# apelykh/deep-audio-mixer

Hardware: AMD Instinct MI355X
Metric: stem-spectrogram-frames/sec (train) (higher is better)
Workload: dtype f32; 1 GPU; C3: model_resnet (ResNet18, 8 stems) train step incl. STFT front-end, 8-stem 3 s @ 44.1 kHz stereo clips, n_fft 2048 hop 1024 -> 8x1025x130 per clip; batch_per_gpu=8, global_batch=8, parallelism=dp1, hip_graph=True, world_size=1, device_index=0, grad_buckets=1, allreduce_overlap=False

## Files before the change

deep-audio-mixer_amd/_lib.py:

```python
import ctypes
import os

import torch
import torch.utils.data

_HERE = os.path.dirname(os.path.abspath(__file__))
LIB_PATH = os.environ.get('DAM_LIB_PATH') or os.path.join(_HERE, 'libdam_hip.so')

EXPECTED_ABI = 27

_STATUS = {0: 'DAM_OK', -1: 'DAM_ERR_BAD_ARG', -2: 'DAM_ERR_UNSUPPORTED', -3: 'DAM_ERR_LAUNCH',
           -4: 'DAM_ERR_WORKSPACE'}

c_i, c_i64, c_f, c_p = ctypes.c_int, ctypes.c_int64, ctypes.c_float, ctypes.c_void_p
c_d = ctypes.c_double

SIGNATURES = {
    'dam_arch': (ctypes.c_char_p, []),
    'dam_abi_version': (c_i, []),
    'dam_host_dontfork_pinned': (c_i, [c_p, c_p]),
    'dam_step_mark_create': (c_i, [c_p]),
    'dam_step_mark_record': (c_i, [c_p, c_p]),
    'dam_step_mark_wait': (c_i, [c_p, c_p]),
    'dam_step_mark_synchronize': (c_i, [c_p]),
    'dam_step_mark_destroy': (c_i, [c_p]),
    'dam_stft_twiddle_count': (c_i64, [c_i]),
    'dam_stft_fill_twiddles_host': (c_i, [c_i, c_p]),
    'dam_stft_logmag_f32': (c_i, [c_p, c_i, c_i64, c_i64, c_i, c_i64, c_p, c_p, c_p, c_i, c_i, c_f, c_i, c_p, c_p]),
    'dam_stft_logmag_strided_f32': (c_i, [c_p, c_i, c_i64, c_i64, c_i64, c_i64, c_i64, c_i, c_i64, c_i64, c_p, c_p, c_p,
                                          c_i, c_i, c_f, c_i, c_p, c_p, c_i, c_p]),
    'dam_stft_complex_f32': (c_i, [c_p, c_i, c_i64, c_i64, c_i, c_i64, c_i64, c_i64, c_p, c_p, c_p, c_i, c_i, c_p, c_p]),
    'dam_stft_complex_strided_f32': (c_i, [c_p, c_i, c_i64, c_i64, c_i64, c_i64, c_i64, c_i64, c_i64, c_i, c_i64, c_i64,
                                           c_p, c_p, c_p, c_i, c_i, c_p, c_p]),
    'dam_istft_workspace_bytes': (c_i64, [c_i64, c_i64, c_i, c_i, c_i64]),
    'dam_istft_f32': (c_i, [c_p, c_p, c_i64, c_i64, c_i, c_i, c_i64, c_p, c_p, c_p, c_p, c_i64, c_p]),
    'dam_augment_gains_f32': (c_i, [ctypes.c_uint64, c_p, c_i64, c_i, c_i, c_f, c_f, c_p, c_p]),
    'dam_conv_packed_weight_count': (c_i64, [c_i, c_i, c_i, c_i]),
    'dam_conv_pack_weights_f32': (c_i, [c_p, c_i, c_i, c_i, c_i, c_i, c_p, c_p]),
    'dam_conv_pack_weights_multi_f32': (c_i, [c_p, c_i, c_i64, c_p]),
    'dam_conv2d_tapgrid_f32': (c_i, [c_p, c_i, c_i, c_i, c_i, c_i, c_p, c_i, c_i, c_p, c_p, c_p, c_i, c_i, c_p] +
                               [c_i] * 17 + [c_p, c_p, c_p, c_p, c_p, c_p, c_i64, c_p, c_p]),
    'dam_conv_batch_bytes': (c_i64, []),
    'dam_conv_batch_init': (c_i, [c_p]),
    'dam_conv_batch_flush': (c_i, [c_p, c_p]),
    'dam_conv_last_launch': (c_i, [c_p]),
    'dam_conv2d_wgrad_workspace_floats': (c_i64, [c_i, c_i, c_i, c_i]),
    'dam_conv2d_wgrad_f32': (c_i, [c_p, c_i, c_i, c_i, c_i, c_i, c_p, c_p, c_i, c_p] + [c_i] * 9 +
                             [c_p, c_i, c_p, c_i64, c_p, c_p]),
    'dam_wgrad_queue_bytes': (c_i64, []),
    'dam_wgrad_queue_init': (c_i, [c_p]),
    'dam_wgrad_queue_pending': (c_i, [c_p]),
    'dam_wgrad_queue_flush': (c_i, [c_p, c_p]),
    'dam_wgrad_queue_set_batching': (c_i, [c_p, c_i]),
    'dam_wgrad_last_launch': (c_i, [c_p]),
    'dam_bn_workspace_floats': (c_i64, [c_i]),
    'dam_bn_stats_f32': (c_i, [c_p, c_i64, c_i, c_p, c_p, c_p, c_p, c_p, c_f, c_f, c_p, c_p, c_p, c_p, c_p, c_p]),
    'dam_bn_finalize_f32': (c_i, [c_p, c_i, c_i, c_p, c_p, c_p, c_p, c_p, c_f, c_f, c_p, c_p, c_p, c_p, c_p]),
    'dam_conv1x1_pair_f32': (c_i, [c_p, c_p, c_i, c_p, c_p, c_i, c_i, c_i, c_i, c_i, c_i, c_p, c_i, c_i, c_i, c_i, c_i, c_p]),
    'dam_dgrad_s2_3x3_f32': (c_i, [c_p, c_p, c_p, c_p, c_i, c_i, c_i, c_i, c_i, c_p, c_i, c_i, c_p, c_p, c_p, c_p]),
    'dam_conv_s2_pair_fwd_f32': (c_i, [c_p, c_p, c_p, c_i, c_i, c_i, c_i, c_i, c_p, c_p, c_p, c_p, c_p, c_p]),
    'dam_bn_finalize_pair_f32': (c_i, [c_p, c_p, c_i, c_i, c_p, c_p, c_p]),
    'dam_strip_diag_counters': (c_i, [c_p, c_i]),
    'dam_bn_stats_partial_f32': (c_i, [c_p, c_i64, c_i, c_p, c_p, c_p]),
    'dam_bn_finalize_apply_f32': (c_i, [c_p, c_i, c_i, c_p, c_p, c_i64, c_p, c_p, c_p, c_i, c_p, c_p, c_p]),
    'dam_bn_eval_affine_f32': (c_i, [c_i, c_p, c_p, c_p, c_p, c_f, c_p, c_p, c_p, c_p, c_p]),
    'dam_bn_apply_f32': (c_i, [c_p, c_i64, c_i, c_p, c_p, c_p, c_p, c_p, c_i, c_p, c_p, c_p]),
    'dam_bn_stats_pair_f32': (c_i, [c_p, c_p, c_i64, c_i, c_p, c_p, c_p, c_p]),
    'dam_bn_pair_workspace_floats': (c_i64, [c_i]),
    'dam_bn_backward_pair_f32': (c_i, [c_p, c_p, c_p, c_i64, c_i, c_i] + [c_p] * 16),
    'dam_bn_backward_f32': (c_i, [c_p, c_p, c_p, c_i64, c_i, c_p, c_p, c_p, c_i, c_p, c_p, c_p, c_p, c_p, c_p, c_p, c_i, c_p]),
    'dam_channel_sum_f32': (c_i, [c_p, c_i64, c_i, c_i, c_p, c_p, c_p]),
    'dam_dropout_tick': (c_i, [c_p, c_i64, c_p, c_p]),
    'dam_dropout_apply_f32': (c_i, [c_p, c_i64, c_f, ctypes.c_uint64, c_p, c_p, c_p]),
    'dam_heads_fwd_f32': (c_i, [c_p, c_i, c_i, c_i, c_i, c_p, c_p, c_p, c_p, c_p, c_p, c_p]),
    'dam_heads_bwd_workspace_floats': (c_i64, [c_i, c_i, c_i, c_i]),
    'dam_heads_bwd_f32': (c_i, [c_p, c_p, c_p, c_i, c_i, c_i, c_i, c_p, c_p, c_p, c_p, c_p, c_p, c_p, c_p, c_p]),
    'dam_masksum_fwd_f32': (c_i, [c_p, c_p, c_i, c_i, c_i64, c_p, c_p]),
    'dam_masksum_workspace_floats': (c_i64, [c_i, c_i]),
    'dam_masksum_bwd_f32': (c_i, [c_p, c_p, c_i, c_i, c_i64, c_p, c_p, c_p]),
    'dam_masksum_mse_f32': (c_i, [c_p, c_p, c_p, c_i, c_i, c_i64, c_p, c_p, c_p, c_p, c_p]),
    'dam_adam_l2_step_f32': (c_i, [c_p, c_p, c_p, c_p, c_i64, c_p, c_p, c_f, c_f, c_f, c_f, c_f, c_f, c_p, c_p]),
    'dam_digest64_u32': (c_i, [c_p, c_i64, c_i64, c_i, c_i, c_p, c_p]),
    'dam_gains_smooth': (c_i, [c_p, c_i, c_i, c_i, c_i, c_p, c_p, c_p, c_p]),
    'dam_gain_ramp_apply': (c_i, [c_p, c_i, c_p, c_i64, c_i64, c_i64, c_i, c_p, c_i, c_p]),
    'dam_mixdown_workspace_elems': (c_i64, [c_i64]),
    'dam_mixdown_peak_normalize': (c_i, [c_p, c_i, c_p, c_i, c_i64, c_i64, c_i, c_i, c_p, c_i, c_p, c_p]),
    'dam_nchw_to_nhwc16_f32': (c_i, [c_p, c_i, c_i, c_i64, c_p, c_p]),
    'dam_loudness_kweight_coeffs': (c_i, [c_d, c_p]),
    'dam_loudness_workspace_bytes': (c_i64, [c_i64, c_i]),
    'dam_loudness_block_energy': (c_i, [c_p, c_i, c_i64, c_i, c_i64, c_i64, c_p, c_p, c_p, c_i, c_d, c_p, c_p, c_p]),
    'dam_loudness_batch_workspace_bytes': (c_i64, [c_i, c_i64, c_i, c_i]),
    'dam_loudness_block_energy_batch': (c_i, [c_p, c_i, c_i, c_i64, c_i, c_i64, c_i64, c_i64, c_p, c_i, c_p, c_p, c_p, c_i,
                                              c_d, c_p, c_p, c_p]),
    'dam_loudness_gate': (c_i, [c_p, c_i, c_i, c_i, c_p, c_p]),
    'dam_loudness_target_gains': (c_i, [c_p, c_p, c_i, c_p, c_p]),
    'dam_pcm_tile_frames': (c_i64, [c_i]),
    'dam_pcm_max_blocks': (c_i, []),
    'dam_pcm_encode': (c_i, [c_p, c_i, c_i, c_i64, c_p, c_i, c_i, c_i, ctypes.c_uint64, c_p, c_p, c_p]),
    'dam_true_peak_taps_host': (c_i, [c_p]),
    'dam_true_peak_tile_samples': (c_i64, []),
    'dam_true_peak_max_blocks': (c_i, []),
    'dam_true_peak_workspace_bytes': (c_i64, [c_i, c_i64, c_i]),
    'dam_true_peak_batch': (c_i, [c_p, c_i, c_i, c_i64, c_i, c_i64, c_i64, c_i64, c_p, c_i, c_p, c_p, c_p, c_p]),
    'dam_peak_limit_gains': (c_i, [c_p, c_p, c_i, c_i, c_d, c_p]),
    'dam_limiter_tile_samples': (c_i64, []),
    'dam_limiter_max_lookahead': (c_i, []),
    'dam_limiter_max_hold': (c_i, []),
    'dam_limiter_workspace_bytes': (c_i64, [c_i, c_i64]),
    'dam_limiter_apply': (c_i, [c_p, c_i, c_i, c_i64, c_i, c_i64, c_i64, c_i64, c_p, c_d, c_i, c_i, c_p, c_i, c_p, c_p, c_p, c_p]),
    'dam_loudness_window_power': (c_i, [c_p, c_i, c_i, c_i, c_i, c_p, c_p, c_p]),
    'dam_loudness_curve_stats': (c_i, [c_p, c_i, c_i, c_p, c_p]),
    'dam_loudness_profile_error': (c_i, [c_p, c_p, c_i, c_i, c_i, c_p, c_p, c_p]),
    'dam_spectrum_frames_per_block': (c_i, []),
    'dam_spectrum_max_bands': (c_i, []),
    'dam_spectrum_workspace_bytes': (c_i64, [c_i, c_i64, c_i, c_i]),
    'dam_spectrum_band_power': (c_i, [c_p, c_i, c_i, c_i, c_i, c_i64, c_i64, c_i64, c_i64, c_i64, c_p, c_i, c_p, c_p, c_i, c_i,
                                      c_p, c_i, c_p, c_p, c_p]),
    'dam_spectrum_balance_error': (c_i, [c_p, c_p, c_i, c_i, c_p, c_p, c_p]),
    'dam_gainfit_tile_samples': (c_i64, []),
    'dam_gainfit_workspace_bytes': (c_i64, [c_i, c_i64, c_i]),
    'dam_gainfit_moments': (c_i, [c_p, c_i, c_i, c_i, c_i64, c_i64, c_i64, c_i64, c_p, c_i, c_i64, c_i64, c_i, c_p, c_p, c_p]),
    'dam_gainfit_solve': (c_i, [c_p, c_i, c_i, c_i, c_d, c_p, c_p, c_p, c_p]),
    'dam_gainfit_gain_error': (c_i, [c_p, c_p, c_i, c_i, c_i, c_i, c_p, c_p, c_p, c_p]),
}



class BnFin(ctypes.Structure):
    _fields_ = [('gamma', c_p), ('beta', c_p), ('running_mean', c_p), ('running_var', c_p), ('num_batches_tracked', c_p),
                ('momentum', c_f), ('eps', c_f), ('save_mean', c_p), ('save_invstd', c_p), ('scale', c_p), ('shift', c_p)]


class BnBwdSums(ctypes.Structure):
    _fields_ = [('x', c_p), ('mean', c_p), ('invstd', c_p), ('mask_scale', c_p), ('mask_shift', c_p), ('res_mask_bits', c_p),
                ('mask_bits', c_p)]


_lib = None


def lib():
    global _lib
    if torch.cuda._is_in_bad_fork() or torch.utils.data.get_worker_info() is not None:
        raise RuntimeError('deep_audio_mixer_amd: a GPU kernel was asked for in a DataLoader worker / forked child process '
                           '(pid %d).  The GPU belongs to the parent: workers of MultitrackAudioDataset return host PCM '
                           '(PcmItem / HostPcmBatch) and the front-end runs in the main process -- see '
                           'features.batch_features(batch)' % os.getpid())
    if _lib is None:
        if not os.path.exists(LIB_PATH):
            raise RuntimeError('libdam_hip.so is not built (%s): run `python __graft_entry__.py` or '
                               '`python deep-audio-mixer_amd/build.py`; there is no CPU fallback' % LIB_PATH)
        l = ctypes.CDLL(LIB_PATH)
        l.dam_abi_version.restype, l.dam_abi_version.argtypes = c_i, []
        have = l.dam_abi_version()
        if have != EXPECTED_ABI:
            raise RuntimeError('%s speaks ABI version %d, this package expects %d: the library is stale -- rebuild it '
                               '(`python deep-audio-mixer_amd/build.py --force`)' % (LIB_PATH, have, EXPECTED_ABI))
        for name, (res, args) in SIGNATURES.items():
            fn = getattr(l, name)
            fn.restype, fn.argtypes = res, args
        _lib = l
    return _lib


def check(status, what):
    if status != 0:
        raise RuntimeError('%s failed: %s (%d)' % (what, _STATUS.get(status, '?'), status))


def ptr(t):
    return None if t is None else t.data_ptr()


def stream():
    return torch.cuda.current_stream().cuda_stream


def require_cuda(*tensors):
    for t in tensors:
        if t is not None and not t.is_cuda:
            raise RuntimeError('deep_audio_mixer_amd kernels run on the GPU only (got a %s tensor); '
                               'there is no CPU fallback' % t.device)
```

deep-audio-mixer_amd/csrc/dam_bn.hip:

```cpp
#include <type_traits>
#include "dam_common.h"

namespace dam {
namespace {

constexpr int BN_MAX_PARTS = 1024;
static_assert(BN_MAX_PARTS == BN_BWD_RECORDS_MAX, "records a data-gradient epilogue may leave");

struct BnLaunch { int threads, q, r, parts; int64_t ppb; };

inline BnLaunch bn_plan(int64_t P, int C, int max_parts = BN_MAX_PARTS) {
    BnLaunch l;
    l.q = C / 4;
    l.r = 256 / l.q;
    if (l.r < 1) l.r = 1;
    l.threads = l.q * l.r;
    int64_t parts = cdiv(P, (int64_t)l.r * 16);
    if (parts > max_parts) {
        parts = max_parts;
        while (l.threads < 1024 && parts * l.threads < 131072 && (size_t)(l.r * 2) * C * 3 * sizeof(float) <= 48 * 1024) {
            l.r *= 2;
            l.threads *= 2;
        }
    }
// ... 534 lines not shown
template <int MASK, int NB>
__global__ __launch_bounds__(FA_THREADS) void bn_bwd_fin_apply_kernel(const float* __restrict__ partial, int parts, int C, int CS,
                                                                       double count, int training, const BnBwdSides<NB> sd,
                                                                       const float* __restrict__ dy, const float* __restrict__ y_mask,
                                                                       int64_t P, int64_t ppr, const float* __restrict__ mscale,
                                                                       const float* __restrict__ mshift) {
    constexpr int NR = 1 + NB;
    __shared__ double red[FA_THREADS * NR];
    __shared__ __attribute__((aligned(16))) float tab[3 * NB * 32];
    const int tid = threadIdx.x, slice = blockIdx.y, q = CS / 4, tq = tid % q, tp = tid / q, ppi = FA_THREADS / q;
    const int Q = C / 4, cq = slice * q + tq;
    const int64_t lo = blockIdx.x * ppr, hi = (lo + ppr < P) ? lo + ppr : P;
    constexpr int UB = NB == 1 ? 3 : 2;
    const int64_t step = (int64_t)ppi * UB;
    float4 gv[2][UB], xv[NB][2][UB], mv[2][UB];
    auto load = [&](auto set, int64_t p0) {
        constexpr int S = decltype(set)::value;
#pragma unroll
        for (int u = 0; u < UB; ++u) {
            const int64_t p = p0 + (int64_t)u * ppi;
            const bool ok = p < hi;
            gv[S][u] = ok ? reinterpret_cast<const float4*>(dy)[p * Q + cq] : zero4();
#pragma unroll
            for (int s = 0; s < NB; ++s) xv[s][S][u] = ok ? reinterpret_cast<const float4*>(sd.s[s].x)[p * Q + cq] : zero4();
            if (MASK == 1) mv[S][u] = ok ? reinterpret_cast<const float4*>(y_mask)[p * Q + cq] : zero4();
            if (MASK == 3) mv[S][u] = sign_quad(ok ? reinterpret_cast<const unsigned char*>(y_mask)[p * Q + cq] : 0);
        }
    };
    load(FaSet<0>{}, lo + tp);
    float4 msc = zero4(), msh = zero4();
    if (MASK == 2) { msc = reinterpret_cast<const float4*>(mscale)[cq]; msh = reinterpret_cast<const float4*>(mshift)[cq]; }
    {
        const int cl = tid % CS, ch = slice * CS + cl;
        float gam[NB], inv[NB], mu[NB];
#pragma unroll
        for (int s = 0; s < NB; ++s) { gam[s] = sd.s[s].gamma[ch]; inv[s] = sd.s[s].invstd[ch]; mu[s] = sd.s[s].mean[ch]; }
        double acc[NR];
        fa_slice_sums<NR, NR>(partial, parts, C, ch, CS, red, acc, [](const float (&r)[NR], double (&v)[NR]) {
#pragma unroll
            for (int k = 0; k < NR; ++k) v[k] = (double)r[k];
        });
        if (tid < CS) {
#pragma unroll
            for (int s = 0; s < NB; ++s) {
                const double s1 = acc[0], s2 = acc[1 + s];
                const double g = (double)gam[s] * inv[s];
                double c2 = 0, c3 = 0;
                if (training) { c2 = -g * inv[s] * s2 / count; c3 = -g * s1 / count - c2 * mu[s]; }
                float* t = tab + 3 * s * CS;
                t[cl] = (float)g; t[CS + cl] = (float)c2; t[2 * CS + cl] = (float)c3;
                if (blockIdx.x == 0) { sd.s[s].dbeta[ch] = (float)s1; sd.s[s].dgamma[ch] = (float)s2; }
            }
        }
        __syncthreads();
    }
    float4 k[NB][3];
#pragma unroll
    for (int i = 0; i < 3 * NB; ++i) k[i / 3][i % 3] = *reinterpret_cast<const float4*>(tab + i * CS + tq * 4);
    fa_stream(lo + tp, hi, step, load, [&](auto set, int64_t p0) {
        constexpr int S = decltype(set)::value;
#pragma unroll
        for (int u = 0; u < UB; ++u) {
            const int64_t p = p0 + (int64_t)u * ppi;
            if (p < hi) {
                float4 g = gv[S][u];
                if (MASK != 0) {
                    float4 m = mv[S][u];
                    if (MASK == 2) {
                        const float4 v = xv[0][S][u];
                        m = make_float4(fmaf(v.x, msc.x, msh.x), fmaf(v.y, msc.y, msh.y), fmaf(v.z, msc.z, msh.z), fmaf(v.w, msc.w, msh.w));
                    }
                    g.x = m.x > 0.f ? g.x : 0.f; g.y = m.y > 0.f ? g.y : 0.f; g.z = m.z > 0.f ? g.z : 0.f; g.w = m.w > 0.f ? g.w : 0.f;
                }
                float4 o[NB];
#pragma unroll
                for (int s = 0; s < NB; ++s) {
                    const float4 v = xv[s][S][u], c1 = k[s][0], c2 = k[s][1], c3 = k[s][2];
                    o[s].x = fmaf(c1.x, g.x, fmaf(c2.x, v.x, c3.x)); o[s].y = fmaf(c1.y, g.y, fmaf(c2.y, v.y, c3.y));
                    o[s].z = fmaf(c1.z, g.z, fmaf(c2.z, v.z, c3.z)); o[s].w = fmaf(c1.w, g.w, fmaf(c2.w, v.w, c3.w));
                }
#pragma unroll
                for (int s = 0; s < NB; ++s) reinterpret_cast<float4*>(sd.s[s].dx)[p * Q + cq] = o[s];
            }
        }
    });
}

inline int elt_blocks(int64_t n) {
    int64_t b = cdiv(n, 256);
    return (int)(b < 4096 ? (b < 1 ? 1 : b) : 4096);
}

constexpr int FA_PARTS_KB = 64;
inline int fa_max_parts(int C, int rec_floats) {
    int m = FA_PARTS_KB * 1024 / (fa_cs(C) * rec_floats * 4);
    if (m > BN_MAX_PARTS) m = BN_MAX_PARTS;
    return m < 64 ? 64 : m;
}

inline bool fin_args(const dam_bn_fin* f, BnFinArgs* a) {
    if (!f || !f->gamma || !f->beta || !f->save_mean || !f->save_invstd || !f->scale || !f->shift) return false;
    *a = BnFinArgs{f->gamma, f->beta, f->running_mean, f->running_var, (long long*)f->num_batches_tracked, f->momentum,
                   f->eps, f->save_mean, f->save_invstd, f->scale, f->shift};
    return true;
}

template <int... MASKS, typename F>
inline bool with_mask(int mask, F f) {
    return ((mask == MASKS ? (f(std::integral_constant<int, MASKS>{}), true) : false) || ...);
}

template <int NB, int... MASKS>
inline int bn_bwd_launch(const BnLaunch& l, bool given, bool fused, int mask, const BnBwdSides<NB>& sd, const float* dy,
                         const float* y_mask, int64_t P, int C, int training, const float* mask_scale, const float* mask_shift,
                         float* workspace, hipStream_t st) {
    if (!given) {
        const bool known = with_mask<MASKS...>(mask, [&](auto m) {
            hipLaunchKernelGGL((bn_bwd_partial_kernel<decltype(m)::value, NB>), dim3(l.parts), dim3(l.threads),
                               (size_t)l.r * C * (1 + NB) * sizeof(float), st, dy, y_mask, sd, P, C, l.q, l.r, l.ppb, mask_scale,
                               mask_shift, workspace);
        });
        if (!known) return DAM_ERR_BAD_ARG;
        DAM_CHECK_LAUNCH();
    }
    if (fused) {
        const FaPlan f = fa_plan(P, C);
        const bool known = with_mask<MASKS...>(mask, [&](auto m) {
            hipLaunchKernelGGL((bn_bwd_fin_apply_kernel<decltype(m)::value, NB>), dim3(f.nranges, f.nslices), dim3(FA_THREADS), 0, st,
                               (const float*)workspace, l.parts, C, f.cs, (double)P, training, sd, dy, y_mask, P, f.ppr, mask_scale,
                               mask_shift);
        });
        if (!known) return DAM_ERR_BAD_ARG;
        DAM_CHECK_LAUNCH();
    }
    return DAM_OK;
}

}
}

using namespace dam;

extern "C" int64_t dam_bn_workspace_floats(int C) { return (int64_t)BN_RECORDS_MAX * C * 3; }

extern "C" int dam_bn_stats_partial_f32(const float* x, int64_t n_pixels, int C, float* workspace, int* parts_host, void* stream) {
    if (!x || !workspace || !parts_host || n_pixels <= 0) return DAM_ERR_BAD_ARG;
    if (C % 16 || C > 1024) return DAM_ERR_UNSUPPORTED;
    const BnLaunch l = bn_plan(n_pixels, C, fa_max_parts(C, 3));
    hipLaunchKernelGGL(bn_stats_partial_kernel, dim3(l.parts), dim3(l.threads), (size_t)l.r * C * 3 * sizeof(float), (hipStream_t)stream,
                       x, n_pixels, C, l.q, l.r, l.ppb, workspace, (const float*)nullptr, (float*)nullptr);
    DAM_CHECK_LAUNCH();
    *parts_host = l.parts;
    return DAM_OK;
}

extern "C" int dam_bn_finalize_apply_f32(const float* partial, int parts, int C, const dam_bn_fin* fin, const float* x,
                                         int64_t n_pixels, const float* res, const float* res_scale, const float* res_shift,
                                         int relu, float* y, uint8_t* sign_bits, void* stream) {
    BnFinArgs a;
    if (!partial || parts <= 0 || !fin_args(fin, &a) || !x || !y || n_pixels <= 0) return DAM_ERR_BAD_ARG;
    if (res_scale && (!res || !res_shift)) return DAM_ERR_BAD_ARG;
    if (C % 16 || C > 1024) return DAM_ERR_UNSUPPORTED;
    hipStream_t st = (hipStream_t)stream;
    if (!fa_fwd_table_ok(C, parts)) {
        int rc = dam_bn_finalize_f32(partial, parts, C, fin->gamma, fin->beta, fin->running_mean, fin->running_var,
                                     fin->num_batches_tracked, fin->momentum, fin->eps, fin->save_mean, fin->save_invstd, fin->scale,
                                     fin->shift, stream);
        if (rc != DAM_OK) return rc;
        return dam_bn_apply_f32(x, n_pixels, C, fin->scale, fin->shift, res, res_scale, res_shift, relu, y, sign_bits, stream);
    }
    const FaPlan f = fa_plan(n_pixels, C);
    hipLaunchKernelGGL(bn_fin_apply_kernel, dim3(f.nranges, f.nslices), dim3(FA_THREADS), 0, st, partial, parts, C, f.cs, a, x,
                       n_pixels, f.ppr, res, res_scale, res_shift, relu, y, sign_bits);
    DAM_CHECK_LAUNCH();
    return DAM_OK;
}

extern "C" int dam_bn_stats_f32(const float* x, int64_t n_pixels, int C, const float* gamma, const float* beta,
                                float* running_mean, float* running_var, int64_t* num_batches_tracked,
                                float momentum, float eps, float* save_mean, float* save_invstd, float* scale,
                                float* shift, float* workspace, void* stream) {
    if (!x || !gamma || !beta || !save_mean || !save_invstd || !scale || !shift || !workspace || n_pixels <= 0)
        return DAM_ERR_BAD_ARG;
    if (C % 16 || C > 1024) return DAM_ERR_UNSUPPORTED;
    const BnLaunch l = bn_plan(n_pixels, C);
    hipStream_t st = (hipStream_t)stream;
    hipLaunchKernelGGL(bn_stats_partial_kernel, dim3(l.parts), dim3(l.threads), (size_t)l.r * C * 3 * sizeof(float), st,
                       x, n_pixels, C, l.q, l.r, l.ppb, workspace, (const float*)nullptr, (float*)nullptr);
    DAM_CHECK_LAUNCH();
    hipLaunchKernelGGL(bn_stats_finalize_kernel, dim3(C), dim3(64), 0, st, workspace, l.parts, C,
                       gamma, beta, running_mean, running_var, (long long*)num_batches_tracked, momentum, eps,
                       save_mean, save_invstd, scale, shift, BnFinArgs{}, (const float*)nullptr);
    DAM_CHECK_LAUNCH();
    return DAM_OK;
}

extern "C" int dam_bn_stats_pair_f32(const float* x_a, const float* x_b, int64_t n_pixels, int C, const dam_bn_fin* a,
                                     const dam_bn_fin* b, float* workspace, void* stream) {
    BnFinArgs fa, fb;
    if (!x_a || !x_b || !fin_args(a, &fa) || !fin_args(b, &fb) || !workspace || n_pixels <= 0) return DAM_ERR_BAD_ARG;
    if (C % 16 || C > 1024) return DAM_ERR_UNSUPPORTED;
    const BnLaunch l = bn_plan(n_pixels, C);
    hipStream_t st = (hipStream_t)stream;
    float* ws_b = workspace + (size_t)BN_RECORDS_MAX * C * 3;
    hipLaunchKernelGGL(bn_stats_partial_kernel, dim3(l.parts, 2), dim3(l.threads), (size_t)l.r * C * 3 * sizeof(float), st, x_a,
                       n_pixels, C, l.q, l.r, l.ppb, workspace, x_b, ws_b);
    DAM_CHECK_LAUNCH();
    hipLaunchKernelGGL(bn_stats_finalize_kernel, dim3(C, 2), dim3(64), 0, st, workspace, l.parts, C, fa.gamma, fa.beta,
                       fa.running_mean, fa.running_var, fa.num_batches, fa.momentum, fa.eps, fa.save_mean, fa.save_invstd, fa.scale,
                       fa.shift, fb, (const float*)ws_b);
    DAM_CHECK_LAUNCH();
    return DAM_OK;
}

extern "C" int dam_bn_finalize_f32(const float* partial, int parts, int C, const float* gamma, const float* beta,
                                   float* running_mean, float* running_var, int64_t* num_batches_tracked,
                                   float momentum, float eps, float* save_mean, float* save_invstd, float* scale,
                                   float* shift, void* stream) {
    if (!partial || parts <= 0 || C <= 0 || !gamma || !beta || !save_mean || !save_invstd || !scale || !shift)
        return DAM_ERR_BAD_ARG;
    hipLaunchKernelGGL(bn_stats_finalize_kernel, dim3(C), dim3(64), 0, (hipStream_t)stream, partial, parts, C, gamma, beta,
                       running_mean, running_var, (long long*)num_batches_tracked, momentum, eps, save_mean, save_invstd,
                       scale, shift, BnFinArgs{}, (const float*)nullptr);
    DAM_CHECK_LAUNCH();
    return DAM_OK;
}

extern "C" int dam_bn_finalize_pair_f32(const float* partial_a, const float* partial_b, int parts, int C, const dam_bn_fin* a,
                                        const dam_bn_fin* b, void* stream) {
    BnFinArgs fa, fb;
    if (!partial_a || !partial_b || parts <= 0 || C <= 0 || !fin_args(a, &fa) || !fin_args(b, &fb)) return DAM_ERR_BAD_ARG;
    hipLaunchKernelGGL(bn_stats_finalize_kernel, dim3(C, 2), dim3(64), 0, (hipStream_t)stream, partial_a, parts, C, fa.gamma, fa.beta,
                       fa.running_mean, fa.running_var, fa.num_batches, fa.momentum, fa.eps, fa.save_mean, fa.save_invstd, fa.scale,
                       fa.shift, fb, partial_b);
    DAM_CHECK_LAUNCH();
    return DAM_OK;
}

extern "C" int dam_bn_eval_affine_f32(int C, const float* gamma, const float* beta, const float* running_mean,
                                      const float* running_var, float eps, float* save_mean, float* save_invstd,
                                      float* scale, float* shift, void* stream) {
    if (!gamma || !beta || !running_mean || !running_var || !save_mean || !save_invstd || !scale || !shift || C <= 0)
        return DAM_ERR_BAD_ARG;
    hipLaunchKernelGGL(bn_eval_affine_kernel, dim3((unsigned)cdiv(C, 64)), dim3(64), 0, (hipStream_t)stream, C, gamma, beta,
                       running_mean, running_var, eps, save_mean, save_invstd, scale, shift);
    DAM_CHECK_LAUNCH();
    return DAM_OK;
}

extern "C" int dam_bn_apply_f32(const float* x, int64_t n_pixels, int C, const float* scale, const float* shift,
                                const float* res, const float* res_scale, const float* res_shift, int relu, float* y,
                                uint8_t* sign_bits, void* stream) {
    if (!x || !scale || !shift || !y || n_pixels <= 0) return DAM_ERR_BAD_ARG;
    if (C % 16) return DAM_ERR_UNSUPPORTED;
    if (res_scale && (!res || !res_shift)) return DAM_ERR_BAD_ARG;
    const int64_t nq = n_pixels * (C / 4);
    hipLaunchKernelGGL(bn_apply_kernel, dim3(elt_blocks(nq)), dim3(256), 0, (hipStream_t)stream, x, nq, C / 4, scale, shift,
                       res, res_scale, res_shift, relu, y, sign_bits);
    DAM_CHECK_LAUNCH();
    return DAM_OK;
}

extern "C" int dam_bn_backward_f32(const float* dy, const float* y_mask, const float* x, int64_t n_pixels, int C,
                                   const float* gamma, const float* save_mean, const float* save_invstd, int training,
                                   const float* mask_scale, const float* mask_shift, const uint8_t* mask_bits, float* dx,
                                   float* dgamma, float* dbeta, float* workspace, int partials_given, void* stream) {
    if (!dy || !x || !gamma || !save_mean || !save_invstd || !dx || !dgamma || !dbeta || !workspace || n_pixels <= 0)
        return DAM_ERR_BAD_ARG;
    if ((mask_scale != nullptr) != (mask_shift != nullptr) || (y_mask && mask_scale) || (mask_bits && (y_mask || mask_scale)))
        return DAM_ERR_BAD_ARG;
    if (mask_bits) y_mask = reinterpret_cast<const float*>(mask_bits);
    if (C % 16 || C > 1024) return DAM_ERR_UNSUPPORTED;
    BnLaunch l = bn_plan(n_pixels, C, fa_max_parts(C, 2));
    if (partials_given < 0 || partials_given > BN_MAX_PARTS) return DAM_ERR_BAD_ARG;
    if (partials_given) l.parts = partials_given;
    const bool fused = fa_table_ok(C, l.parts, 2);
    hipStream_t st = (hipStream_t)stream;
    const int mask = mask_bits ? 3 : (y_mask ? 1 : (mask_scale ? 2 : 0));
    const BnBwdSides<1> sd{{{x, gamma, save_mean, save_invstd, dx, dgamma, dbeta}}};
    const int rc = bn_bwd_launch<1, 0, 1, 2, 3>(l, partials_given != 0, fused, mask, sd, dy, y_mask, n_pixels, C, training,
                                                mask_scale, mask_shift, workspace, st);
    if (rc != DAM_OK || fused) return rc;
    float* coef = workspace + (size_t)BN_MAX_PARTS * C * 2;
    hipLaunchKernelGGL(bn_bwd_finalize_kernel, dim3(C), dim3(64), 0, st, workspace, l.parts, C,
                       (double)n_pixels, gamma, save_mean, save_invstd, training, dgamma, dbeta, coef);
    DAM_CHECK_LAUNCH();
    const int64_t nq = n_pixels * (C / 4);
    const bool known = with_mask<0, 1, 2, 3>(mask, [&](auto m) {
        hipLaunchKernelGGL(bn_bwd_apply_kernel<decltype(m)::value>, dim3(elt_blocks(nq)), dim3(256), 0, st, dy, y_mask, x, nq, C / 4,
                           C, (const float*)coef, mask_scale, mask_shift, dx);
    });
    if (!known) return DAM_ERR_BAD_ARG;
    DAM_CHECK_LAUNCH();
    return DAM_OK;
}

extern "C" int64_t dam_bn_pair_workspace_floats(int C) { return (int64_t)BN_MAX_PARTS * C * 3 + 6 * (int64_t)C; }

extern "C" int dam_bn_backward_pair_f32(const float* dy, const float* y_mask, const uint8_t* mask_bits, int64_t n_pixels, int C,
                                        int training,
                                        const float* x_a, const float* gamma_a, const float* mean_a, const float* invstd_a,
                                        float* dx_a, float* dgamma_a, float* dbeta_a,
                                        const float* x_b, const float* gamma_b, const float* mean_b, const float* invstd_b,
                                        float* dx_b, float* dgamma_b, float* dbeta_b, float* workspace, void* stream) {
    if ((y_mask != nullptr) == (mask_bits != nullptr)) return DAM_ERR_BAD_ARG;
    const bool bits = mask_bits != nullptr;
    if (bits) y_mask = reinterpret_cast<const float*>(mask_bits);
    if (!dy || !y_mask || !x_a || !gamma_a || !mean_a || !invstd_a || !dx_a || !dgamma_a || !dbeta_a || !x_b || !gamma_b ||
        !mean_b || !invstd_b || !dx_b || !dgamma_b || !dbeta_b || !workspace || n_pixels <= 0)
        return DAM_ERR_BAD_ARG;
    if (C % 16 || C > 1024) return DAM_ERR_UNSUPPORTED;
    const BnLaunch l = bn_plan(n_pixels, C, fa_max_parts(C, 3));
    if ((size_t)l.r * C * 3 * sizeof(float) > 64 * 1024) return DAM_ERR_UNSUPPORTED;
    const BnBwdSides<2> sd{{{x_a, gamma_a, mean_a, invstd_a, dx_a, dgamma_a, dbeta_a},
                            {x_b, gamma_b, mean_b, invstd_b, dx_b, dgamma_b, dbeta_b}}};
    return bn_bwd_launch<2, 1, 3>(l, false, true, bits ? 3 : 1, sd, dy, y_mask, n_pixels, C, training, nullptr, nullptr, workspace,
                                  (hipStream_t)stream);
}

extern "C" int dam_channel_sum_f32(const float* x, int64_t n_pixels, int C, int n_real, float* out, float* workspace,
                                   void* stream) {
    if (!x || !out || !workspace || n_pixels <= 0 || n_real <= 0 || n_real > C) return DAM_ERR_BAD_ARG;
    if (C % 16 || C > 1024) return DAM_ERR_UNSUPPORTED;
    const BnLaunch l = bn_plan(n_pixels, C);
    hipStream_t st = (hipStream_t)stream;
    hipLaunchKernelGGL(channel_sum_partial_kernel, dim3(l.parts), dim3(l.threads), (size_t)l.r * C * sizeof(float), st, x,
                       n_pixels, C, l.q, l.r, l.ppb, workspace);
    DAM_CHECK_LAUNCH();
    hipLaunchKernelGGL(channel_sum_finalize_kernel, dim3(n_real), dim3(64), 0, st, workspace, l.parts, C,
                       n_real, out);
    DAM_CHECK_LAUNCH();
    return DAM_OK;
}
```

deep-audio-mixer_amd/csrc/dam_conv.hip:

```cpp
#include <cstdlib>
#include "dam_common.h"
#include "dam_conv_geo.h"
#include "dam_conv_stage.h"

namespace dam {

namespace {

typedef float v4f __attribute__((ext_vector_type(4)));

constexpr int GEO_PACK_MAX = 4;
struct ConvGeoPack {
    ConvGeo g[GEO_PACK_MAX];
    int n, B;
};

template <int MB, int NB>
__global__ __launch_bounds__(256) void conv_igemm_kernel(const ConvGeoPack pk, const float* __restrict__ X,
                                                         const float4* __restrict__ Wp, const float* __restrict__ bias,
                                                         const float* __restrict__ in_scale,
                                                         const float* __restrict__ in_shift, float* __restrict__ Y,
                                                         const float* __restrict__ res, const float* __restrict__ res_mask,
                                                         float* __restrict__ splitk_ws) {
    extern __shared__ __attribute__((aligned(16))) unsigned char smem[];
// ... 249 lines not shown
};

int conv_pack_dispatch(const ConvGeoPack& pk, const ConvLaunchRec& r, hipStream_t st) {
#define DAM_CONV_PCASE(M_, N_) \
    if (r.MB == M_ && r.NB == N_) return launch_conv_pack<M_, N_>(pk, r.lds, r.X, r.Wp, r.bias, r.sc, r.sh, r.Y, r.res, r.res_mask, r.ws, st)
    DAM_CONV_PCASE(4, 4); DAM_CONV_PCASE(4, 2); DAM_CONV_PCASE(4, 1);
    DAM_CONV_PCASE(4, 3); DAM_CONV_PCASE(2, 3); DAM_CONV_PCASE(1, 3);
    DAM_CONV_PCASE(2, 4); DAM_CONV_PCASE(2, 2); DAM_CONV_PCASE(2, 1);
    DAM_CONV_PCASE(1, 4); DAM_CONV_PCASE(1, 2); DAM_CONV_PCASE(1, 1);
#undef DAM_CONV_PCASE
    return DAM_ERR_UNSUPPORTED;
}

int conv_batch_flush(ConvBatch& b, hipStream_t st) {
    int i = 0, rc = DAM_OK;
    while (i < b.n && rc == DAM_OK) {
        const ConvLaunchRec& r = b.rec[i];
        ConvGeoPack pk;
        pk.B = r.g.B; pk.n = 0;
        size_t lds = 0;
        int k = i;
        while (k < b.n && pk.n < GEO_PACK_MAX) {
            const ConvLaunchRec& q = b.rec[k];
            if (q.MB != r.MB || q.NB != r.NB || q.X != r.X || q.Wp != r.Wp || q.bias != r.bias || q.sc != r.sc || q.sh != r.sh ||
                q.Y != r.Y || q.res != r.res || q.res_mask != r.res_mask || q.g.B != r.g.B)
                break;
            pk.g[pk.n++] = q.g;
            lds = q.lds > lds ? q.lds : lds;
            ++k;
        }
        ConvLaunchRec merged = r;
        merged.lds = lds;
        rc = conv_pack_dispatch(pk, merged, st);
        i = k;
    }
    b.n = 0;
    return rc;
}

}
}

extern "C" int64_t dam_conv_packed_weight_count(int n_out, int k_in, int kh, int kw) {
    if (n_out <= 0 || k_in <= 0 || kh <= 0 || kw <= 0) return 0;
    return (int64_t)kh * kw * dam::cdiv(k_in, 16) * dam::cdiv(n_out, 16) * 256;
}

extern "C" int dam_conv_pack_weights_f32(const float* w_oihw, int O, int I, int KH, int KW, int transpose,
                                         float* packed, void* stream) {
    using namespace dam;
    if (!w_oihw || !packed || O <= 0 || I <= 0 || KH <= 0 || KW <= 0) return DAM_ERR_BAD_ARG;
    const int n = transpose ? I : O, k = transpose ? O : I;
    const int nchunks = (int)cdiv(k, 16), nblks = (int)cdiv(n, 16);
    const int64_t total = (int64_t)KH * KW * nchunks * nblks * 256;
    const int blocks = (int)(cdiv(total, 256) < 2048 ? cdiv(total, 256) : 2048);
    hipLaunchKernelGGL(pack_weights_kernel, dim3(blocks), dim3(256), 0, (hipStream_t)stream, w_oihw, O, I, KH, KW,
                       transpose, nchunks, nblks, packed, total);
    DAM_CHECK_LAUNCH();
    return DAM_OK;
}

extern "C" int dam_conv_pack_weights_multi_f32(const int64_t* desc_dev, int n_tensors, int64_t max_total, void* stream) {
    using namespace dam;
    if (!desc_dev || n_tensors <= 0 || max_total <= 0) return DAM_ERR_BAD_ARG;
    if (n_tensors > 65535) return DAM_ERR_UNSUPPORTED;
    int64_t bx = cdiv(max_total, 256 * 9);
    if (bx > 256) bx = 256;
    if (bx < 1) bx = 1;
    hipLaunchKernelGGL(pack_weights_multi_kernel, dim3((unsigned)bx, (unsigned)n_tensors), dim3(256), 0, (hipStream_t)stream,
                       reinterpret_cast<const long long*>(desc_dev));
    DAM_CHECK_LAUNCH();
    return DAM_OK;
}

namespace dam {
namespace {

template <int NB, int NCHMAX>
__global__ __launch_bounds__(256) void conv1x1_direct_kernel(const ConvGeo g, const float* __restrict__ X,
                                                             const float4* __restrict__ Wp, const float* __restrict__ bias,
                                                             float* __restrict__ Y, const float* __restrict__ res,
                                                             const float* __restrict__ res_mask, int segs, int total_units) {
    const int lane = threadIdx.x & 63, wave = threadIdx.x >> 6;
    const int j = lane & 15, kq = lane >> 4;
    const int unit = blockIdx.x * 4 + wave;
    if (unit >= total_units) return;
    const int nb0 = blockIdx.y * NB;
    const int seg = unit % segs, row = unit / segs, img = row / g.Ho, oh = row - img * g.Ho;
    const int ow = seg * 16 + j;
    const bool valid = ow < g.Wo;
    const int ih = oh * g.s + g.off_h, iw = ow * g.s + g.off_w;
    const bool inb = valid && ih >= 0 && ih < g.H && iw >= 0 && iw < g.W;
    const __amdgpu_buffer_rsrc_t xr = __builtin_amdgcn_make_buffer_rsrc(const_cast<float*>(X), 0, 0x7fffffff, 0x00020000);
    const __amdgpu_buffer_rsrc_t wr = __builtin_amdgcn_make_buffer_rsrc(const_cast<float4*>(Wp), 0, 0x7fffffff, 0x00020000);
    const int xoff = inb ? (((img * g.H + ih) * g.W + iw) * g.C + kq * 4) * 4 : 0x7fffffff;
    const int tap = g.wt_base;
    float4 xv[NCHMAX], wa[NCHMAX][NB];
#pragma unroll
    for (int c = 0; c < NCHMAX; ++c) {
        const bool cok = c < g.nchunks;
        xv[c] = __builtin_bit_cast(float4, __builtin_amdgcn_raw_buffer_load_b128(xr, cok ? xoff : 0x7fffffff, c * 64, 0));
#pragma unroll
        for (int nb = 0; nb < NB; ++nb)
            wa[c][nb] = __builtin_bit_cast(float4, __builtin_amdgcn_raw_buffer_load_b128(
                wr, cok ? lane * 16 : 0x7fffffff, (((tap * g.nchunks + c) * g.NBtot + nb0 + nb) * 64) * 16, 0));
    }
    v4f acc[NB];
#pragma unroll
    for (int nb = 0; nb < NB; ++nb) acc[nb] = (v4f){0.f, 0.f, 0.f, 0.f};
#pragma unroll
    for (int c = 0; c < NCHMAX; ++c)
#pragma unroll
        for (int nb = 0; nb < NB; ++nb) {
            acc[nb] = __builtin_amdgcn_mfma_f32_16x16x4f32(wa[c][nb].x, xv[c].x, acc[nb], 0, 0, 0);
            acc[nb] = __builtin_amdgcn_mfma_f32_16x16x4f32(wa[c][nb].y, xv[c].y, acc[nb], 0, 0, 0);
            acc[nb] = __builtin_amdgcn_mfma_f32_16x16x4f32(wa[c][nb].z, xv[c].z, acc[nb], 0, 0, 0);
            acc[nb] = __builtin_amdgcn_mfma_f32_16x16x4f32(wa[c][nb].w, xv[c].w, acc[nb], 0, 0, 0);
        }
    if (!valid) return;
    const size_t opix = ((size_t)img * g.OHt + (oh * g.os + g.oo_h)) * g.OWt + (ow * g.os + g.oo_w);
#pragma unroll
    for (int nb = 0; nb < NB; ++nb) {
        const int ch = (nb0 + nb) * 16 + kq * 4;
        v4f v = acc[nb];
        if (bias) v += *reinterpret_cast<const v4f*>(bias + ch);
        const size_t o = opix * g.N + ch;
        if (res) {
            const float4 rv = *reinterpret_cast<const float4*>(res + o);
            if (res_mask) {
                const float4 mv = *reinterpret_cast<const float4*>(res_mask + o);
                v.x += mv.x > 0.f ? rv.x : 0.f; v.y += mv.y > 0.f ? rv.y : 0.f;
                v.z += mv.z > 0.f ? rv.z : 0.f; v.w += mv.w > 0.f ? rv.w : 0.f;
            } else {
                v.x += rv.x; v.y += rv.y; v.z += rv.z; v.w += rv.w;
            }
        }
        if (g.relu_out) { v.x = fmaxf(v.x, 0.f); v.y = fmaxf(v.y, 0.f); v.z = fmaxf(v.z, 0.f); v.w = fmaxf(v.w, 0.f); }
        *reinterpret_cast<float4*>(Y + o) = make_float4(v.x, v.y, v.z, v.w);
    }
}

template <int NB, int R, bool BOTH>
__global__ __launch_bounds__(256) void conv1x1_pair_kernel(const float* __restrict__ X1, const float4* __restrict__ Wp1, int tap1,
                                                           const float* __restrict__ X2, const float4* __restrict__ Wp2, int tap2,
                                                           int B, int H, int W, int C, int N, float* __restrict__ Y, int OHt, int OWt,
                                                           int os, int oo_h, int oo_w, int segs, int total_units) {
    const int lane = threadIdx.x & 63, wave = threadIdx.x >> 6;
    const int j = lane & 15, kq = lane >> 4;
    const int unit = blockIdx.x * 4 + wave;
    if (unit >= total_units) return;
    const int nb0 = blockIdx.y * NB, nch = C / 16, NBtot = N / 16;
    const int seg = unit % segs, row = unit / segs, img = row / H, oh = row - img * H;
    const int ow = seg * 16 + j;
    const bool valid = ow < W;
    const int xoff = valid ? (((img * H + oh) * W + ow) * C + kq * 4) * 4 : 0x7fffffff;
    v4f acc[NB];
#pragma unroll
    for (int nb = 0; nb < NB; ++nb) acc[nb] = (v4f){0.f, 0.f, 0.f, 0.f};
    const __amdgpu_buffer_rsrc_t xr1 = __builtin_amdgcn_make_buffer_rsrc(const_cast<float*>(X1), 0, 0x7fffffff, 0x00020000);
    const __amdgpu_buffer_rsrc_t wr1 = __builtin_amdgcn_make_buffer_rsrc(const_cast<float4*>(Wp1), 0, 0x7fffffff, 0x00020000);
    const __amdgpu_buffer_rsrc_t xr2 = __builtin_amdgcn_make_buffer_rsrc(const_cast<float*>(X2), 0, 0x7fffffff, 0x00020000);
    const __amdgpu_buffer_rsrc_t wr2 = __builtin_amdgcn_make_buffer_rsrc(const_cast<float4*>(Wp2), 0, 0x7fffffff, 0x00020000);
#define DAM_PAIR_LOAD(XR_, WR_, TAP_, C0_, XV_, WA_)                                                                          \
    _Pragma("unroll") for (int c = 0; c < R; ++c) {                                                                           \
        const bool cok = (C0_) + c < nch;                                                                                     \
        XV_[c] = __builtin_bit_cast(float4, __builtin_amdgcn_raw_buffer_load_b128(XR_, cok ? xoff : 0x7fffffff, ((C0_) + c) * 64, 0)); \
        _Pragma("unroll") for (int nb = 0; nb < NB; ++nb)                                                                     \
            WA_[c][nb] = __builtin_bit_cast(float4, __builtin_amdgcn_raw_buffer_load_b128(                                    \
                WR_, cok ? lane * 16 : 0x7fffffff, ((((TAP_) * nch + (C0_) + c) * NBtot + nb0 + nb) * 64) * 16, 0));          \
    }
#define DAM_PAIR_MFMA(XV_, WA_)                                    \
    _Pragma("unroll") for (int c = 0; c < R; ++c)                                                                             \
        _Pragma("unroll") for (int nb = 0; nb < NB; ++nb) {                                                                   \
            acc[nb] = __builtin_amdgcn_mfma_f32_16x16x4f32(WA_[c][nb].x, XV_[c].x, acc[nb], 0, 0, 0);                         \
            acc[nb] = __builtin_amdgcn_mfma_f32_16x16x4f32(WA_[c][nb].y, XV_[c].y, acc[nb], 0, 0, 0);                         \
            acc[nb] = __builtin_amdgcn_mfma_f32_16x16x4f32(WA_[c][nb].z, XV_[c].z, acc[nb], 0, 0, 0);                         \
            acc[nb] = __builtin_amdgcn_mfma_f32_16x16x4f32(WA_[c][nb].w, XV_[c].w, acc[nb], 0, 0, 0);                         \
        }
    if constexpr (BOTH) {
        float4 xa[R], wa[R][NB], xb[R], wb[R][NB];
        DAM_PAIR_LOAD(xr1, wr1, tap1, 0, xa, wa)
        DAM_PAIR_LOAD(xr2, wr2, tap2, 0, xb, wb)
        DAM_PAIR_MFMA(xa, wa)
        DAM_PAIR_MFMA(xb, wb)
    } else {
        float4 xa[R], wa[R][NB], xb[R], wb[R][NB];
        const int rounds = (nch + R - 1) / R, total = 2 * rounds;
        DAM_PAIR_LOAD(xr1, wr1, tap1, 0, xa, wa)
#pragma unroll 1
        for (int r = 0; r < total; r += 2) {
            {
                const int q = r + 1, c0 = (q >= rounds ? q - rounds : q) * R;
                if (q >= rounds) { DAM_PAIR_LOAD(xr2, wr2, tap2, c0, xb, wb) } else { DAM_PAIR_LOAD(xr1, wr1, tap1, c0, xb, wb) }
            }
            DAM_PAIR_MFMA(xa, wa)
            if (r + 2 < total) {
                const int q = r + 2, c0 = (q >= rounds ? q - rounds : q) * R;
                if (q >= rounds) { DAM_PAIR_LOAD(xr2, wr2, tap2, c0, xa, wa) } else { DAM_PAIR_LOAD(xr1, wr1, tap1, c0, xa, wa) }
            }
            DAM_PAIR_MFMA(xb, wb)
        }
    }
#undef DAM_PAIR_LOAD
#undef DAM_PAIR_MFMA
    if (!valid) return;
    const size_t opix = ((size_t)img * OHt + (oh * os + oo_h)) * OWt + (ow * os + oo_w);
#pragma unroll
    for (int nb = 0; nb < NB; ++nb) {
        const int ch = (nb0 + nb) * 16 + kq * 4;
        *reinterpret_cast<float4*>(Y + opix * N + ch) = make_float4(acc[nb].x, acc[nb].y, acc[nb].z, acc[nb].w);
    }
}

template <int NB, int NCHMAX>
int launch_conv1x1(const ConvGeo& g, const float* X, const float* Wp, const float* bias, float* Y, const float* res,
                   const float* res_mask, hipStream_t st) {
    const int segs = (int)cdiv(g.Wo, 16);
    const int64_t units = (int64_t)g.B * g.Ho * segs;
    if (units >= (1ll << 30)) return DAM_ERR_UNSUPPORTED;
    hipLaunchKernelGGL((conv1x1_direct_kernel<NB, NCHMAX>), dim3((unsigned)cdiv(units, 4), (unsigned)(g.N / 16 / NB)), dim3(256), 0, st,
                       g, X, reinterpret_cast<const float4*>(Wp), bias, Y, res, res_mask, segs, (int)units);
    DAM_CHECK_LAUNCH();
    conv_last_launch = ConvLaunchNote{CONV_FAM_1X1, 0, NB, NCHMAX, 0, 0, 0, 0, 0, 0, 0, 1, 1};
    return DAM_OK;
}

}
}

extern "C" int dam_conv1x1_pair_f32(const float* x1, const float* w1_packed, int tap1, const float* x2, const float* w2_packed,
                                    int tap2, int B, int H, int W, int C, int n_out, float* y, int OHt, int OWt, int out_stride,
                                    int out_off_h, int out_off_w, void* stream) {
    using namespace dam;
    if (!x1 || !w1_packed || !x2 || !w2_packed || !y || B <= 0 || H <= 0 || W <= 0 || tap1 < 0 || tap2 < 0 || out_stride < 1)
        return DAM_ERR_BAD_ARG;
    if (C % 16 || n_out % 16 || C <= 0 || n_out <= 0) return DAM_ERR_UNSUPPORTED;
    if ((H - 1) * out_stride + out_off_h >= OHt || (W - 1) * out_stride + out_off_w >= OWt || out_off_h < 0 || out_off_w < 0)
        return DAM_ERR_BAD_ARG;
    if ((int64_t)B * H * W * C * 4 >= (1ll << 31)) return DAM_ERR_UNSUPPORTED;
    const int segs = (int)cdiv(W, 16);
    const int64_t units = (int64_t)B * H * segs;
    if (units >= (1ll << 30)) return DAM_ERR_UNSUPPORTED;
    const int nblk = n_out / 16, nch = C / 16;
    hipStream_t st = (hipStream_t)stream;
#define DAM_PAIR_GO(NB_, R_, BOTH_)                                                                                           \
    hipLaunchKernelGGL((conv1x1_pair_kernel<NB_, R_, BOTH_>), dim3((unsigned)cdiv(units, 4), (unsigned)(nblk / NB_)), dim3(256), 0, st, x1, \
                       reinterpret_cast<const float4*>(w1_packed), tap1, x2, reinterpret_cast<const float4*>(w2_packed), tap2, B, H, W, \
                       C, n_out, y, OHt, OWt, out_stride, out_off_h, out_off_w, segs, (int)units)
    if (nblk % 2 == 0) {
        if (nch <= 2) DAM_PAIR_GO(2, 2, true); else if (nch <= 4) DAM_PAIR_GO(2, 4, true); else DAM_PAIR_GO(2, 4, false);
    } else {
        if (nch <= 2) DAM_PAIR_GO(1, 2, true); else if (nch <= 4) DAM_PAIR_GO(1, 4, true); else DAM_PAIR_GO(1, 8, false);
    }
#undef DAM_PAIR_GO
    DAM_CHECK_LAUNCH();
    return DAM_OK;
}

namespace dam {
thread_local ConvLaunchNote conv_last_launch{};
}

extern "C" int dam_conv_last_launch(int* out16_host) {
    if (!out16_host) return DAM_ERR_BAD_ARG;
    const dam::ConvLaunchNote& n = dam::conv_last_launch;
    const int v[16] = {n.family, n.MB, n.NB, n.NCH, n.T33, n.LW, n.EPI, n.SO, n.PU, n.STATS, n.KS, n.ksplit, n.ranges, 0, 0, 0};
    for (int i = 0; i < 16; ++i) out16_host[i] = v[i];
    return DAM_OK;
}

extern "C" int64_t dam_conv_batch_bytes(void) { return (int64_t)sizeof(dam::ConvBatch); }

extern "C" int dam_conv_batch_init(void* batch) {
    if (!batch) return DAM_ERR_BAD_ARG;
    dam::ConvBatch* b = static_cast<dam::ConvBatch*>(batch);
    b->magic = dam::CONV_BATCH_MAGIC;
    b->n = 0;
    return DAM_OK;
}

extern "C" int dam_conv_batch_flush(void* batch, void* stream) {
    dam::ConvBatch* b = static_cast<dam::ConvBatch*>(batch);
    if (!b || b->magic != dam::CONV_BATCH_MAGIC) return DAM_ERR_BAD_ARG;
    return dam::conv_batch_flush(*b, (hipStream_t)stream);
}

extern "C" int dam_conv2d_tapgrid_f32(const float* x, int B, int H, int W, int C, int in_nchw, const float* w_packed,
                                      int k_chunks, int n_out, const float* bias, const float* in_scale,
                                      const float* in_shift, int relu_in, int relu_out, float* y, int OHt, int OWt, int Ho, int Wo,
                                      int out_stride, int out_off_h, int out_off_w, int in_stride, int nA, int nB,
                                      int off_h, int step_h, int off_w, int step_w, int wt_base, int wt_sa, int wt_sb,
                                      const float* res, const float* res_mask, float* bn_partial, int* bn_parts_host,
                                      const dam_bn_bwd_sums* bn_bwd, float* workspace, int64_t workspace_floats,
                                      void* batch, void* stream) {
    using namespace dam;
    conv_last_launch = ConvLaunchNote{};
    if (bn_parts_host) *bn_parts_host = 0;
    BnBwdEpi bwd{};
    if (bn_bwd && bn_bwd->x) {
        if (!bn_partial || !bn_parts_host || !bn_bwd->mean || !bn_bwd->invstd) return DAM_ERR_BAD_ARG;
        if (bn_bwd->mask_bits ? (bn_bwd->mask_scale || bn_bwd->mask_shift || !res) : (!bn_bwd->mask_scale || !bn_bwd->mask_shift))
            return DAM_ERR_BAD_ARG;
        if (res && (!bn_bwd->res_mask_bits || !res_mask)) return DAM_ERR_BAD_ARG;
        bwd = BnBwdEpi{bn_bwd->x, bn_bwd->mean, bn_bwd->invstd, bn_bwd->mask_scale, bn_bwd->mask_shift, bn_bwd->res_mask_bits,
                       bn_bwd->mask_bits};
    }
    if (!x || !w_packed || !y || B <= 0 || H <= 0 || W <= 0 || C <= 0 || Ho <= 0 || Wo <= 0 || nA <= 0 || nB <= 0)
        return DAM_ERR_BAD_ARG;
    if (n_out % 16 || (in_stride != 1 && in_stride != 2) || out_stride < 1) return DAM_ERR_UNSUPPORTED;
    if (in_nchw ? (C > 16 || k_chunks != 1) : (C % 16 || k_chunks != C / 16)) return DAM_ERR_UNSUPPORTED;
    if (in_scale && !in_shift) return DAM_ERR_BAD_ARG;
    if (B > 65535) return DAM_ERR_UNSUPPORTED;
    ConvGeo g;
    g.B = B; g.H = H; g.W = W; g.C = C; g.Ho = Ho; g.Wo = Wo; g.N = n_out; g.OHt = OHt; g.OWt = OWt;
    g.os = out_stride; g.oo_h = out_off_h; g.oo_w = out_off_w; g.s = in_stride; g.nA = nA; g.nB = nB;
    g.off_h = off_h; g.step_h = step_h; g.off_w = off_w; g.step_w = step_w;
    g.wt_base = wt_base; g.wt_sa = wt_sa; g.wt_sb = wt_sb;
    g.in_nchw = in_nchw; g.relu_in = relu_in; g.relu_out = relu_out != 0; g.nchunks = k_chunks; g.NBtot = n_out / 16;
    g.epi_bwd = 0;
    const int h_lo = off_h + (step_h < 0 ? (nA - 1) * step_h : 0), h_hi = off_h + (step_h > 0 ? (nA - 1) * step_h : 0);
    const int w_lo = off_w + (step_w < 0 ? (nB - 1) * step_w : 0), w_hi = off_w + (step_w > 0 ? (nB - 1) * step_w : 0);
    g.r0 = h_lo; g.c0 = w_lo;
    g.PWin = (Wo - 1) * in_stride + (w_hi - w_lo) + 1;
    g.PWs = (int)cdiv(g.PWin, in_stride);
    g.PWT = g.PWs * in_stride;

    hipStream_t st = (hipStream_t)stream;
    g.PR = 0; g.CG = 1; g.tiles_m = 0; g.ksplit = 1; g.gps = 1 << 30;
    if (nA == 1 && nB == 1 && !in_nchw && !in_scale && k_chunks <= 8 &&
        (int64_t)B * H * W * C * 4 < (1ll << 31) && (int64_t)B * OHt * OWt * n_out * 4 < (1ll << 62)) {
        const int nblk = n_out / 16;
        if (k_chunks <= 2) return nblk % 2 == 0 ? launch_conv1x1<2, 2>(g, x, w_packed, bias, y, res, res_mask, st)
                                                : launch_conv1x1<1, 2>(g, x, w_packed, bias, y, res, res_mask, st);
        if (k_chunks <= 4) return nblk % 2 == 0 ? launch_conv1x1<2, 4>(g, x, w_packed, bias, y, res, res_mask, st)
                                                : launch_conv1x1<1, 4>(g, x, w_packed, bias, y, res, res_mask, st);
        return nblk % 2 == 0 ? launch_conv1x1<2, 8>(g, x, w_packed, bias, y, res, res_mask, st)
                             : launch_conv1x1<1, 8>(g, x, w_packed, bias, y, res, res_mask, st);
    }
    if (!in_nchw) {
        int parts = 0;
        const int rc = conv_strip_try(g, h_lo, h_hi, x, w_packed, bias, y, res, res_mask, bn_partial, &parts,
                                      in_scale, in_shift, bwd, st);
        if (rc == DAM_OK) {
            if (bn_partial && bn_parts_host) *bn_parts_host = parts;
            return DAM_OK;
        }
        if (rc != DAM_ERR_UNSUPPORTED) return rc;
        if (bn_partial) {
            const int rc2 = conv_strip_try(g, h_lo, h_hi, x, w_packed, bias, y, res, res_mask, nullptr, nullptr, in_scale, in_shift,
                                           BnBwdEpi{}, st);
            if (rc2 == DAM_OK) return DAM_OK;
            if (rc2 != DAM_ERR_UNSUPPORTED) return rc2;
        }
    }
    if (!getenv("DAM_NO_PIPE")) {
        int parts = 0;
        const int rc = conv_pipe_try(g, h_hi - h_lo, x, w_packed, bias, in_scale, in_shift, y, res, res_mask, workspace,
                                     (bwd.x && res) ? nullptr : bn_partial, &parts, (bwd.x && res) ? BnBwdEpi{} : bwd, st);
        if (rc == DAM_OK && bn_partial && bn_parts_host) *bn_parts_host = parts;
        if (rc != DAM_ERR_UNSUPPORTED) return rc;
        if (nA == 3 && nB == 3 && !in_nchw && !bn_partial) {
            for (int ns = 2; ns <= 4; ++ns) {
                const int wd0 = (int)cdiv(Wo, ns);
                if (wd0 < 16) break;
                int rc2 = DAM_OK, done = 0;
                for (int ow0 = 0; ow0 < Wo && rc2 == DAM_OK; ow0 += wd0, ++done) {
                    ConvGeo g2 = g;
                    g2.Wo = Wo - ow0 < wd0 ? Wo - ow0 : wd0;
                    g2.oo_w = out_off_w + ow0 * out_stride;
                    g2.off_w = off_w + ow0 * in_stride;
                    g2.c0 = w_lo + ow0 * in_stride;
                    g2.PWin = (g2.Wo - 1) * in_stride + (w_hi - w_lo) + 1;
                    g2.PWs = (int)cdiv(g2.PWin, in_stride);
                    g2.PWT = g2.PWs * in_stride;
                    rc2 = conv_pipe_try(g2, h_hi - h_lo, x, w_packed, bias, in_scale, in_shift, y, res, res_mask, workspace, nullptr,
                                        nullptr, BnBwdEpi{}, st);
                }
                if (rc2 == DAM_OK) {
                    conv_last_launch.family = CONV_FAM_PIPE_RANGES;
                    conv_last_launch.ranges = done;
                    return DAM_OK;
                }
                if (rc2 != DAM_ERR_UNSUPPORTED || done > 1) return rc2 == DAM_ERR_UNSUPPORTED ? DAM_ERR_LAUNCH : rc2;
            }
        }
    }
    const int64_t npix = (int64_t)Ho * Wo;
    const int nblk = n_out / 16;
    int MB = 4, NB = nblk % 4 == 0 ? 4 : (nblk % 3 == 0 ? 3 : (nblk % 2 == 0 ? 2 : 1));
    auto wgs = [&](int mb, int nb) { return cdiv(npix, 64 * mb) * cdiv(nblk, nb) * B; };
    const bool can_split = workspace && out_stride == 1 && Ho == OHt && Wo == OWt && out_off_h == 0 && out_off_w == 0 &&
                           k_chunks >= 4;
    bool split = can_split;
    if (split) {
        int64_t best = -1;
        for (int mb = 4; mb >= 1; mb >>= 1) {
            const int64_t w = wgs(mb, NB);
            if (w < 400) continue;
            const int64_t cost = cdiv(w, 256) * (mb * NB + 1);
            if (best < 0 || cost < best) { best = cost; MB = mb; split = false; }
        }
    }
    if (split) {
        int64_t best_pad = -1;
        for (int mb = 4; mb >= 1; mb >>= 1) {
            const int64_t pad = cdiv(npix, 64 * mb) * 64 * mb;
            if (best_pad < 0 || pad * 10 < best_pad * 9) { best_pad = pad; MB = mb; }
        }
    } else if (!can_split) {
        while (wgs(MB, NB) < 512 && (MB > 1 || NB > 1)) {
            if (MB > 1 && (MB >= NB || NB == 1)) MB >>= 1; else NB >>= 1;
        }
    }
    const size_t LDS_MAX = 64 * 1024;
    int CG = 1;
    while (CG * 2 <= 4 && k_chunks % (CG * 2) == 0) CG *= 2;
    auto patch_rows = [&](int mb) {
        const int tm = 64 * mb;
        int rows_out = (int)((tm + Wo - 2) / Wo + 1);
        if (rows_out > Ho) rows_out = Ho;
        return (rows_out - 1) * in_stride + (h_hi - h_lo) + 1;
    };
    for (;;) {
        g.PR = patch_rows(MB);
        const size_t bytes = (size_t)CG * g.PR * g.PWT * 64;
        if (bytes <= LDS_MAX) break;
        if (CG > 1) CG >>= 1;
        else if (MB > 1) MB >>= 1;
        else if (bytes <= 150 * 1024) break;
        else return DAM_ERR_UNSUPPORTED;
    }
    g.CG = CG;
    g.tiles_m = (int)cdiv(npix, 64 * MB);
    if (split) {
        const int ngroups = k_chunks / CG;
        const int64_t w = wgs(MB, NB), out_elems = (int64_t)B * OHt * OWt * n_out;
        int ksplit = (int)cdiv(512, w);
        if (ksplit > 8) ksplit = 8;
        if (ksplit > ngroups) ksplit = ngroups;
        while (ksplit > 1 && ksplit * out_elems > workspace_floats) --ksplit;
        if (ksplit > 1) {
            g.gps = (int)cdiv(ngroups, ksplit);
            g.ksplit = (int)cdiv(ngroups, g.gps);
        }
    }
    const size_t lds = (size_t)CG * g.PR * g.PWT * 64;
    if (batch && g.ksplit == 1) {
        ConvBatch* cb = static_cast<ConvBatch*>(batch);
        if (cb->magic != CONV_BATCH_MAGIC) return DAM_ERR_BAD_ARG;
        if (cb->n == CONV_BATCH_MAX) {
            const int rc = conv_batch_flush(*cb, st);
            if (rc != DAM_OK) return rc;
        }
        ConvLaunchRec& r = cb->rec[cb->n++];
        r.g = g; r.MB = MB; r.NB = NB; r.lds = lds; r.X = x; r.Wp = w_packed; r.bias = bias; r.sc = in_scale; r.sh = in_shift;
        r.res = res; r.res_mask = res_mask; r.Y = y; r.ws = workspace;
        conv_last_launch = ConvLaunchNote{CONV_FAM_TILE_BATCH, MB, NB, 0, 0, 0, 0, 0, 0, 0, 0, 1, 1};
        return DAM_OK;
    }
#define DAM_CONV_CASE(M_, N_) \
    if (MB == M_ && NB == N_) return launch_conv<M_, N_>(g, lds, x, w_packed, bias, in_scale, in_shift, y, res, res_mask, workspace, st)
    DAM_CONV_CASE(4, 4); DAM_CONV_CASE(4, 2); DAM_CONV_CASE(4, 1);
    DAM_CONV_CASE(4, 3); DAM_CONV_CASE(2, 3); DAM_CONV_CASE(1, 3);
    DAM_CONV_CASE(2, 4); DAM_CONV_CASE(2, 2); DAM_CONV_CASE(2, 1);
    DAM_CONV_CASE(1, 4); DAM_CONV_CASE(1, 2); DAM_CONV_CASE(1, 1);
#undef DAM_CONV_CASE
    return DAM_ERR_UNSUPPORTED;
}
```

deep-audio-mixer_amd/csrc/dam_conv_geo.h:

```cpp
#pragma once
#include "dam_common.h"

namespace dam {

struct ConvGeo {
    int B, H, W, C;
    int Ho, Wo;
    int N;
    int OHt, OWt;
    int os, oo_h, oo_w;
    int s;
    int nA, nB;
    int off_h, step_h, off_w, step_w;
    int wt_base, wt_sa, wt_sb;
    int r0, c0;
    int PR, PWin, PWs, PWT;
    int nchunks, CG;
    int NBtot;
    int tiles_m;
    int in_nchw;
    int relu_in;
    int relu_out;
    int ksplit;
    int gps;
    int epi_bwd;
};

struct BnBwdEpi {
    const float* x;
    const float* mean; const float* invstd; const float* mscale; const float* mshift;
    const unsigned char* res_bits;
    const unsigned char* mask_bits;
};

struct StripGeo {
    int NR;
    int RH;
    int tiles_m, tpw, strips;
    int ring_off;
    int w_lds;
    int w_taps;
    unsigned wo_magic;
};

enum ConvFamily { CONV_FAM_NONE = 0, CONV_FAM_STRIP = 1, CONV_FAM_PIPE = 2, CONV_FAM_PIPE_RANGES = 3, CONV_FAM_TILE = 4,
                  CONV_FAM_TILE_BATCH = 5, CONV_FAM_1X1 = 6 };
struct ConvLaunchNote {
    int family, MB, NB, NCH, T33, LW, EPI, SO, PU, STATS, KS, ksplit, ranges;
};
extern thread_local ConvLaunchNote conv_last_launch;

int conv_strip_try(ConvGeo& g, int h_lo, int h_hi, const float* X, const float* Wp, const float* bias, float* Y,
                   const float* res, const float* res_mask, float* stats, int* stats_parts,
                   const float* in_scale, const float* in_shift, const BnBwdEpi& bwd, hipStream_t st);

int conv_pipe_try(ConvGeo g, int row_span, const float* X, const float* Wp, const float* bias, const float* sc, const float* sh,
                  float* Y, const float* res, const float* res_mask, float* workspace, float* stats, int* stats_parts,
                  const BnBwdEpi& bwd, hipStream_t st);

}
```

deep-audio-mixer_amd/csrc/dam_conv_pipe.hip:

```cpp
#include <climits>
#include <cstdlib>
#include "dam_common.h"
#include "dam_conv_geo.h"
#include "dam_conv_stage.h"

namespace dam {
namespace {

typedef float v4f __attribute__((ext_vector_type(4)));

constexpr int PIPE_LT = 256;
constexpr int PIPE_THREADS = 256 + PIPE_LT;
constexpr int PIPE_BUF1 = 32768;

#define DAM_PIPE_BARRIER() asm volatile("s_waitcnt lgkmcnt(0)\n\ts_barrier" ::: "memory")

#ifdef DAM_PIPE_STAMPS
#define DAM_PSTAMP(role, tag)                                                                                         \
    do {                                                                                                              \
        if (lane == 0 && (wave == 0 || wave == 4) && stamp_n < 64) {                                                  \
            const unsigned long long t_ = __builtin_readcyclecounter();                                               \
            stamp_p[(role) * 64 + stamp_n++] = ((unsigned long long)(tag) << 56) | (t_ & ((1ull << 56) - 1));         \
        }                                                                                                             \
    } while (0)
#else
#define DAM_PSTAMP(role, tag) do { } while (0)
#endif

struct PipeUnit {
    int p0, img, nb0, oh_first;
};

template <int UPX, int NB>
__device__ __forceinline__ PipeUnit pipe_decode(const ConvGeo& g, int unit, int nby, float inv_wo) {
    PipeUnit u;
    const int r = unit / g.tiles_m, tm = unit - r * g.tiles_m;
    u.img = r / nby;
    u.nb0 = (r - u.img * nby) * NB;
    u.p0 = tm * UPX;
    u.oh_first = fast_div(u.p0, g.Wo, inv_wo);
    return u;
}

template <int MB, int NB, int PIPE_U, int STATS, int KS>
__global__ __launch_bounds__(PIPE_THREADS) void conv_pipe_kernel(const ConvGeo g, const int nunits, const float* __restrict__ X,
                                                                 const float4* __restrict__ Wp, const float* __restrict__ bias,
                                                                 const float* __restrict__ in_scale,
                                                                 const float* __restrict__ in_shift, float* __restrict__ Y,
                                                                 const float* __restrict__ res, const float* __restrict__ res_mask,
                                                                 float* __restrict__ stamps, float* __restrict__ stats,
                                                                 const BnBwdEpi bwd) {
    extern __shared__ __attribute__((aligned(16))) unsigned char smem[];
    const int tid = threadIdx.x, lane = tid & 63;
    const int wave = __builtin_amdgcn_readfirstlane(tid >> 6);
    constexpr int MW = 16 * MB;
    constexpr int MT = 4 / KS;
    constexpr int UPX = MW * MT;
    constexpr int QM = 4 * KS - 1;
    const int HoWo = g.Ho * g.Wo;
    const float inv_wo = 1.0f / (float)g.Wo;
    const int chunk_bytes = g.PR * g.PWT * 64;
    const int stage_bytes = chunk_bytes * KS;
    const int nst = g.nchunks / KS;
    const int nby = g.N / 16 / NB;
    const bool xa = (gridDim.x & 7) == 0;
    const int G = xa ? (int)gridDim.x >> 3 : (int)gridDim.x;
    const int per_xcd = xa ? (nunits + 7) >> 3 : nunits;
    const int u_lo = xa ? (int)(blockIdx.x & 7) * per_xcd : 0;
    const int unit_end = u_lo + per_xcd < nunits ? u_lo + per_xcd : nunits;
    const int unit0 = u_lo + (xa ? (int)(blockIdx.x >> 3) : (int)blockIdx.x);
    if (unit0 >= unit_end) return;
    const size_t img_floats = (size_t)g.H * g.W * g.C;
#ifdef DAM_PIPE_STAMPS
    unsigned long long* stamp_p = reinterpret_cast<unsigned long long*>(stamps) + (size_t)blockIdx.x * 128;
    int stamp_n = 0;
#endif
    DAM_PSTAMP(wave >> 2, 1);

    if (wave >= 4) {
        const int ltid = tid - 256;
        const int WC = g.W * g.C;
        const int ipr = g.PWin * 4 * KS;
        const int total = g.PR * ipr;
        const int tab_off = PIPE_BUF1 + stage_bytes;
        const int dump_off = tab_off + (in_scale ? 2 * g.C * 4 : 0);
        int dst[PIPE_U], gcol[PIPE_U];
        {
            const int step_r = PIPE_LT / ipr, step_c = PIPE_LT - step_r * ipr;
            int pr = fast_div(ltid, ipr, 1.0f / (float)ipr), rem = ltid - pr * ipr;
#pragma unroll
            for (int u = 0; u < PIPE_U; ++u) {
                dst[u] = dump_off + ltid * 16; gcol[u] = INT_MIN;
                if (ltid + PIPE_LT * u < total) {
                    const int pw = rem / (4 * KS), cq = rem & QM;
                    const int slot = g.s == 1 ? pw : (pw & 1) * g.PWs + (pw >> 1);
                    dst[u] = ((pr * g.PWT + slot) * 16 + (cq & 3) * 4) * 4 + (cq >> 2) * chunk_bytes;
                    const int iw = g.c0 + pw;
                    if (iw >= 0 && iw < g.W) gcol[u] = (pr * WC + iw * g.C + cq * 4) * 4;
                }
                pr += step_r; rem += step_c;
                if (rem >= ipr) { rem -= ipr; ++pr; }
            }
        }
        const int cq4 = (lane & QM) * 4;
        const float relu_lo = g.relu_in ? 0.f : -__builtin_inff();
        float4 v[2][PIPE_U];
        int unit = unit0;
        PipeUnit cur = pipe_decode<UPX, NB>(g, unit, nby, inv_wo);
        int icg = 0;
        int rowb = (cur.oh_first * g.s + g.r0) * WC * 4;
        const unsigned img_bytes = (unsigned)img_floats * 4u;
        __amdgpu_buffer_rsrc_t xrsrc =
            __builtin_amdgcn_make_buffer_rsrc(const_cast<float*>(X + (size_t)cur.img * img_floats), 0, img_bytes, 0x00020000);
        bool head = true;
        int s_sb[2] = {0, 0}, s_cg[2] = {0, 0};
        bool s_live[2] = {false, false};
#define DAM_PIPE_REFILL(S_)                                                                                                \
    do {                                                                                                                   \
        const int sb_ = head ? rowb + icg * (64 * KS) : INT_MIN;                                                                \
        _Pragma("unroll") for (int u = 0; u < PIPE_U; ++u)                                                                 \
            v[S_][u] = __builtin_bit_cast(float4, __builtin_amdgcn_raw_buffer_load_b128(xrsrc, gcol[u] + sb_, 0, 0));      \
        s_sb[S_] = sb_; s_cg[S_] = icg; s_live[S_] = head;                                                                 \
        if (head) {                                                                                  \
            if (icg + 1 < nst) {                                                                                           \
                ++icg;                                                                                                     \
            } else if (unit + G < unit_end) {                                                                                \
                unit += G;                                                                                                 \
                cur = pipe_decode<UPX, NB>(g, unit, nby, inv_wo);                                                          \
                icg = 0;                                                                                                   \
                rowb = (cur.oh_first * g.s + g.r0) * WC * 4;                                                               \
                xrsrc = __builtin_amdgcn_make_buffer_rsrc(const_cast<float*>(X + (size_t)cur.img * img_floats), 0, img_bytes, \
                                                          0x00020000);                                                     \
            } else {                                                                                                       \
                head = false;                                                                                              \
            }                                                                                                              \
        }                                                                                                                  \
    } while (0)
#define DAM_PIPE_COMMIT(S_)                                  \
    do {                                                                                                                   \
        constexpr int boff_ = (S_) * PIPE_BUF1;                                                                            \
        if (in_scale) {                                          \
            const float4 sc = *reinterpret_cast<const float4*>(smem + tab_off + (s_cg[S_] * (16 * KS) + cq4) * 4);         \
            const float4 sh = *reinterpret_cast<const float4*>(smem + tab_off + (g.C + s_cg[S_] * (16 * KS) + cq4) * 4);   \
            _Pragma("unroll") for (int u = 0; u < PIPE_U; ++u) {                                                           \
                float4 x = v[S_][u];                                                                                       \
                x.x = fmaf(x.x, sc.x, sh.x); x.y = fmaf(x.y, sc.y, sh.y);                                                  \
                x.z = fmaf(x.z, sc.z, sh.z); x.w = fmaf(x.w, sc.w, sh.w);                                                  \
                x.x = fmaxf(x.x, relu_lo); x.y = fmaxf(x.y, relu_lo); x.z = fmaxf(x.z, relu_lo); x.w = fmaxf(x.w, relu_lo);  \
                if ((unsigned)(gcol[u] + s_sb[S_]) >= img_bytes) x = make_float4(0.f, 0.f, 0.f, 0.f);                      \
                *reinterpret_cast<float4*>(smem + boff_ + dst[u]) = x;                                                     \
            }                                                                                                              \
        } else {                                                                                                           \
            _Pragma("unroll") for (int u = 0; u < PIPE_U; ++u)                                                             \
                *reinterpret_cast<float4*>(smem + boff_ + dst[u]) = v[S_][u];                                              \
        }                                                                                                                  \
    } while (0)
#define DAM_PIPE_ROUND_END()                                 \
    do {                                                                                                                   \
        DAM_PSTAMP(1, 6);                                                                                                  \
        DAM_PIPE_BARRIER();                                                                                                \
        DAM_PSTAMP(1, 7);                                                                                                  \
    } while (0)
        if (in_scale)
            for (int e = ltid * 4; e < g.C; e += PIPE_LT * 4) {
                *reinterpret_cast<float4*>(smem + tab_off + e * 4) = *reinterpret_cast<const float4*>(in_scale + e);
                *reinterpret_cast<float4*>(smem + tab_off + (g.C + e) * 4) = *reinterpret_cast<const float4*>(in_shift + e);
            }
        if (g.s != 1)
            for (int e = ltid * 16; e < stage_bytes; e += PIPE_LT * 16) {
                *reinterpret_cast<float4*>(smem + e) = make_float4(0.f, 0.f, 0.f, 0.f);
                *reinterpret_cast<float4*>(smem + PIPE_BUF1 + e) = make_float4(0.f, 0.f, 0.f, 0.f);
            }
        DAM_PIPE_REFILL(0);
        __builtin_amdgcn_sched_barrier(0);
        DAM_PIPE_REFILL(1);
        __builtin_amdgcn_sched_barrier(0);
        DAM_PSTAMP(1, 2);
        DAM_PIPE_BARRIER();
        DAM_PSTAMP(1, 3);
        for (;;) {
            DAM_PIPE_COMMIT(0);
            DAM_PIPE_REFILL(0);
            DAM_PIPE_ROUND_END();
            if (!s_live[1]) break;
            DAM_PIPE_COMMIT(1);
            DAM_PIPE_REFILL(1);
            DAM_PIPE_ROUND_END();
            if (!s_live[0]) break;
        }
        DAM_PIPE_BARRIER();
#undef DAM_PIPE_REFILL
#undef DAM_PIPE_COMMIT
#undef DAM_PIPE_ROUND_END
        return;
    }

    const int j = lane & 15, kq = lane >> 4;
    const int mt = wave & (MT - 1), kh = wave / MT;
    const int part_off = PIPE_BUF1 + stage_bytes + (in_scale ? 2 * g.C * 4 : 0) + PIPE_LT * 16;
    int tapw[9], tapx[9];
#pragma unroll
    for (int t = 0; t < 9; ++t) {
        const int a = t / 3, b = t % 3;
        tapw[t] = (g.wt_base + a * g.wt_sa + b * g.wt_sb) * g.nchunks * g.NBtot * 1024;
        const int roff = g.off_h + a * g.step_h - g.r0, coff = g.off_w + b * g.step_w - g.c0;
        const int slotoff = g.s == 1 ? coff : (coff & 1) * g.PWs + (coff >> 1);
        tapx[t] = (roff * g.PWT + slotoff) * 64;
    }
    const int lane16 = lane * 16;
    const __amdgpu_buffer_rsrc_t wrsrc = __builtin_amdgcn_make_buffer_rsrc(const_cast<float4*>(Wp), 0, 0x7fffffff, 0x00020000);
    constexpr bool W9 = MB * NB == 1;
    constexpr int WSETS = W9 ? 9 : 3;
    v4f acc[MB][NB];
    float4 wa[WSETS][NB], xv[3][MB];
    int base_b[MB];
    int unit = unit0;
    PipeUnit cur = pipe_decode<UPX, NB>(g, unit, nby, inv_wo);
    int sbuf = 0;
#define DAM_PIPE_W(S_, CPART_, T_)                                                                                         \
    do {                                                                                                                   \
        const int ws_ = tapw[T_] + (CPART_);                                                                                \
        _Pragma("unroll") for (int nb = 0; nb < NB; ++nb)                                                                  \
            wa[S_][nb] = __builtin_bit_cast(float4, __builtin_amdgcn_raw_buffer_load_b128(wrsrc, lane16 + nb * 1024, ws_, 0)); \
    } while (0)
#define DAM_PIPE_X(S_, T_)                                                                                                 \
    do {                                                                                                                   \
        const int lo_ = boff + tapx[T_];                                                                                   \
        _Pragma("unroll") for (int mb = 0; mb < MB; ++mb)                                                                  \
            xv[S_][mb] = *reinterpret_cast<const float4*>(smem + base_b[mb] + lo_);                                        \
    } while (0)
#define DAM_PIPE_MFMA2(SW_, SX_)                                                                                           \
    do {                                                                                                                   \
        _Pragma("unroll") for (int mb = 0; mb < MB; ++mb)                                                                  \
            _Pragma("unroll") for (int nb = 0; nb < NB; ++nb) {                                                            \
                acc[mb][nb] = __builtin_amdgcn_mfma_f32_16x16x4f32(wa[SW_][nb].x, xv[SX_][mb].x, acc[mb][nb], 0, 0, 0);    \
                acc[mb][nb] = __builtin_amdgcn_mfma_f32_16x16x4f32(wa[SW_][nb].y, xv[SX_][mb].y, acc[mb][nb], 0, 0, 0);    \
                acc[mb][nb] = __builtin_amdgcn_mfma_f32_16x16x4f32(wa[SW_][nb].z, xv[SX_][mb].z, acc[mb][nb], 0, 0, 0);    \
                acc[mb][nb] = __builtin_amdgcn_mfma_f32_16x16x4f32(wa[SW_][nb].w, xv[SX_][mb].w, acc[mb][nb], 0, 0, 0);    \
            }                                                                                                              \
    } while (0)
#define DAM_PIPE_MFMA(S_) DAM_PIPE_MFMA2(S_, S_)
    {
        const int cfirst = (kh * g.NBtot + cur.nb0) * 1024;
        DAM_PIPE_W(0, cfirst, 0);
        DAM_PIPE_W(1, cfirst, 1);
        if constexpr (W9) {
            DAM_PIPE_W(2 % WSETS, cfirst, 2); DAM_PIPE_W(3 % WSETS, cfirst, 3); DAM_PIPE_W(4 % WSETS, cfirst, 4);
            DAM_PIPE_W(5 % WSETS, cfirst, 5); DAM_PIPE_W(6 % WSETS, cfirst, 6); DAM_PIPE_W(7 % WSETS, cfirst, 7);
            DAM_PIPE_W(8 % WSETS, cfirst, 8);
        }
    }
    DAM_PSTAMP(0, 2);
    DAM_PIPE_BARRIER();
    DAM_PSTAMP(0, 3);
    DAM_PIPE_BARRIER();
    DAM_PSTAMP(0, 5);
    for (;;) {
        const bool has_next = unit + G < unit_end;
        const PipeUnit nxt = has_next ? pipe_decode<UPX, NB>(g, unit + G, nby, inv_wo) : cur;
#pragma unroll
        for (int mb = 0; mb < MB; ++mb) {
            int p = cur.p0 + mt * MW + mb * 16 + j;
            p = p < HoWo ? p : HoWo - 1;
            const int oh = fast_div(p, g.Wo, inv_wo), ow = p - oh * g.Wo;
            base_b[mb] = (((oh - cur.oh_first) * g.s) * g.PWT + ow) * 64 + kq * 16;
#pragma unroll
            for (int nb = 0; nb < NB; ++nb) acc[mb][nb] = (v4f){0.f, 0.f, 0.f, 0.f};
        }
        for (int cg = 0; cg < nst; ++cg) {
            const int boff = (sbuf & 1) * PIPE_BUF1 + kh * chunk_bytes;
            ++sbuf;
            const int ccur = ((cg * KS + kh) * g.NBtot + cur.nb0) * 1024;
            const int cnext = cg + 1 < nst ? ccur + KS * g.NBtot * 1024 : (kh * g.NBtot + nxt.nb0) * 1024;
#define DAM_PIPE_SCHED_A()                                                                                                 \
    do { if constexpr (NB < 4) __builtin_amdgcn_sched_barrier(0); } while (0)
#define DAM_PIPE_SCHED_B()                                                                                                 \
    do {                                                                                                                   \
        if constexpr (NB >= 4) {                                                                                           \
            _Pragma("unroll") for (int i_ = 0; i_ < NB; ++i_) {                                                            \
                __builtin_amdgcn_sched_group_barrier(0x008, 1, 0);                                                         \
                __builtin_amdgcn_sched_group_barrier(0x020, 1, 0);                                                         \
            }                                                                                                              \
            __builtin_amdgcn_sched_group_barrier(0x008, 1, 0);                                                             \
            __builtin_amdgcn_sched_group_barrier(0x100, MB, 0);                                                            \
            __builtin_amdgcn_sched_group_barrier(0x008, 4 * MB * NB, 0);                                                   \
        }                                                                                                                  \
        __builtin_amdgcn_sched_barrier(0);                                                                                 \
    } while (0)
#define DAM_PIPE_ITEM(SW_, CP_, TW_, SX_, TX_, SM_)                                                                        \
    do {                                                                                                                   \
        DAM_PIPE_W(SW_, CP_, TW_);                                                                                         \
        if ((TX_) >= 0) DAM_PIPE_X(SX_, (TX_) < 0 ? 0 : (TX_));                                                            \
        DAM_PIPE_SCHED_A();                                                                                                \
        DAM_PIPE_MFMA(SM_);                                                                                                \
        DAM_PIPE_SCHED_B();                                                                                                \
    } while (0)
#define DAM_PIPE_ITEM9(T_)                                   \
    do {                                                                                                                   \
        if ((T_) + 2 < 9) DAM_PIPE_X(((T_) + 2) % 3, (T_) + 2 < 9 ? (T_) + 2 : 0);                                         \
        __builtin_amdgcn_sched_barrier(0);                                                                                 \
        DAM_PIPE_MFMA2((T_) % WSETS, (T_) % 3);                                                                            \
        DAM_PIPE_W((T_) % WSETS, cnext, T_);                                                                               \
        __builtin_amdgcn_sched_barrier(0);                                                                                 \
    } while (0)
            DAM_PIPE_X(0, 0);
            DAM_PIPE_X(1, 1);
            __builtin_amdgcn_sched_barrier(0);
            if constexpr (W9) {
                DAM_PIPE_ITEM9(0); DAM_PIPE_ITEM9(1); DAM_PIPE_ITEM9(2); DAM_PIPE_ITEM9(3); DAM_PIPE_ITEM9(4);
                DAM_PIPE_ITEM9(5); DAM_PIPE_ITEM9(6); DAM_PIPE_ITEM9(7); DAM_PIPE_ITEM9(8);
            } else {
            DAM_PIPE_ITEM(2, ccur, 2, 2, 2, 0);
            DAM_PIPE_ITEM(0, ccur, 3, 0, 3, 1);
            DAM_PIPE_ITEM(1, ccur, 4, 1, 4, 2);
            DAM_PIPE_ITEM(2, ccur, 5, 2, 5, 0);
            DAM_PIPE_ITEM(0, ccur, 6, 0, 6, 1);
            DAM_PIPE_ITEM(1, ccur, 7, 1, 7, 2);
            DAM_PIPE_ITEM(2, ccur, 8, 2, 8, 0);
            DAM_PIPE_ITEM(0, cnext, 0, 0, -1, 1);
            DAM_PIPE_ITEM(1, cnext, 1, 0, -1, 2);
            }
#undef DAM_PIPE_ITEM
#undef DAM_PIPE_ITEM9
            DAM_PSTAMP(0, 6);
            if (KS == 2 && kh == 1 && cg + 1 == nst) {
#pragma unroll
                for (int mb = 0; mb < MB; ++mb)
#pragma unroll
                    for (int nb = 0; nb < NB; ++nb)
                        *reinterpret_cast<v4f*>(smem + part_off + ((mt * MB + mb) * NB + nb) * 1024 + lane * 16) = acc[mb][nb];
            }
            DAM_PIPE_BARRIER();
            DAM_PSTAMP(0, 7);
        }
        if (KS == 2) {
            if (kh == 1) {
                if (!has_next) break;
                unit += G;
                cur = nxt;
                continue;
            }
#pragma unroll
            for (int mb = 0; mb < MB; ++mb)
#pragma unroll
                for (int nb = 0; nb < NB; ++nb)
                    acc[mb][nb] += *reinterpret_cast<const v4f*>(smem + part_off + ((mt * MB + mb) * NB + nb) * 1024 + lane * 16);
        }

        float st_k[NB][4], st_s1[NB][4], st_s2[NB][4];
        float st_n = 0.f;
#pragma unroll
        for (int nb = 0; nb < NB; ++nb)
#pragma unroll
            for (int r = 0; r < 4; ++r) {
                const float first = reinterpret_cast<const float*>(&acc[0][nb])[r] +
                                    (bias ? bias[(cur.nb0 + nb) * 16 + kq * 4 + r] : 0.f);
                st_k[nb][r] = STATS == 1 ? __builtin_bit_cast(float, __builtin_amdgcn_update_dpp(0, __builtin_bit_cast(int, first), 0x150, 0xF, 0xF, false))
                                    : 0.f;
                st_s1[nb][r] = 0.f; st_s2[nb][r] = 0.f;
            }
        v4f bw_ms[STATS == 2 ? NB : 1], bw_mh[STATS == 2 ? NB : 1], bw_k1[STATS == 2 ? NB : 1], bw_k2[STATS == 2 ? NB : 1];
#pragma unroll
        for (int nb = 0; nb < (STATS == 2 ? NB : 0); ++nb) {
            const int ch = (cur.nb0 + nb) * 16 + kq * 4;
            bw_ms[nb] = *reinterpret_cast<const v4f*>(bwd.mscale + ch);
            bw_mh[nb] = *reinterpret_cast<const v4f*>(bwd.mshift + ch);
            bw_k1[nb] = *reinterpret_cast<const v4f*>(bwd.invstd + ch);
            bw_k2[nb] = -(*reinterpret_cast<const v4f*>(bwd.mean + ch)) * bw_k1[nb];
        }
#pragma unroll
        for (int mb = 0; mb < MB; ++mb) {
            const int p = cur.p0 + mt * MW + mb * 16 + j;
            if (p >= HoWo) continue;
            const int oh = fast_div(p, g.Wo, inv_wo), ow = p - oh * g.Wo;
            const size_t opix = ((size_t)cur.img * g.OHt + (oh * g.os + g.oo_h)) * g.OWt + (ow * g.os + g.oo_w);
#pragma unroll
            for (int nb = 0; nb < NB; ++nb) {
                const int ch = (cur.nb0 + nb) * 16 + kq * 4;
                if (ch >= g.N) continue;
                v4f v = acc[mb][nb];
                const size_t o = opix * g.N + ch;
                if (bias) {
                    const float4 bv = *reinterpret_cast<const float4*>(bias + ch);
                    v.x += bv.x; v.y += bv.y; v.z += bv.z; v.w += bv.w;
                }
                if (STATS == 2) {
                    const v4f rv = *reinterpret_cast<const v4f*>(res + o);
                    const v4f m = __builtin_elementwise_fma(rv, bw_ms[nb], bw_mh[nb]);
                    const v4f xh = __builtin_elementwise_fma(rv, bw_k1[nb], bw_k2[nb]);
                    const float dz[4] = {m.x > 0.f ? v.x : 0.f, m.y > 0.f ? v.y : 0.f, m.z > 0.f ? v.z : 0.f, m.w > 0.f ? v.w : 0.f};
                    const float xe[4] = {xh.x, xh.y, xh.z, xh.w};
#pragma unroll
                    for (int r = 0; r < 4; ++r) {
                        st_s1[nb][r] += dz[r];
                        st_s2[nb][r] = fmaf(dz[r], xe[r], st_s2[nb][r]);
                    }
                } else if (res) {
                    const float4 rv = *reinterpret_cast<const float4*>(res + o);
                    if (res_mask) {
                        const float4 mv = *reinterpret_cast<const float4*>(res_mask + o);
                        v.x += mv.x > 0.f ? rv.x : 0.f; v.y += mv.y > 0.f ? rv.y : 0.f;
                        v.z += mv.z > 0.f ? rv.z : 0.f; v.w += mv.w > 0.f ? rv.w : 0.f;
                    } else {
                        v.x += rv.x; v.y += rv.y; v.z += rv.z; v.w += rv.w;
                    }
                }
                if (g.relu_out) { v.x = fmaxf(v.x, 0.f); v.y = fmaxf(v.y, 0.f); v.z = fmaxf(v.z, 0.f); v.w = fmaxf(v.w, 0.f); }
                *reinterpret_cast<float4*>(Y + o) = make_float4(v.x, v.y, v.z, v.w);
                if (STATS == 1) {
                    const float e[4] = {v.x, v.y, v.z, v.w};
#pragma unroll
                    for (int r = 0; r < 4; ++r) {
                        const float d = e[r] - st_k[nb][r];
                        st_s1[nb][r] += d;
                        st_s2[nb][r] = fmaf(d, d, st_s2[nb][r]);
                    }
                }
            }
            if (STATS == 1) st_n += 1.f;
        }
        if (STATS) {
#define DAM_ROW_SUM(V_)                                                                                                     \
    do {                                                                                                                    \
        V_ += __builtin_bit_cast(float, __builtin_amdgcn_update_dpp(0, __builtin_bit_cast(int, V_), 0x128, 0xF, 0xF, false)); \
        V_ += __builtin_bit_cast(float, __builtin_amdgcn_update_dpp(0, __builtin_bit_cast(int, V_), 0x124, 0xF, 0xF, false)); \
        V_ += __builtin_bit_cast(float, __builtin_amdgcn_update_dpp(0, __builtin_bit_cast(int, V_), 0x122, 0xF, 0xF, false)); \
        V_ += __builtin_bit_cast(float, __builtin_amdgcn_update_dpp(0, __builtin_bit_cast(int, V_), 0x121, 0xF, 0xF, false)); \
    } while (0)
            const size_t rec = ((size_t)cur.img * g.tiles_m + (cur.p0 / UPX)) * MT + mt;
            float n = st_n;
            DAM_ROW_SUM(n);
#pragma unroll
            for (int nb = 0; nb < NB; ++nb)
#pragma unroll
                for (int r = 0; r < 4; ++r) {
                    float s1 = st_s1[nb][r], s2 = st_s2[nb][r];
                    DAM_ROW_SUM(s1);
                    DAM_ROW_SUM(s2);
                    const int ch = (cur.nb0 + nb) * 16 + kq * 4 + r;
                    if (STATS == 2) {
                        if (j == 0 && ch < g.N) { float* o = stats + (rec * g.N + ch) * 2; o[0] = s1; o[1] = s2; }
                    } else if (j == 0 && ch < g.N) {
                        const float md = n > 0.f ? s1 / n : 0.f;
                        float* o = stats + (rec * g.N + ch) * 3;
                        o[0] = n; o[1] = st_k[nb][r] + md; o[2] = n > 0.f ? fmaxf(s2 - s1 * md, 0.f) : 0.f;
                    }
                }
#undef DAM_ROW_SUM
        }
        DAM_PSTAMP(0, 8);
        if (!has_next) break;
        unit += G;
        cur = nxt;
    }
#undef DAM_PIPE_W
#undef DAM_PIPE_X
#undef DAM_PIPE_MFMA
}

template <int MB, int NB, int PU, int STATS, int KS>
int pipe_slots(size_t lds) {
    const int cus = device_cus();
    static PerDevice<size_t> cached_lds_pd;
    static PerDevice<int> cached_pd;
    size_t& cached_lds = cached_lds_pd();
    int& cached = cached_pd();
    if (cached_lds != lds || !cached) {
        int per_cu = 0;
        if (hipOccupancyMaxActiveBlocksPerMultiprocessor(&per_cu, reinterpret_cast<const void*>(&conv_pipe_kernel<MB, NB, PU, STATS, KS>), PIPE_THREADS,
                                                         lds) != hipSuccess || per_cu < 1)
            per_cu = 1;
        cached = per_cu * cus;
        cached_lds = lds;
    }
    return cached;
}

template <int MB, int NB, int PU, int KS>
int launch_pipe(const ConvGeo& g, size_t lds, const float* X, const float* Wp, const float* bias, const float* sc, const float* sh,
                float* Y, const float* res, const float* res_mask, float* workspace, float* stats, int* stats_parts,
                const BnBwdEpi& bwd, hipStream_t st) {
    const int nunits = g.tiles_m * (g.N / 16 / NB) * g.B;
    int mode = 0;
    if (stats) {
        const int64_t parts = (int64_t)g.B * g.tiles_m * (4 / KS);
        mode = bwd.x ? 2 : 1;
        if (parts > (bwd.x ? BN_BWD_RECORDS_MAX : BN_RECORDS_MAX)) { stats = nullptr; mode = 0; }
        else if (stats_parts) *stats_parts = (int)parts;
    }
    if (bwd.x) res = mode == 2 ? bwd.x : nullptr;
    int wgs = mode == 2 ? pipe_slots<MB, NB, PU, 2, KS>(lds) : (mode == 1 ? pipe_slots<MB, NB, PU, 1, KS>(lds) : pipe_slots<MB, NB, PU, 0, KS>(lds));
    if (const char* e = getenv("DAM_PIPE_WGS")) wgs = atoi(e);
    if (wgs < 1) wgs = 1;
    if (wgs > nunits) wgs = nunits;
#define DAM_PIPE_LAUNCH(S_)                                                                                                 \
    hipLaunchKernelGGL((conv_pipe_kernel<MB, NB, PU, S_, KS>), dim3((unsigned)wgs), dim3(PIPE_THREADS), lds, st, g, nunits, X,  \
                       reinterpret_cast<const float4*>(Wp), bias, sc, sh, Y, res, res_mask, workspace, stats, bwd)
    if (mode == 2) DAM_PIPE_LAUNCH(2); else if (mode == 1) DAM_PIPE_LAUNCH(1); else DAM_PIPE_LAUNCH(0);
#undef DAM_PIPE_LAUNCH
    DAM_CHECK_LAUNCH();
    conv_last_launch = ConvLaunchNote{CONV_FAM_PIPE, MB, NB, 0, 0, 0, 0, 0, PU, mode, KS, 1, 1};
    return DAM_OK;
}

}

int conv_pipe_try(ConvGeo g, int row_span, const float* X, const float* Wp, const float* bias, const float* sc, const float* sh,
                  float* Y, const float* res, const float* res_mask, float* workspace, float* stats, int* stats_parts,
                  const BnBwdEpi& bwd, hipStream_t st) {
    if (bwd.x && (res || !stats)) return DAM_ERR_BAD_ARG;
    if (g.nA != 3 || g.nB != 3 || g.in_nchw) return DAM_ERR_UNSUPPORTED;
    if ((size_t)g.H * g.W * g.C * 4 >= ((size_t)1 << 30)) return DAM_ERR_UNSUPPORTED;
    const int64_t npix = (int64_t)g.Ho * g.Wo;
    const int nblk = g.N / 16;
    auto patch_rows_px = [&](int px) {
        int rows_out = (int)((px + g.Wo - 2) / g.Wo + 1);
        if (rows_out > g.Ho) rows_out = g.Ho;
        return (rows_out - 1) * g.s + row_span + 1;
    };
    auto patch_rows = [&](int mb) { return patch_rows_px(64 * mb); };
    auto fits = [&](int mb, int nb) {
        const int pr = patch_rows(mb);
        return nblk % nb == 0 && pr * g.PWin * 4 <= PIPE_LT * 8 && (size_t)pr * g.PWT * 64 <= PIPE_BUF1;
    };
    static const int cand[5][2] = {{1, 4}, {2, 2}, {1, 2}, {2, 1}, {1, 1}};
    int MB = 0, NB = 0;
    int64_t most = -1;
    for (int i = 0; i < 5; ++i) {
        const int mb = cand[i][0], nb = cand[i][1];
        if (!fits(mb, nb)) continue;
        const int64_t units = cdiv(npix, 64 * mb) * (nblk / nb) * g.B;
        if (units >= 384) { MB = mb; NB = nb; break; }
        if (units > most) { most = units; MB = mb; NB = nb; }
    }
    if (const char* e = getenv("DAM_TILE")) {
        MB = e[0] - '0'; NB = e[2] - '0';
        if (MB < 1 || NB < 1 || !fits(MB, NB)) return DAM_ERR_UNSUPPORTED;
    }
    if (!MB) return DAM_ERR_UNSUPPORTED;
    int KS = 1;
    if (MB == 1 && NB == 1 && g.nchunks % 2 == 0 && g.nchunks >= 4 && cdiv(npix, 64) * nblk * g.B < 768) {
        const int pr = patch_rows_px(32);
        if (pr * g.PWin * 8 <= PIPE_LT * 3 && (size_t)pr * g.PWT * 128 <= PIPE_BUF1) KS = 2;
    }
    if (const char* e = getenv("DAM_PIPE_KS")) { if (atoi(e) == 1) KS = 1; }
    const int upx = 64 * MB / KS;
    g.PR = patch_rows_px(upx);
    g.tiles_m = (int)cdiv(npix, upx);
    g.CG = 1; g.ksplit = 1; g.gps = g.nchunks;
    const size_t lds = PIPE_BUF1 + (size_t)KS * g.PR * g.PWT * 64 + (sc ? (size_t)2 * g.C * 4 : 0) + PIPE_LT * 16 +
                       (KS == 2 ? (size_t)2 * MB * NB * 1024 : 0);
    const bool big = g.PR * g.PWin * 4 * KS > PIPE_LT * 5;
    if (KS == 2) return launch_pipe<1, 1, 3, 2>(g, lds, X, Wp, bias, sc, sh, Y, res, res_mask, workspace, stats, stats_parts, bwd, st);
#define DAM_PIPE_CASE(M_, N_)                                                                                              \
    if (MB == M_ && NB == N_)                                                                                              \
        return big ? launch_pipe<M_, N_, 8, 1>(g, lds, X, Wp, bias, sc, sh, Y, res, res_mask, workspace, stats, stats_parts, bwd, st) \
                   : launch_pipe<M_, N_, 5, 1>(g, lds, X, Wp, bias, sc, sh, Y, res, res_mask, workspace, stats, stats_parts, bwd, st)
    DAM_PIPE_CASE(1, 4); DAM_PIPE_CASE(2, 2); DAM_PIPE_CASE(1, 2); DAM_PIPE_CASE(2, 1); DAM_PIPE_CASE(1, 1);
#undef DAM_PIPE_CASE
    return DAM_ERR_UNSUPPORTED;
}

}
```

deep-audio-mixer_amd/layers.py:

```python
import torch
import torch.nn as nn

from . import ops


def _slot(p):
    return None if p is None else getattr(p, '_dam_grad', None)


class ConvSpec:

    def __init__(self, cin, cout, k, stride=1, pad=0, dil=1, in_nchw=False):
        self.cin, self.cout, self.k, self.stride, self.pad, self.dil, self.in_nchw = cin, cout, k, stride, pad, dil, in_nchw
        self.wp = self.wpt = None
        self.nhwc16 = None
        if in_nchw and k == 3 and stride == 1 and pad == 1 and dil == 1 and cin <= 16:
            self.nhwc16 = _Nhwc16Spec(self)

    def packed(self, w, transpose=False):
        cached = self.wpt if transpose else self.wp
        return cached if cached is not None else ops.pack_weights(w, transpose=transpose)

    def fwd(self, x, w, bias=None):
        return ops.conv2d_fwd(x, self.packed(w), self.cout, self.k, self.k, self.stride, self.pad, self.dil,
                              bias=bias, in_nchw=self.in_nchw)

    def fwd_conv(self, x, w, bn, training, bias=None, in_affine=None, fuse_stats=True, finalize=True):
        wp = self.packed(w)
        aff = {} if in_affine is None else dict(in_scale=in_affine[0], in_shift=in_affine[1], relu_in=True)
        if training and not self.in_nchw and fuse_stats:
            n16 = (self.cout + 15) // 16 * 16
            buf = ops.bn_partial_buffer(x.device, n16)
            c, parts, out4 = ops.conv2d_fwd(x, wp, self.cout, self.k, self.k, self.stride, self.pad, self.dil, bias=bias,
                                            bn_partial=buf, bn=_bn_args(bn, training), finalize=finalize, **aff)
            if not finalize:
                return c, ((buf, parts) if parts > 0 else None)
            return c, ((out4[0], out4[1], out4[2], out4[3]) if parts > 0 else None)
        return ops.conv2d_fwd(x, wp, self.cout, self.k, self.k, self.stride, self.pad, self.dil, bias=bias,
                              in_nchw=self.in_nchw, **aff), None

    def fwd_bn(self, x, w, bn, training, bias=None, in_affine=None):
        c, stats = self.fwd_conv(x, w, bn, training, bias=bias, in_affine=in_affine)
        return (c,) + tuple(stats if stats is not None else _bn_fwd_stats(c, bn, training))

    def fwd_bn_apply(self, x, w, bn, training, in_affine=None, res=None, res_affine=None, sign_bits=False, bias=None):
        rs, rh = res_affine if res_affine is not None else (None, None)
        if training:
            c, rec = self.fwd_conv(x, w, bn, training, bias=bias, in_affine=in_affine, finalize=False)
            rec = rec if rec is not None else ops.bn_stats_partial(c)
            (m, i, sc, sh), out = ops.bn_finalize_apply(rec[0], rec[1], _bn_args(bn, training), c, relu=True, res=res,
                                                        res_scale=rs, res_shift=rh, sign_bits=sign_bits)
            return c, m, i, sc, sh, out
        c, m, i, sc, sh = self.fwd_bn(x, w, bn, training, bias=bias, in_affine=in_affine)
        return c, m, i, sc, sh, ops.bn_apply(c, sc, sh, relu=True, res=res, res_scale=rs, res_shift=rh, sign_bits=sign_bits)

    def wgrad(self, x, dy, in_affine=None, out=None):
        aff = {} if in_affine is None else dict(in_scale=in_affine[0], in_shift=in_affine[1], relu_in=True)
        return ops.conv2d_wgrad(x, dy, self.cout, self.k, self.k, self.stride, self.pad, self.dil,
                                in_nchw=self.in_nchw, out=out, defer=out is not None, **aff)

    def dgrad(self, dy, w, hw, **kw):
        return ops.conv2d_dgrad(dy, self.packed(w, transpose=True), self.cin, hw[0], hw[1], self.k, self.k,
                                self.stride, self.pad, self.dil, **kw)


class _Nhwc16Spec(ConvSpec):

    def __init__(self, parent):
        self.cin, self.cout, self.k, self.stride, self.pad, self.dil, self.in_nchw = 16, parent.cout, 3, 1, 1, 1, False
        self.parent, self.nhwc16, self.wpt = parent, None, None

    @property
    def wp(self):
        return self.parent.wp

    def packed(self, w, transpose=False):
        return self.parent.packed(w, transpose)

    def wgrad(self, x, dy, in_affine=None, out=None):
        return ops.conv2d_wgrad(x, dy, self.cout, 3, 3, 1, 1, 1, out=out, c_real=self.parent.cin, defer=out is not None)


class WeightPacker:

    def __init__(self, pairs):
        self.pairs = list(pairs)
        self._key = None

    def _build(self):
        rows, dev = [], self.pairs[0][1].device
        L = ops._lib.lib()
        for spec, w, need_t in self.pairs:
            o, i, kh, kw = w.shape
            for transpose in ((False, True) if need_t else (False,)):
                n_out, k_in = (i, o) if transpose else (o, i)
                n = L.dam_conv_packed_weight_count(n_out, k_in, kh, kw)
                buf = torch.empty(n, dtype=torch.float32, device=dev)
                if transpose:
                    spec.wpt = buf
                else:
                    spec.wp = buf
                rows.append([w.data_ptr(), buf.data_ptr(), o, i, kh, kw, int(transpose), n])
        self.desc = torch.tensor(rows, dtype=torch.int64).to(dev)
        self.n, self.max_total = len(rows), max(r[7] for r in rows)

    def pack_all(self):
        key = tuple(w.data_ptr() for _, w, _ in self.pairs)
        if key != self._key:
            self._build()
            self._key = key
        ops.pack_weights_multi(self.desc, self.n, self.max_total)


def _bn_args(bn, training):
    mom = bn.momentum if bn.momentum is not None else 0.1
    track = training and bn.track_running_stats
    return (bn.weight, bn.bias, bn.running_mean if track else None, bn.running_var if track else None,
            bn.num_batches_tracked if track else None, mom, bn.eps)


def _bn_fwd_stats(c, bn, training):
    if training or bn.running_mean is None:
        return ops.bn_stats(c, *_bn_args(bn, training))
    return ops.bn_eval_affine(bn.weight, bn.bias, bn.running_mean, bn.running_var, bn.eps)


def _hw(x, in_nchw):
    return (x.shape[2], x.shape[3]) if in_nchw else (x.shape[1], x.shape[2])


class FoldedConvBn:

    def __init__(self, spec, conv, bn):
        self.spec, self.conv, self.bn = spec, conv, bn
        self._key = self.wp = self.bias = None

    def foldable(self):
        return self.bn.running_mean is not None and self.bn.running_var is not None

    def _tensors(self):
        bn, conv = self.bn, self.conv
        return [t for t in (conv.weight, conv.bias, bn.weight, bn.bias, bn.running_mean, bn.running_var) if t is not None]

    def get(self):
        key = (ops.PARAM_EPOCH,) + tuple((t.data_ptr(), t._version) for t in self._tensors())
        if key != self._key:
            bn, conv = self.bn, self.conv
            with torch.no_grad():
                scale = bn.weight * torch.rsqrt(bn.running_var + bn.eps)
                shift = bn.bias - bn.running_mean * scale
                if conv.bias is not None:
                    shift = shift + conv.bias * scale
                n16 = (self.spec.cout + 15) // 16 * 16
                bias = torch.zeros(n16, dtype=torch.float32, device=scale.device)
                bias[:self.spec.cout] = shift
                self.wp = ops.pack_weights(conv.weight * scale.view(-1, 1, 1, 1))
                self.bias = bias
            self._key = key
        return self.wp, self.bias

    def fwd(self, x, res=None, relu=True):
        wp, bias = self.get()
        sp = self.spec
        if sp.nhwc16 is not None:
            sp, x = sp.nhwc16, ops.nchw_to_nhwc16(x)
        return ops.conv2d_fwd(x, wp, sp.cout, sp.k, sp.k, sp.stride, sp.pad, sp.dil, bias=bias, in_nchw=sp.in_nchw,
                              res=res, relu_out=relu)


def inference_mode(module):
    return not module.training and not torch.is_grad_enabled()


UNIT_SEED = '_dam_unit_seed'


class _UpstreamBn:
    __slots__ = ('c', 'mean', 'invstd', 'scale', 'shift', 'bits', 'partials', 'dx_ptr', 'dx_version')

    def __init__(self, c, mean, invstd, scale, shift, bits=None):
        self.c, self.mean, self.invstd, self.scale, self.shift, self.bits = c, mean, invstd, scale, shift, bits
        self.partials, self.dx_ptr, self.dx_version = None, None, None

    def request(self):
        return (self.c, self.mean, self.invstd, self.scale, self.shift) + ((self.bits,) if self.bits is not None else ())

    def offer(self, sums, dx):
        self.partials, self.dx_ptr, self.dx_version = sums, dx.data_ptr(), dx._version

    def take(self, grad):
        ok = self.partials is not None and self.dx_ptr == grad.data_ptr() and self.dx_version == grad._version
        sums = self.partials if ok else None
        self.partials = None
        if sums is not None:
            _UpstreamBn.hits += 1
        return sums

    hits = 0


class ConvBnReluFn(torch.autograd.Function):

    @staticmethod
    def forward(ctx, x, w, bias, gamma, beta, spec, bn, training):
        if spec.nhwc16 is not None and not ctx.needs_input_grad[0]:
            spec, x = spec.nhwc16, ops.nchw_to_nhwc16(x)
        c, mean, invstd, scale, shift, a = spec.fwd_bn_apply(x, w.detach(), bn, training,
                                                             bias=None if bias is None else bias.detach())
        ctx.save_for_backward(x, w, c, gamma, mean, invstd, scale, shift)
        ctx.up = a._dam_upstream = _UpstreamBn(c, mean, invstd, scale, shift) if ops.DGRAD_BN_SUMS else None
        ctx.spec, ctx.training, ctx.has_bias = spec, training, bias is not None
        ctx.slots = (_slot(w), _slot(bias), _slot(gamma), _slot(beta))
        return a

    @staticmethod
    def backward(ctx, da):
        x, w, c, gamma, mean, invstd, scale, shift = ctx.saved_tensors
        spec = ctx.spec
        sw, sb, sg, sbt = ctx.slots
        da = da.contiguous()
        sums = ctx.up.take(da) if ctx.up is not None else None
        dc, dgamma, dbeta = ops.bn_backward(da, None, c, gamma, mean, invstd, ctx.training,
                                            mask_affine=(scale, shift), dgamma=sg, dbeta=sbt, partials=sums)
        dw = spec.wgrad(x, dc, out=None if sw is None else sw.view(w.shape))
        dbias = ops.channel_sum(dc, spec.cout, out=sb) if ctx.has_bias else None
        dx = spec.dgrad(dc, w, _hw(x, spec.in_nchw)) if ctx.needs_input_grad[0] else None
        return (dx, None if sw is not None else dw, None if sb is not None else dbias, None if sg is not None else dgamma,
                None if sbt is not None else dbeta, None, None, None)


class DropoutFn(torch.autograd.Function):

    @staticmethod
    def forward(ctx, x, p):
        ops.dropout_check(x.numel(), p)
        snap = ops.dropout_tick(x.device, x.numel())
        ctx.p, ctx.seed = p, torch.initial_seed()
        ctx.save_for_backward(snap)
        return ops.dropout_apply(x, p, ctx.seed, snap)

    @staticmethod
    def backward(ctx, dy):
        (snap,) = ctx.saved_tensors
        return ops.dropout_apply(dy, ctx.p, ctx.seed, snap), None


class BasicBlockFn(torch.autograd.Function):

    @staticmethod
    def forward(ctx, x, w1, g1, b1, w2, g2, b2, wsc, gsc, bsc, blk, training):
        if wsc is not None:
            bn_sc = blk.shortcut[1]
            one = None
            if (training and blk.spec1.k == 3 and blk.spec1.stride == 2 and blk.spec1.pad == 1
                    and blk.spec1.dil == 1 and blk.spec_sc.k == 1 and blk.spec_sc.stride == 2 and blk.spec_sc.pad == 0
                    and not blk.spec1.in_nchw):
                one = ops.conv_s2_pair_fwd(x, blk.spec1.packed(w1.detach()), blk.spec_sc.packed(wsc.detach()), blk.spec1.cout)
            if one is not None:
                c1, cs, (p1, p2, parts) = one
                st1, sts = ops.bn_finalize_pair(p1, p2, parts, _bn_args(blk.bn1, True), _bn_args(bn_sc, True))
            else:
                c1, st1 = blk.spec1.fwd_conv(x, w1.detach(), blk.bn1, training, fuse_stats=False)
                cs, sts = blk.spec_sc.fwd_conv(x, wsc.detach(), bn_sc, training, fuse_stats=False)
            if st1 is None and sts is None and training and c1.shape == cs.shape:
                st1, sts = ops.bn_stats_pair(c1, _bn_args(blk.bn1, True), cs, _bn_args(bn_sc, True))
            m1, i1, sc1, sh1 = st1 if st1 is not None else _bn_fwd_stats(c1, blk.bn1, training)
            ms, is_, scs, shs = sts if sts is not None else _bn_fwd_stats(cs, bn_sc, training)
            c2, m2, i2, sc2, sh2, (out, bits) = blk.spec2.fwd_bn_apply(c1, w2.detach(), blk.bn2, training, in_affine=(sc1, sh1),
                                                                       res=cs, res_affine=(scs, shs), sign_bits=True)
            ctx.save_for_backward(x, w1, g1, w2, g2, c1, c2, out, m1, i1, m2, i2, sc1, sh1, bits, wsc, gsc, cs, ms, is_)
        else:
            c1, m1, i1, sc1, sh1 = blk.spec1.fwd_bn(x, w1.detach(), blk.bn1, training)
            c2, m2, i2, sc2, sh2, (out, bits) = blk.spec2.fwd_bn_apply(c1, w2.detach(), blk.bn2, training, in_affine=(sc1, sh1),
                                                                       res=x, sign_bits=True)
            ctx.save_for_backward(x, w1, g1, w2, g2, c1, c2, out, m1, i1, m2, i2, sc1, sh1, bits)
        ctx.up_self = None
        if wsc is None and ops.DGRAD_BN_SUMS:
            ctx.up_self = out._dam_upstream = _UpstreamBn(c2, m2, i2, None, None, bits)
        ctx.blk, ctx.training, ctx.has_sc = blk, training, wsc is not None
        ctx.upstream = getattr(x, '_dam_upstream', None)
        if wsc is not None and (ctx.upstream is None or ctx.upstream.bits is None or ctx.upstream.scale is not None):
            ctx.upstream = None
        ctx.slots = tuple(_slot(p) for p in (w1, g1, b1, w2, g2, b2, wsc, gsc, bsc))
        return out

    @staticmethod
    def backward(ctx, dout):
        blk, tr = ctx.blk, ctx.training
        if ctx.has_sc:
            x, w1, g1, w2, g2, c1, c2, out, m1, i1, m2, i2, sc1, sh1, bits, wsc, gsc, cs, ms, is_ = ctx.saved_tensors
        else:
            x, w1, g1, w2, g2, c1, c2, out, m1, i1, m2, i2, sc1, sh1, bits = ctx.saved_tensors
        dout = dout.contiguous()
        hw = (x.shape[1], x.shape[2])
        s_w1, s_g1, s_b1, s_w2, s_g2, s_b2, s_ws, s_gs, s_bs = ctx.slots
        keep = lambda grad, slot: None if slot is not None else grad
        wview = lambda slot, w: None if slot is None else slot.view(w.shape)
        if ctx.has_sc:
            (dc2, dg2, db2), (dcs, dgs, dbs) = ops.bn_backward_pair(dout, None, (c2, g2, m2, i2, s_g2, s_b2),
                                                                    (cs, gsc, ms, is_, s_gs, s_bs), tr, mask_bits=bits)
        else:
            sums2 = ctx.up_self.take(dout) if ctx.up_self is not None else None
            dc2, dg2, db2 = ops.bn_backward(dout, None, c2, g2, m2, i2, tr, dgamma=s_g2, dbeta=s_b2, mask_bits=bits, partials=sums2)
        dw2 = blk.spec2.wgrad(c1, dc2, in_affine=(sc1, sh1), out=wview(s_w2, w2))
        sums = None
        if ops.DGRAD_BN_SUMS:
            da1, sums = blk.spec2.dgrad(dc2, w2, (c1.shape[1], c1.shape[2]), bn_bwd=(c1, m1, i1, sc1, sh1))
        else:
            da1 = blk.spec2.dgrad(dc2, w2, (c1.shape[1], c1.shape[2]))
        dc1, dg1, db1 = ops.bn_backward(da1, None, c1, g1, m1, i1, tr, mask_affine=(sc1, sh1),
                                        dgamma=s_g1, dbeta=s_b1, partials=sums)
        dw1 = blk.spec1.wgrad(x, dc1, out=wview(s_w1, w1))
        first = (keep(dw1, s_w1), keep(dg1, s_g1), keep(db1, s_b1), keep(dw2, s_w2), keep(dg2, s_g2), keep(db2, s_b2))
        if ctx.has_sc:
            dws = blk.spec_sc.wgrad(x, dcs, out=wview(s_ws, wsc))
            if (blk.spec1.k == 3 and blk.spec1.stride == 2 and blk.spec1.pad == 1 and blk.spec1.dil == 1
                    and blk.spec_sc.k == 1 and blk.spec_sc.stride == 2 and blk.spec_sc.pad == 0):
                up = ctx.upstream
                pair = (dcs, blk.spec_sc.packed(wsc, transpose=True))
                if up is not None and ops.DGRAD_BN_SUMS and ops.DGRAD_S2 and up.c.shape == x.shape:
                    dx, sums = blk.spec1.dgrad(dc1, w1, hw, pair_1x1=pair, bn_bwd=up.request())
                    if sums is not None:
                        up.offer(sums, dx)
                else:
                    dx = blk.spec1.dgrad(dc1, w1, hw, pair_1x1=pair)
            else:
                dx = blk.spec1.dgrad(dc1, w1, hw)
                blk.spec_sc.dgrad(dcs, wsc, hw, accumulate_into=dx)
            return (dx,) + first + (keep(dws, s_ws), keep(dgs, s_gs), keep(dbs, s_bs), None, None)
        up = ctx.upstream
        if up is not None and ops.DGRAD_BN_SUMS and up.c.shape == x.shape:
            dx, sums = blk.spec1.dgrad(dc1, w1, hw, res=dout, res_mask=out, res_mask_bits=bits, bn_bwd=up.request())
            up.offer(sums, dx)
        else:
            dx = blk.spec1.dgrad(dc1, w1, hw, res=dout, res_mask=out)
        return (dx,) + first + (None, None, None, None, None)


class HeadsFn(torch.autograd.Function):

    @staticmethod
    def forward(ctx, trunk, x, cw, cb, fw, fb):
        h, g = ops.heads_fwd(trunk, cw.detach(), cb.detach(), fw.detach(), fb.detach())
        masked = ops.masksum_fwd(x, g)
        ctx.save_for_backward(trunk, x, h, cw, fw)
        ctx.set_materialize_grads(False)
        ctx.slots = (_slot(cw), _slot(cb), _slot(fw), _slot(fb))
        return masked, g

    @staticmethod
    def backward(ctx, dmasked, dg_out):
        trunk, x, h, cw, fw = ctx.saved_tensors
        dg = None
        if dmasked is not None:
            dg = ops.masksum_bwd(dmasked.contiguous(), x)
        if dg_out is not None:
            dg = dg_out.contiguous() if dg is None else dg + dg_out
        if dg is None:
            return None, None, None, None, None, None
        dtrunk, dcw, dcb, dfw, dfb = ops.heads_bwd(dg, h, trunk, cw, fw, outs=ctx.slots)
        sl = ctx.slots
        return (dtrunk, None, None if sl[0] is not None else dcw, None if sl[1] is not None else dcb,
                None if sl[2] is not None else dfw, None if sl[3] is not None else dfb)


class HeadsMseFn(torch.autograd.Function):

    @staticmethod
    def forward(ctx, trunk, x, gt, cw, cb, fw, fb):
        h, g = ops.heads_fwd(trunk, cw.detach(), cb.detach(), fw.detach(), fb.detach())
        masked, loss, dg = ops.masksum_mse(x, g, gt.contiguous())
        ctx.save_for_backward(trunk, h, cw, fw, dg)
        ctx.mark_non_differentiable(masked, g)
        ctx.set_materialize_grads(False)
        ctx.slots = (_slot(cw), _slot(cb), _slot(fw), _slot(fb))
        return loss.reshape(()), masked, g

    @staticmethod
    def backward(ctx, dloss, _dm, _dg):
        trunk, h, cw, fw, dg = ctx.saved_tensors
        if dloss is None:
            dloss = torch.zeros((), dtype=torch.float32, device=dg.device)
        seed = dg if getattr(dloss, UNIT_SEED, False) else dg * dloss
        dtrunk, dcw, dcb, dfw, dfb = ops.heads_bwd(seed, h, trunk, cw, fw, outs=ctx.slots)
        sl = ctx.slots
        return (dtrunk, None, None, None if sl[0] is not None else dcw, None if sl[1] is not None else dcb,
                None if sl[2] is not None else dfw, None if sl[3] is not None else dfb)


class BasicBlock(nn.Module):
    expansion = 1

    def __init__(self, in_channels, out_channels, stride=1):
        super().__init__()
        self.conv1 = nn.Conv2d(in_channels, out_channels, kernel_size=3, stride=stride, padding=1, bias=False)
        self.bn1 = nn.BatchNorm2d(out_channels)
        self.conv2 = nn.Conv2d(out_channels, out_channels, kernel_size=3, stride=1, padding=1, bias=False)
        self.bn2 = nn.BatchNorm2d(out_channels)
        self.shortcut = nn.Sequential()
        if stride != 1 or in_channels != self.expansion * out_channels:
            self.shortcut = nn.Sequential(
                nn.Conv2d(in_channels, self.expansion * out_channels, kernel_size=1, stride=stride, bias=False),
                nn.BatchNorm2d(self.expansion * out_channels))
        self.spec1 = ConvSpec(in_channels, out_channels, 3, stride, 1)
        self.spec2 = ConvSpec(out_channels, out_channels, 3, 1, 1)
        self.spec_sc = ConvSpec(in_channels, out_channels, 1, stride, 0) if len(self.shortcut) else None

    def _folded(self):
        f = getattr(self, '_fold', None)
        if f is None:
            f = self._fold = (FoldedConvBn(self.spec1, self.conv1, self.bn1), FoldedConvBn(self.spec2, self.conv2, self.bn2),
                              FoldedConvBn(self.spec_sc, self.shortcut[0], self.shortcut[1]) if self.spec_sc is not None else None)
        return f

    def forward(self, x):
        if inference_mode(self):
            f1, f2, fs = self._folded()
            if f1.foldable() and f2.foldable() and (fs is None or fs.foldable()):
                a1 = f1.fwd(x)
                return f2.fwd(a1, res=x if fs is None else fs.fwd(x, relu=False))
        if self.spec_sc is not None:
            sc, sbn = self.shortcut[0], self.shortcut[1]
            return BasicBlockFn.apply(x, self.conv1.weight, self.bn1.weight, self.bn1.bias, self.conv2.weight,
                                      self.bn2.weight, self.bn2.bias, sc.weight, sbn.weight, sbn.bias, self, self.training)
        return BasicBlockFn.apply(x, self.conv1.weight, self.bn1.weight, self.bn1.bias, self.conv2.weight,
                                  self.bn2.weight, self.bn2.bias, None, None, None, self, self.training)


class ConvBlock2d(nn.Module):

    def __init__(self, in_channels, out_channels, kernel_size, stride=1, dilation=1, dropout_p=-1.0, in_nchw=False):
        super().__init__()
        self.add_padding = None
        self.conv = nn.Conv2d(in_channels=in_channels, out_channels=out_channels, kernel_size=kernel_size,
                              stride=stride, padding=0, dilation=dilation)
        self.batch_norm = nn.BatchNorm2d(num_features=out_channels, momentum=0.90, eps=0.001)
        self.activation = nn.ReLU()
        self.dropout = nn.Dropout(dropout_p) if dropout_p != -1 else None
        self.spec = ConvSpec(in_channels, out_channels, kernel_size, stride, 0, dilation, in_nchw=in_nchw)

    def forward(self, x):
        if inference_mode(self):
            f = getattr(self, '_fold', None)
            if f is None:
                f = self._fold = FoldedConvBn(self.spec, self.conv, self.batch_norm)
            if f.foldable():
                return f.fwd(x)
        out = ConvBnReluFn.apply(x, self.conv.weight, self.conv.bias, self.batch_norm.weight, self.batch_norm.bias,
                                 self.spec, self.batch_norm, self.training)
        if self.training and self.dropout:
            out = DropoutFn.apply(out, self.dropout.p) if self.dropout.p > 0 else out
        return out


class GainHeads(nn.Module):

    def __init__(self, channels, n_stems, flattened_dim):
        super().__init__()
        self.n_stems, self.channels, self.flattened_dim = n_stems, channels, flattened_dim
        cw, cb, fw, fb = [], [], [], []
        for _ in range(n_stems):
            conv, fc = nn.Conv2d(channels, 1, kernel_size=(1, 1)), nn.Linear(flattened_dim, 1)
            cw.append(conv.weight.detach().view(1, channels)), cb.append(conv.bias.detach())
            fw.append(fc.weight.detach()), fb.append(fc.bias.detach())
        self.conv_w, self.conv_b = nn.Parameter(torch.cat(cw)), nn.Parameter(torch.cat(cb))
        self.fc_w, self.fc_b = nn.Parameter(torch.cat(fw)), nn.Parameter(torch.cat(fb))

    def reference_items(self):
        for i in range(self.n_stems):
            yield 'conv_head%d.weight' % (i + 1), self.conv_w[i].view(1, self.channels, 1, 1)
            yield 'conv_head%d.bias' % (i + 1), self.conv_b[i:i + 1]
            yield 'fc_head%d.weight' % (i + 1), self.fc_w[i:i + 1]
            yield 'fc_head%d.bias' % (i + 1), self.fc_b[i:i + 1]

    def forward(self, trunk, x):
        return HeadsFn.apply(trunk, x, self.conv_w, self.conv_b, self.fc_w, self.fc_b)

    def forward_mse(self, trunk, x, gt):
        return HeadsMseFn.apply(trunk, x, gt, self.conv_w, self.conv_b, self.fc_w, self.fc_b)


class MixingNet(nn.Module):

    def _init_heads(self, channels, n_stems, flattened_dim):
        self._heads = GainHeads(channels, n_stems, flattened_dim)
        self.n_stems = n_stems
        self._register_state_dict_hook(MixingNet._sd_hook)
        self._register_load_state_dict_pre_hook(self._load_hook)

    @staticmethod
    def _sd_hook(module, state_dict, prefix, local_metadata):
        for k in ('conv_w', 'conv_b', 'fc_w', 'fc_b'):
            state_dict.pop(prefix + '_heads.' + k, None)
        for name, view in module._heads.reference_items():
            state_dict[prefix + name] = view.detach()
        return state_dict

    def _load_hook(self, state_dict, prefix, local_metadata, strict, missing_keys, unexpected_keys, error_msgs):
        h = self._heads
        parts = {}
        for i in range(h.n_stems):
            for kind in ('conv_head%d.weight', 'conv_head%d.bias', 'fc_head%d.weight', 'fc_head%d.bias'):
                key = prefix + kind % (i + 1)
                if key in state_dict:
                    parts.setdefault(kind, []).append(state_dict.pop(key))
        if not parts:
            return
        if any(len(v) != h.n_stems for v in parts.values()) or len(parts) != 4:
            error_msgs.append('incomplete per-stem head parameters in state_dict')
            return
        dev = h.conv_w.device
        state_dict[prefix + '_heads.conv_w'] = torch.cat([t.reshape(1, h.channels) for t in parts['conv_head%d.weight']]).to(dev)
        state_dict[prefix + '_heads.conv_b'] = torch.cat([t.reshape(1) for t in parts['conv_head%d.bias']]).to(dev)
        state_dict[prefix + '_heads.fc_w'] = torch.cat([t.reshape(1, -1) for t in parts['fc_head%d.weight']]).to(dev)
        state_dict[prefix + '_heads.fc_b'] = torch.cat([t.reshape(1) for t in parts['fc_head%d.bias']]).to(dev)

    def trunk(self, x, tap=None):
        raise NotImplementedError

    def ddp_late_parameters(self):
        raise NotImplementedError

    @staticmethod
    def _check_input(x):
        if x.dim() != 4:
            raise ValueError('expected x of shape [B, S, F, T]')
        if not x.is_cuda:
            raise RuntimeError('deep_audio_mixer_amd models run on the GPU only (got a %s tensor); there is no CPU '
                               'fallback' % x.device)
        if x.dtype != torch.float32:
            raise RuntimeError('expected scalar type Float but found %s' % str(x.dtype).replace('torch.', '').capitalize())
        return x.contiguous()

    @staticmethod
    def _refuse_input_grad(x):
        if x.requires_grad and torch.is_grad_enabled():
            raise RuntimeError('input gradients are not supported: x requires grad (detach it, or run under torch.no_grad())')

    def conv_pairs(self):
        return []

    def _pack_weights(self):
        if self.training:
            ops.params_changed()
        if getattr(self, '_packer', None) is None:
            pairs = self.conv_pairs()
            self._packer = WeightPacker(pairs) if pairs else False
        if self._packer:
            self._packer.pack_all()

    def forward(self, x):
        x = self._check_input(x)
        self._refuse_input_grad(x)
        self._pack_weights()
        masked, g = self._heads(self.trunk(x), x)
        return masked, tuple(g[:, s:s + 1] for s in range(self.n_stems))

    def predict_gains(self, x):
        x = self._check_input(x)
        self._pack_weights()
        with torch.no_grad():
            h = self._heads
            return ops.heads_fwd(self.trunk(x), h.conv_w, h.conv_b, h.fc_w, h.fc_b)[1]

    def forward_mse(self, x, gt, tap=None):
        x = self._check_input(x)
        self._refuse_input_grad(x)
        self._pack_weights()
        loss, masked, g = self._heads.forward_mse(self.trunk(x) if tap is None else self.trunk(x, tap), x, gt)
        return loss, masked, tuple(g[:, s:s + 1] for s in range(self.n_stems))
```

deep-audio-mixer_amd/ops.py:

```python
import collections
import ctypes
import numbers
import os

import torch

from . import _lib


def _f32c(t, name):
    if t is None:
        return None
    if t.dtype != torch.float32 or not t.is_contiguous():
        raise ValueError('%s must be a contiguous float32 tensor' % name)
    return t


def conv_out_size(n, k, stride=1, pad=0, dil=1):
    return (n + 2 * pad - dil * (k - 1) - 1) // stride + 1


def pack_weights(w, transpose=False, out=None):
    _lib.require_cuda(w)
    w = _f32c(w.detach(), 'weight')
    o, i, kh, kw = w.shape
    n_out, k_in = (i, o) if transpose else (o, i)
    n = _lib.lib().dam_conv_packed_weight_count(n_out, k_in, kh, kw)
    if out is None:
        out = torch.empty(n, dtype=torch.float32, device=w.device)
    _lib.check(_lib.lib().dam_conv_pack_weights_f32(_lib.ptr(w), o, i, kh, kw, 1 if transpose else 0,
                                                    _lib.ptr(out), _lib.stream()), 'dam_conv_pack_weights_f32')
    return out


def pack_weights_multi(desc, n_tensors, max_total):
    _lib.check(_lib.lib().dam_conv_pack_weights_multi_f32(_lib.ptr(desc), n_tensors, max_total, _lib.stream()),
               'dam_conv_pack_weights_multi_f32')


DGRAD_S2 = not os.environ.get('DAM_NO_DGRAD_S2')
dgrad_s2_launches = 0
DGRAD_BN_SUMS = not os.environ.get('DAM_NO_DGRAD_SUMS')


def _bn_fin_struct(bn, out4):
    gamma, beta, rm, rv, nbt, mom, eps = bn
    return _lib.BnFin(_lib.ptr(gamma), _lib.ptr(beta), _lib.ptr(rm), _lib.ptr(rv), _lib.ptr(nbt), float(mom), float(eps),
                      _lib.ptr(out4[0]), _lib.ptr(out4[1]), _lib.ptr(out4[2]), _lib.ptr(out4[3]))


def _tapgrid(x, B, H, W, C, in_nchw, wp, k_chunks, n_out, bias, in_scale, in_shift, relu_in, y, OHt, OWt, Ho, Wo,
             out_stride, oo_h, oo_w, in_stride, nA, nB, off_h, step_h, off_w, step_w, wt_base, wt_sa, wt_sb,
             res=None, res_mask=None, bn_partial=None, relu_out=False, batch=None, bn_bwd=None):
    parts = ctypes.c_int(0)
    ws = _workspace(y.device, min(8 * y.numel(), 8 * 400 * 64 * 64))
    st = _lib.lib().dam_conv2d_tapgrid_f32(
        _lib.ptr(x), B, H, W, C, 1 if in_nchw else 0, _lib.ptr(wp), k_chunks, n_out, _lib.ptr(bias),
        _lib.ptr(in_scale), _lib.ptr(in_shift), 1 if relu_in else 0, 1 if relu_out else 0, _lib.ptr(y), OHt, OWt, Ho, Wo,
        out_stride,
        oo_h, oo_w, in_stride, nA, nB, off_h, step_h, off_w, step_w, wt_base, wt_sa, wt_sb, _lib.ptr(res),
        _lib.ptr(res_mask), _lib.ptr(bn_partial), ctypes.byref(parts) if bn_partial is not None else None,
        ctypes.byref(bn_bwd) if bn_bwd is not None else None,
        _lib.ptr(ws), ws.numel(),
        ctypes.addressof(batch) if batch is not None else None, _lib.stream())
    _lib.check(st, 'dam_conv2d_tapgrid_f32')
    return parts.value


def conv2d_fwd(x, wp, n_out, kh, kw, stride=1, pad=0, dil=1, bias=None, in_scale=None, in_shift=None,
               relu_in=False, in_nchw=False, bn_partial=None, bn=None, res=None, relu_out=False, finalize=True, out=None):
    _lib.require_cuda(x, wp)
    _f32c(x, 'x'), _f32c(bias, 'bias'), _f32c(in_scale, 'in_scale'), _f32c(in_shift, 'in_shift'), _f32c(res, 'res')
    if in_nchw:
        B, C, H, W = x.shape
        k_chunks = 1
    else:
        B, H, W, C = x.shape
        k_chunks = C // 16
    n16 = (n_out + 15) // 16 * 16
    Ho, Wo = conv_out_size(H, kh, stride, pad, dil), conv_out_size(W, kw, stride, pad, dil)
    if Ho <= 0 or Wo <= 0:
        raise ValueError('convolution output would be empty')
    if out is None:
        y = torch.empty((B, Ho, Wo, n16), dtype=torch.float32, device=x.device)
    else:
        if out.dtype != torch.float32 or not out.is_contiguous() or tuple(out.shape) != (B, Ho, Wo, n16) or out.device != x.device:
            raise ValueError('out must be a contiguous float32 tensor of shape %s on %s' % ((B, Ho, Wo, n16), x.device))
        y = out
    parts = _tapgrid(x, B, H, W, C, in_nchw, wp, k_chunks, n16, bias, in_scale, in_shift, relu_in, y, Ho, Wo, Ho, Wo,
                     1, 0, 0, stride, kh, kw, -pad, dil, -pad, dil, 0, kw, 1, res=res, bn_partial=bn_partial,
                     relu_out=relu_out)
    if bn is not None and bn_partial is not None:
        out4 = bn_finalize(bn_partial, parts, *bn) if parts > 0 and finalize else None
        return y, parts, out4
    if bn_partial is not None:
        return y, parts
    return y


CONV_FAMILIES = ('none', 'strip', 'pipe', 'pipe_ranges', 'tile', 'tile_batch', '1x1')
ConvLaunch = collections.namedtuple('ConvLaunch', 'family MB NB NCH T33 LW EPI SO PU STATS KS ksplit ranges')


def conv_last_launch():
    v = (ctypes.c_int * 16)()
    _lib.check(_lib.lib().dam_conv_last_launch(v), 'dam_conv_last_launch')
    return ConvLaunch(CONV_FAMILIES[v[0]], *v[1:13])


def _dgrad_axis(parity, pad, dil, k, stride):
    valid = [t for t in range(k) if (parity + pad - t * dil) % stride == 0]
    if not valid:
        return None
    k0 = valid[0]
    kstep = valid[1] - valid[0] if len(valid) > 1 else 1
    return len(valid), k0, kstep, (parity + pad - k0 * dil) // stride, -(kstep * dil) // stride


def conv2d_dgrad(dy, wpt, n_in, H, W, kh, kw, stride=1, pad=0, dil=1, res=None, res_mask=None, accumulate_into=None,
                 bn_bwd=None, res_mask_bits=None, pair_1x1=None, _s2_sums=None):
    _lib.require_cuda(dy, wpt)
    if bn_bwd is not None and stride == 2:
        if accumulate_into is not None or res is not None or len(bn_bwd) < 6 or bn_bwd[5] is None or bn_bwd[3] is not None:
            raise ValueError('bn_bwd at stride 2: mask as sign bytes, no residual / accumulation')
        xb, mean, invstd, up_bits = bn_bwd[0], bn_bwd[1], bn_bwd[2], bn_bwd[5]
        _lib.require_cuda(xb)
        n16 = (n_in + 15) // 16 * 16
        if tuple(xb.shape) != (dy.shape[0], H, W, n16):
            raise ValueError('bn_bwd: x has the shape of the data gradient')
        rec = torch.empty(_lib.lib().dam_bn_workspace_floats(n16), dtype=torch.float32, device=dy.device)
        epi = _lib.BnBwdSums(_lib.ptr(xb), _lib.ptr(mean), _lib.ptr(invstd), None, None, None, _lib.ptr(up_bits))
        got = conv2d_dgrad(dy, wpt, n_in, H, W, kh, kw, stride, pad, dil, pair_1x1=pair_1x1, _s2_sums=(epi, rec))
        return got if isinstance(got, tuple) else (got, None)
    if bn_bwd is not None:
        if stride != 1 or accumulate_into is not None:
            raise ValueError('bn_bwd: stride-1 data gradients only')
        if res is not None and (res_mask is None or res_mask_bits is None):
            raise ValueError('bn_bwd with a residual: res_mask and res_mask_bits')
        _f32c(dy, 'dy'), _f32c(res, 'res'), _f32c(res_mask, 'res_mask')
        xb, mean, invstd, msc, msh = bn_bwd[:5]
        up_bits = bn_bwd[5] if len(bn_bwd) > 5 else None
        if (up_bits is None) == (msc is None) or (up_bits is not None and res is None):
            raise ValueError('bn_bwd: the mask as (scale, shift) or -- with a residual -- as sign bytes')
        _lib.require_cuda(xb)
        B, Ho, Wo, Co = dy.shape
        n16 = (n_in + 15) // 16 * 16
        if tuple(xb.shape) != (B, H, W, n16):
            raise ValueError('bn_bwd: x has the shape of the data gradient')
        dx = torch.empty((B, H, W, n16), dtype=torch.float32, device=dy.device)
        rec = torch.empty(_lib.lib().dam_bn_workspace_floats(n16), dtype=torch.float32, device=dy.device)
        epi = _lib.BnBwdSums(_lib.ptr(xb), _lib.ptr(mean), _lib.ptr(invstd), _lib.ptr(msc), _lib.ptr(msh), _lib.ptr(res_mask_bits),
                             _lib.ptr(up_bits))
        parts = _tapgrid(dy, B, Ho, Wo, Co, False, wpt, Co // 16, n16, None, None, None, False, dx, H, W, H, W, 1, 0, 0, 1,
                         kh, kw, pad, -dil, pad, -dil, 0, kw, 1, res, res_mask, bn_partial=rec, bn_bwd=epi)
        return dx, ((rec, parts) if parts > 0 else None)
    _f32c(dy, 'dy'), _f32c(res, 'res'), _f32c(res_mask, 'res_mask')
    B, Ho, Wo, Co = dy.shape
    n16 = (n_in + 15) // 16 * 16
    if accumulate_into is not None:
        dx, res, res_mask = accumulate_into, accumulate_into, None
    else:
        dx = torch.empty((B, H, W, n16), dtype=torch.float32, device=dy.device)
    if stride == 1:
        _tapgrid(dy, B, Ho, Wo, Co, False, wpt, Co // 16, n16, None, None, None, False, dx, H, W, H, W, 1, 0, 0, 1,
                 kh, kw, pad, -dil, pad, -dil, 0, kw, 1, res, res_mask)
        return dx
    if pair_1x1 is not None:
        dy2, wpt2 = pair_1x1
        _lib.require_cuda(dy2, wpt2)
        _f32c(dy2, 'pair dy')
        if accumulate_into is not None or res is not None or tuple(dy2.shape) != tuple(dy.shape):
            raise ValueError('pair_1x1: a second gradient of the same shape, no residual / accumulation')
        a0 = _dgrad_axis(0, pad, dil, kh, stride), _dgrad_axis(0, pad, dil, kw, stride)
        if a0[0] is None or a0[1] is None or a0[0][0] != 1 or a0[1][0] != 1 or a0[0][3] != 0 or a0[1][3] != 0:
            raise ValueError('pair_1x1: class (0, 0) of this operator is not a single tap at offset 0')
    if (DGRAD_S2 and stride == 2 and kh == 3 and kw == 3 and pad == 1 and dil == 1 and accumulate_into is None and res is None
            and Ho == (H + 1) // 2 and Wo == (W + 1) // 2):
        parts = ctypes.c_int(0)
        st = _lib.lib().dam_dgrad_s2_3x3_f32(_lib.ptr(dy), _lib.ptr(wpt), _lib.ptr(pair_1x1[0]) if pair_1x1 else None,
                                             _lib.ptr(pair_1x1[1]) if pair_1x1 else None, B, Ho, Wo, Co, n16, _lib.ptr(dx), H, W,
                                             ctypes.byref(_s2_sums[0]) if _s2_sums else None,
                                             _lib.ptr(_s2_sums[1]) if _s2_sums else None, ctypes.byref(parts) if _s2_sums else None,
                                             _lib.stream())
        if st == 0:
            global dgrad_s2_launches
            dgrad_s2_launches += 1
            if _s2_sums:
                return dx, ((_s2_sums[1], parts.value) if parts.value > 0 else None)
            return dx
        if st != -2:
            _lib.check(st, 'dam_dgrad_s2_3x3_f32')
    classes = [(_dgrad_axis(ph, pad, dil, kh, stride), _dgrad_axis(pw, pad, dil, kw, stride))
               for ph in range(stride) for pw in range(stride)]
    if any(a is None or b is None for a, b in classes) and accumulate_into is None:
        if res is not None:
            raise ValueError('a fused residual needs every output parity class to receive taps')
        dx.zero_()
    batch = _conv_batch(dy.device)
    try:
        for ph in range(stride):
            for pw in range(stride):
                ah, aw = _dgrad_axis(ph, pad, dil, kh, stride), _dgrad_axis(pw, pad, dil, kw, stride)
                nh, nw = (H - ph + stride - 1) // stride, (W - pw + stride - 1) // stride
                if nh <= 0 or nw <= 0 or ah is None or aw is None:
                    continue
                if pair_1x1 is not None and ph == 0 and pw == 0:
                    if nh != Ho or nw != Wo:
                        raise ValueError('pair_1x1: class (0, 0) does not cover the gradient\'s pixels')
                    _lib.check(_lib.lib().dam_conv1x1_pair_f32(_lib.ptr(dy), _lib.ptr(wpt), ah[1] * kw + aw[1], _lib.ptr(pair_1x1[0]),
                                                               _lib.ptr(pair_1x1[1]), 0, B, Ho, Wo, Co, n16, _lib.ptr(dx), H, W, stride,
                                                               0, 0, _lib.stream()), 'dam_conv1x1_pair_f32')
                    continue
                _tapgrid(dy, B, Ho, Wo, Co, False, wpt, Co // 16, n16, None, None, None, False, dx, H, W, nh, nw,
                         stride, ph, pw, 1, ah[0], aw[0], ah[3], ah[4], aw[3], aw[4], ah[1] * kw + aw[1],
                         ah[2] * kw, aw[2], res, res_mask, batch=batch)
        _lib.check(_lib.lib().dam_conv_batch_flush(ctypes.addressof(batch), _lib.stream()), 'dam_conv_batch_flush')
    except Exception:
        _lib.lib().dam_conv_batch_init(ctypes.addressof(batch))
        raise
    return dx


_conv_batches = {}


def _conv_batch(device):
    key = (device.type, device.index)
    b = _conv_batches.get(key)
    if b is None:
        L = _lib.lib()
        b = _conv_batches[key] = ctypes.create_string_buffer(int(L.dam_conv_batch_bytes()))
        _lib.check(L.dam_conv_batch_init(ctypes.addressof(b)), 'dam_conv_batch_init')
    return b


_workspaces = {}
_retired = []


def _grow(table, key, device, floats):
    ws = table.get(key)
    if ws is None or ws.numel() < floats:
        if ws is not None:
            _retired.append(ws)
        ws = torch.empty(int(floats), dtype=torch.float32, device=device)
        table[key] = ws
    return ws


def _workspace(device, floats):
    return _grow(_workspaces, (device.type, device.index), device, floats)


PARAM_EPOCH = 0


def params_changed():
    global PARAM_EPOCH
    PARAM_EPOCH += 1


WGRAD_BATCH = True
_wgrad_queues = {}


def _wgrad_queue(device):
    key = (device.type, device.index)
    q = _wgrad_queues.get(key)
    if q is None:
        L = _lib.lib()
        buf = ctypes.create_string_buffer(int(L.dam_wgrad_queue_bytes()))
        _lib.check(L.dam_wgrad_queue_init(ctypes.addressof(buf)), 'dam_wgrad_queue_init')
        _lib.check(L.dam_wgrad_queue_set_batching(ctypes.addressof(buf), int(WGRAD_BATCH)), 'dam_wgrad_queue_set_batching')
        q = _wgrad_queues[key] = [buf, 0, []]
    return q


def wgrad_abandon(device=None):
    for key, q in _wgrad_queues.items():
        if q[1] and (device is None or key == (device.type, device.index)):
            _lib.check(_lib.lib().dam_wgrad_queue_init(ctypes.addressof(q[0])), 'dam_wgrad_queue_init')
            del q[2][:]
            q[1] = 0


def wgrad_flush(device=None):
    for key, q in _wgrad_queues.items():
        if q[1] and (device is None or key == (device.type, device.index)):
            _lib.check(_lib.lib().dam_wgrad_queue_flush(ctypes.addressof(q[0]), _lib.stream()), 'dam_wgrad_queue_flush')
            q[1] = 0
            del q[2][:]


def conv2d_wgrad(x, dy, n_out, kh, kw, stride=1, pad=0, dil=1, in_scale=None, in_shift=None, relu_in=False,
                 in_nchw=False, out=None, c_real=None, defer=False):
    _lib.require_cuda(x, dy)
    _f32c(x, 'x'), _f32c(dy, 'dy')
    if in_nchw:
        B, C, H, W = x.shape
    else:
        B, H, W, C = x.shape
    _, Ho, Wo, n_chan = dy.shape
    L = _lib.lib()
    floats = L.dam_conv2d_wgrad_workspace_floats(n_out, C, kh, kw)
    cr = C if c_real is None else int(c_real)
    if out is None:
        if defer:
            raise ValueError('a deferred weight gradient needs the buffer it will be written to')
        out = torch.empty((n_out, cr, kh, kw), dtype=torch.float32, device=x.device)
    elif out.numel() != n_out * cr * kh * kw or not out.is_contiguous() or out.dtype != torch.float32:
        raise ValueError('bad out tensor for the weight gradient')
    if defer:
        q = _wgrad_queue(x.device)
        ws = _grow(_workspaces, (x.device.type, x.device.index, 'wgrad slabs', q[1]), x.device, floats)
        q[1] += 1
        q[2].append((x, dy, in_scale, in_shift))
        queue = ctypes.addressof(q[0])
    else:
        ws, queue = _workspace(x.device, floats), None
    _lib.check(L.dam_conv2d_wgrad_f32(_lib.ptr(x), B, H, W, C, 1 if in_nchw else 0, _lib.ptr(in_scale),
                                      _lib.ptr(in_shift), 1 if relu_in else 0, _lib.ptr(dy), Ho, Wo, n_chan, n_out,
                                      kh, kw, stride, pad, dil, _lib.ptr(out), cr, _lib.ptr(ws), ws.numel(), queue,
                                      _lib.stream()), 'dam_conv2d_wgrad_f32')
    return out


WGRAD_FAMILIES = ('none', 'rows', 'rows_s2', 'direct', 'tile')
WgradLaunch = collections.namedtuple('WgradLaunch', 'family TNB TKB STEPS KP GPP GPPD HV NL TA TB nx nsplit spi rps TMW issued')


def wgrad_last_launch():
    v = (ctypes.c_int * 16)()
    _lib.check(_lib.lib().dam_wgrad_last_launch(v), 'dam_wgrad_last_launch')
    fam = WGRAD_FAMILIES[v[0]]
    rows = fam in ('rows', 'rows_s2')
    return WgradLaunch(fam, *v[1:13], v[13] if rows else 0, v[14] if rows else 0, v[13] if fam == 'tile' else 0, v[15])


def nchw_to_nhwc16(x):
    _lib.require_cuda(x)
    _f32c(x, 'x')
    B, C, H, W = x.shape
    y = torch.empty((B, H, W, 16), dtype=torch.float32, device=x.device)
    _lib.check(_lib.lib().dam_nchw_to_nhwc16_f32(_lib.ptr(x), B, C, H * W, _lib.ptr(y), _lib.stream()), 'dam_nchw_to_nhwc16_f32')
    return y


def _bn_ws(device, C):
    return _workspace(device, _lib.lib().dam_bn_workspace_floats(C))


_bn_partials = {}


def bn_stats(x, gamma, beta, running_mean, running_var, num_batches_tracked, momentum, eps):
    _lib.require_cuda(x)
    C = x.shape[-1]
    P = x.numel() // C
    out = torch.empty((4, C), dtype=torch.float32, device=x.device)
    ws = _bn_ws(x.device, C)
    _lib.check(_lib.lib().dam_bn_stats_f32(_lib.ptr(x), P, C, _lib.ptr(gamma), _lib.ptr(beta), _lib.ptr(running_mean),
                                           _lib.ptr(running_var), _lib.ptr(num_batches_tracked), float(momentum), float(eps),
                                           _lib.ptr(out[0]), _lib.ptr(out[1]), _lib.ptr(out[2]), _lib.ptr(out[3]),
                                           _lib.ptr(ws), _lib.stream()), 'dam_bn_stats_f32')
    return out[0], out[1], out[2], out[3]


def bn_stats_partial(x):
    _lib.require_cuda(x)
    C = x.shape[-1]
    ws = bn_partial_buffer(x.device, C)
    parts = ctypes.c_int(0)
    _lib.check(_lib.lib().dam_bn_stats_partial_f32(_lib.ptr(x), x.numel() // C, C, _lib.ptr(ws), ctypes.byref(parts), _lib.stream()),
               'dam_bn_stats_partial_f32')
    return ws, parts.value


def bn_finalize_apply(partial, parts, bn, x, relu=True, res=None, res_scale=None, res_shift=None, sign_bits=False):
    _lib.require_cuda(partial, x)
    C = x.shape[-1]
    out4 = torch.empty((4, C), dtype=torch.float32, device=x.device)
    fin = _bn_fin_struct(bn, out4)
    y = torch.empty_like(x)
    bits = torch.empty(x.shape[:-1] + (C // 4,), dtype=torch.uint8, device=x.device) if sign_bits else None
    _lib.check(_lib.lib().dam_bn_finalize_apply_f32(_lib.ptr(partial), int(parts), C, ctypes.byref(fin), _lib.ptr(x), x.numel() // C,
                                                    _lib.ptr(res), _lib.ptr(res_scale), _lib.ptr(res_shift), 1 if relu else 0,
                                                    _lib.ptr(y), _lib.ptr(bits), _lib.stream()), 'dam_bn_finalize_apply_f32')
    return (out4[0], out4[1], out4[2], out4[3]), ((y, bits) if sign_bits else y)


def bn_partial_buffer(device, C):
    return _grow(_bn_partials, (device.type, device.index, C), device, _lib.lib().dam_bn_workspace_floats(C))


def bn_stats_pair(xa, bn_a, xb, bn_b):
    _lib.require_cuda(xa, xb)
    if xa.shape != xb.shape:
        raise ValueError('the two tensors of a pair have the same shape')
    C = xa.shape[-1]
    L = _lib.lib()
    outs = [torch.empty((4, C), dtype=torch.float32, device=xa.device) for _ in range(2)]
    fa, fb = _bn_fin_struct(bn_a, outs[0]), _bn_fin_struct(bn_b, outs[1])
    ws = _workspace(xa.device, 2 * L.dam_bn_workspace_floats(C))
    _lib.check(L.dam_bn_stats_pair_f32(_lib.ptr(xa), _lib.ptr(xb), xa.numel() // C, C, ctypes.byref(fa), ctypes.byref(fb),
                                       _lib.ptr(ws), _lib.stream()), 'dam_bn_stats_pair_f32')
    return tuple(outs[0]), tuple(outs[1])


def conv_s2_pair_fwd(x, wp, wp_sc, n_out, stats=True):
    _lib.require_cuda(x, wp, wp_sc)
    _f32c(x, 'x')
    B, H, W, C = x.shape
    n16 = (n_out + 15) // 16 * 16
    Hd, Wd = (H + 1) // 2, (W + 1) // 2
    c1 = torch.empty((B, Hd, Wd, n16), dtype=torch.float32, device=x.device)
    cs = torch.empty_like(c1)
    p1 = p2 = None
    parts = ctypes.c_int(0)
    if stats:
        n = _lib.lib().dam_bn_workspace_floats(n16)
        p1 = torch.empty(n, dtype=torch.float32, device=x.device)
        p2 = torch.empty(n, dtype=torch.float32, device=x.device)
    st = _lib.lib().dam_conv_s2_pair_fwd_f32(_lib.ptr(x), _lib.ptr(wp), _lib.ptr(wp_sc), B, H, W, C, n16, _lib.ptr(c1), _lib.ptr(cs),
                                             _lib.ptr(p1), _lib.ptr(p2), ctypes.byref(parts), _lib.stream())
    if st == -2:
        return None
    _lib.check(st, 'dam_conv_s2_pair_fwd_f32')
    return c1, cs, ((p1, p2, parts.value) if stats else None)


def bn_finalize_pair(partial_a, partial_b, parts, bn_a, bn_b):
    C = bn_a[0].numel()
    outs = [torch.empty((4, C), dtype=torch.float32, device=partial_a.device) for _ in range(2)]
    fa, fb = _bn_fin_struct(bn_a, outs[0]), _bn_fin_struct(bn_b, outs[1])
    _lib.check(_lib.lib().dam_bn_finalize_pair_f32(_lib.ptr(partial_a), _lib.ptr(partial_b), parts, C, ctypes.byref(fa),
                                                   ctypes.byref(fb), _lib.stream()), 'dam_bn_finalize_pair_f32')
    return tuple(outs[0]), tuple(outs[1])


def bn_finalize(partial, parts, gamma, beta, running_mean, running_var, num_batches_tracked, momentum, eps):
    C = gamma.numel()
    out = torch.empty((4, C), dtype=torch.float32, device=gamma.device)
    _lib.check(_lib.lib().dam_bn_finalize_f32(_lib.ptr(partial), parts, C, _lib.ptr(gamma), _lib.ptr(beta),
                                              _lib.ptr(running_mean), _lib.ptr(running_var), _lib.ptr(num_batches_tracked),
                                              float(momentum), float(eps), _lib.ptr(out[0]), _lib.ptr(out[1]), _lib.ptr(out[2]),
                                              _lib.ptr(out[3]), _lib.stream()), 'dam_bn_finalize_f32')
    return out[0], out[1], out[2], out[3]


def bn_eval_affine(gamma, beta, running_mean, running_var, eps):
    _lib.require_cuda(gamma)
    C = gamma.numel()
    out = torch.empty((4, C), dtype=torch.float32, device=gamma.device)
    _lib.check(_lib.lib().dam_bn_eval_affine_f32(C, _lib.ptr(gamma), _lib.ptr(beta), _lib.ptr(running_mean),
                                                 _lib.ptr(running_var), float(eps), _lib.ptr(out[0]), _lib.ptr(out[1]),
                                                 _lib.ptr(out[2]), _lib.ptr(out[3]), _lib.stream()), 'dam_bn_eval_affine_f32')
    return out[0], out[1], out[2], out[3]


def bn_apply(x, scale, shift, relu=True, res=None, res_scale=None, res_shift=None, sign_bits=False):
    _lib.require_cuda(x)
    C = x.shape[-1]
    y = torch.empty_like(x)
    bits = torch.empty(x.shape[:-1] + (C // 4,), dtype=torch.uint8, device=x.device) if sign_bits else None
    _lib.check(_lib.lib().dam_bn_apply_f32(_lib.ptr(x), x.numel() // C, C, _lib.ptr(scale), _lib.ptr(shift), _lib.ptr(res),
                                           _lib.ptr(res_scale), _lib.ptr(res_shift), 1 if relu else 0, _lib.ptr(y),
                                           _lib.ptr(bits), _lib.stream()), 'dam_bn_apply_f32')
    return (y, bits) if sign_bits else y


def bn_backward_pair(dy, y_mask, a, b, training=True, mask_bits=None):
    _lib.require_cuda(dy, a[0], b[0])
    if (y_mask is None) == (mask_bits is None):
        raise ValueError('exactly one of y_mask / mask_bits')
    C = a[0].shape[-1]
    if b[0].shape != a[0].shape or dy.shape != a[0].shape:
        raise ValueError('the two BatchNorms of a pair see the same shape')
    outs = []
    for x, gamma, mean, invstd, dgamma, dbeta in (a, b):
        dx = torch.empty_like(x)
        dgamma = torch.empty(C, dtype=torch.float32, device=x.device) if dgamma is None else dgamma
        dbeta = torch.empty(C, dtype=torch.float32, device=x.device) if dbeta is None else dbeta
        outs.append((dx, dgamma, dbeta))
    L = _lib.lib()
    ws = _workspace(dy.device, L.dam_bn_pair_workspace_floats(C))
    args = []
    for (x, gamma, mean, invstd, _, _), (dx, dgamma, dbeta) in zip((a, b), outs):
        args += [_lib.ptr(x), _lib.ptr(gamma), _lib.ptr(mean), _lib.ptr(invstd), _lib.ptr(dx), _lib.ptr(dgamma), _lib.ptr(dbeta)]
    _lib.check(L.dam_bn_backward_pair_f32(_lib.ptr(dy), _lib.ptr(y_mask), _lib.ptr(mask_bits), dy.numel() // C, C,
                                          1 if training else 0, *args,
                                          _lib.ptr(ws), _lib.stream()), 'dam_bn_backward_pair_f32')
    return outs[0], outs[1]


def bn_backward(dy, y_mask, x, gamma, save_mean, save_invstd, training=True, mask_affine=None, dgamma=None, dbeta=None,
                mask_bits=None, partials=None):
    _lib.require_cuda(dy, x)
    C = x.shape[-1]
    dx = torch.empty_like(x)
    if dgamma is None:
        dgamma = torch.empty(C, dtype=torch.float32, device=x.device)
    if dbeta is None:
        dbeta = torch.empty(C, dtype=torch.float32, device=x.device)
    ws, given = (_bn_ws(x.device, C), 0) if partials is None else partials
    _lib.check(_lib.lib().dam_bn_backward_f32(_lib.ptr(dy), _lib.ptr(y_mask), _lib.ptr(x), x.numel() // C, C, _lib.ptr(gamma),
                                              _lib.ptr(save_mean), _lib.ptr(save_invstd), 1 if training else 0,
                                              _lib.ptr(mask_affine[0]) if mask_affine else None,
                                              _lib.ptr(mask_affine[1]) if mask_affine else None, _lib.ptr(mask_bits), _lib.ptr(dx),
                                              _lib.ptr(dgamma), _lib.ptr(dbeta), _lib.ptr(ws), given, _lib.stream()),
               'dam_bn_backward_f32')
    return dx, dgamma, dbeta


def channel_sum(x, n_real, out=None):
    _lib.require_cuda(x)
    C = x.shape[-1]
    if out is None:
        out = torch.empty(n_real, dtype=torch.float32, device=x.device)
    ws = _bn_ws(x.device, C)
    _lib.check(_lib.lib().dam_channel_sum_f32(_lib.ptr(x), x.numel() // C, C, n_real, _lib.ptr(out), _lib.ptr(ws),
                                              _lib.stream()), 'dam_channel_sum_f32')
    return out


def heads_fwd(trunk, conv_w, conv_b, fc_w, fc_b):
    _lib.require_cuda(trunk)
    B, C = trunk.shape[0], trunk.shape[-1]
    P = trunk.numel() // (B * C)
    S = conv_w.shape[0]
    if fc_w.shape != (S, P):
        raise ValueError('fc_head expects %d inputs but the trunk gives %d (flattened_dim mismatch)' % (fc_w.shape[1], P))
    h = torch.empty((B, S, P), dtype=torch.float32, device=trunk.device)
    g = torch.empty((B, S), dtype=torch.float32, device=trunk.device)
    _lib.check(_lib.lib().dam_heads_fwd_f32(_lib.ptr(trunk), B, P, C, S, _lib.ptr(conv_w), _lib.ptr(conv_b), _lib.ptr(fc_w),
                                            _lib.ptr(fc_b), _lib.ptr(h), _lib.ptr(g), _lib.stream()), 'dam_heads_fwd_f32')
    return h, g


def heads_bwd(dgains, h, trunk, conv_w, fc_w, outs=None):
    B, S, P = h.shape
    C = trunk.shape[-1]
    dev = trunk.device
    dtrunk = torch.empty_like(trunk)
    o = outs or (None, None, None, None)
    dcw = o[0] if o[0] is not None else torch.empty((S, C), dtype=torch.float32, device=dev)
    dcb = o[1] if o[1] is not None else torch.empty(S, dtype=torch.float32, device=dev)
    dfw = o[2] if o[2] is not None else torch.empty((S, P), dtype=torch.float32, device=dev)
    dfb = o[3] if o[3] is not None else torch.empty(S, dtype=torch.float32, device=dev)
    L = _lib.lib()
    ws = _workspace(dev, L.dam_heads_bwd_workspace_floats(B, P, C, S))
    _lib.check(L.dam_heads_bwd_f32(_lib.ptr(dgains), _lib.ptr(h), _lib.ptr(trunk), B, P, C, S, _lib.ptr(conv_w), _lib.ptr(fc_w),
                                   _lib.ptr(dtrunk), _lib.ptr(dcw), _lib.ptr(dcb), _lib.ptr(dfw), _lib.ptr(dfb), _lib.ptr(ws),
                                   _lib.stream()), 'dam_heads_bwd_f32')
    return dtrunk, dcw, dcb, dfw, dfb


def masksum_fwd(x, gains):
    _lib.require_cuda(x, gains)
    B, S, F, T = x.shape
    masked = torch.empty((B, F, T), dtype=torch.float32, device=x.device)
    _lib.check(_lib.lib().dam_masksum_fwd_f32(_lib.ptr(x), _lib.ptr(gains), B, S, F * T, _lib.ptr(masked), _lib.stream()),
               'dam_masksum_fwd_f32')
    return masked


def masksum_bwd(dmasked, x):
    B, S, F, T = x.shape
    dg = torch.empty((B, S), dtype=torch.float32, device=x.device)
    L = _lib.lib()
    ws = _workspace(x.device, L.dam_masksum_workspace_floats(B, S))
    _lib.check(L.dam_masksum_bwd_f32(_lib.ptr(dmasked), _lib.ptr(x), B, S, F * T, _lib.ptr(dg), _lib.ptr(ws), _lib.stream()),
               'dam_masksum_bwd_f32')
    return dg


def masksum_mse(x, gains, gt, want_masked=True):
    _lib.require_cuda(x, gains, gt)
    B, S, F, T = x.shape
    dev = x.device
    masked = torch.empty((B, F, T), dtype=torch.float32, device=dev) if want_masked else None
    loss = torch.empty(1, dtype=torch.float32, device=dev)
    dg = torch.empty((B, S), dtype=torch.float32, device=dev)
    L = _lib.lib()
    ws = _workspace(dev, L.dam_masksum_workspace_floats(B, S))
    _lib.check(L.dam_masksum_mse_f32(_lib.ptr(x), _lib.ptr(gains), _lib.ptr(gt), B, S, F * T, _lib.ptr(masked), _lib.ptr(loss),
                                     _lib.ptr(dg), _lib.ptr(ws), _lib.stream()), 'dam_masksum_mse_f32')
    return masked, loss, dg


def adam_l2_step(params, grads, exp_avg, exp_avg_sq, step, derived, lr, beta1, beta2, eps, weight_decay, grad_scale=1.0,
                 hyper=None):
    _lib.require_cuda(params, grads, hyper)
    _lib.check(_lib.lib().dam_adam_l2_step_f32(_lib.ptr(params), _lib.ptr(grads), _lib.ptr(exp_avg), _lib.ptr(exp_avg_sq),
                                               params.numel(), _lib.ptr(step), _lib.ptr(derived), float(lr), float(beta1),
                                               float(beta2), float(eps), float(weight_decay), float(grad_scale),
                                               _lib.ptr(hyper), _lib.stream()), 'dam_adam_l2_step_f32')


def digest64(t, out=None, index_base=0, accumulate=False, max_blocks=0):
    _lib.require_cuda(t, out)
    if t.element_size() != 4 or not t.is_contiguous():
        raise ValueError('digest64: a contiguous tensor of 4-byte elements expected (got %s, contiguous=%s)'
                         % (t.dtype, t.is_contiguous()))
    if out is None:
        out = torch.empty(1, dtype=torch.int64, device=t.device)
    elif out.dtype != torch.int64 or out.numel() != 1 or not out.is_contiguous():
        raise ValueError('digest64: out must be a contiguous int64 tensor of one element')
    _lib.check(_lib.lib().dam_digest64_u32(_lib.ptr(t) if t.numel() else None, t.numel(), int(index_base), int(max_blocks),
                                           int(bool(accumulate)), _lib.ptr(out), _lib.stream()), 'dam_digest64_u32')
    return out


def _audio_kind(t, what):
    if t.dtype not in (torch.float32, torch.float64):
        raise TypeError('%s must be float32 or float64' % what)
    return 1 if t.dtype == torch.float64 else 0


def gain_ramp_arg(gains, N, n):
    if gains is None:
        return None, 0
    if gains.dtype != torch.float64:
        raise TypeError('gains must be float64')
    gains = gains.reshape(N, -1).contiguous()
    if not 1 <= gains.shape[1] <= n:
        raise ValueError('between one gain and one gain per sample expected')
    return gains, gains.shape[1]


def gains_smooth(raw_db, window, polyorder=2, out=None, want_f32=False):
    _lib.require_cuda(raw_db, out)
    raw_db = _f32c(raw_db, 'raw_db')
    n, S = raw_db.shape
    if window % 2 == 0 or window <= polyorder or window > n:
        raise ValueError('savgol_filter needs an odd window with polyorder < window <= len(x): window=%d polyorder=%d '
                         'len=%d' % (window, polyorder, n))
    if out is None:
        out = torch.empty((2, S, n), dtype=torch.float64, device=raw_db.device)
    elif tuple(out.shape) != (2, S, n) or out.dtype != torch.float64 or not out.is_contiguous():
        raise ValueError('bad out tensor')
    s32 = torch.empty((S, n), dtype=torch.float32, device=raw_db.device) if want_f32 else None
    _lib.check(_lib.lib().dam_gains_smooth(_lib.ptr(raw_db), n, S, window, polyorder, _lib.ptr(out[0]), _lib.ptr(out[1]),
                                           _lib.ptr(s32), _lib.stream()), 'dam_gains_smooth')
    return (out[0], out[1], s32) if want_f32 else (out[0], out[1])


def gain_ramp_apply(audio, gains, out=None, out_dtype=None):
    _lib.require_cuda(audio, gains, out)
    ak = _audio_kind(audio, 'audio')
    if gains.dtype != torch.float64:
        raise TypeError('gains must be float64')
    audio, gains = audio.contiguous(), gains.contiguous()
    if audio.dim() == 2:
        rpg, rows, n = audio.shape[0], audio.shape[0], audio.shape[1]
        n_gains = gains.numel()
    else:
        G, rpg, n = audio.shape
        rows, n_gains = G * rpg, gains.shape[-1]
        if gains.numel() != G * n_gains:
            raise ValueError('one gain sequence per leading index expected')
    if out is None:
        out = torch.empty(audio.shape, dtype=out_dtype or torch.float64, device=audio.device)
    elif out.shape != audio.shape or not out.is_contiguous():
        raise ValueError('bad out tensor')
    _lib.check(_lib.lib().dam_gain_ramp_apply(_lib.ptr(audio), ak, _lib.ptr(gains), rows, rpg, n, n_gains, _lib.ptr(out),
                                              _audio_kind(out, 'out'), _lib.stream()), 'dam_gain_ramp_apply')
    return out


def mixdown_peak_normalize(audio, gains, normalize=True, out=None, out_dtype=None, workspace=None):
    _lib.require_cuda(audio, gains, out)
    ak = _audio_kind(audio, 'audio')
    if gains.dtype != torch.float64:
        raise TypeError('gains must be float64')
    audio, gains = audio.contiguous(), gains.contiguous()
    S, rows, n = audio.shape
    if out is None:
        out = torch.empty((rows, n), dtype=out_dtype or torch.float64, device=audio.device)
    L = _lib.lib()
    if workspace is None:
        workspace = torch.empty(L.dam_mixdown_workspace_elems(rows), dtype=out.dtype, device=audio.device)
    _lib.check(L.dam_mixdown_peak_normalize(_lib.ptr(audio), ak, _lib.ptr(gains), S, rows, n, gains.shape[1],
                                            1 if normalize else 0, _lib.ptr(out), _audio_kind(out, 'out'),
                                            _lib.ptr(workspace), _lib.stream()), 'dam_mixdown_peak_normalize')
    return out


PCM_FORMATS = {'PCM_16': (0, 2), 'PCM_24': (1, 3), 'PCM_32': (2, 4), 'FLOAT': (3, 4)}
PCM_MAX_CHANNELS = 8


def pcm_grid_frames(dtype):
    L = _lib.lib()
    return L.dam_pcm_tile_frames(1 if dtype in (torch.float64, 'float64') else 0) * L.dam_pcm_max_blocks()


def pcm_encode(x, subtype, scale=None, dither_seed=None, out=None, clip_count=None):
    _lib.require_cuda(x, scale, out, clip_count)
    if subtype not in PCM_FORMATS:
        raise ValueError('pcm_encode: subtype must be one of %s, got %r' % (sorted(PCM_FORMATS), subtype))
    fmt, width = PCM_FORMATS[subtype]
    xk = _audio_kind(x, 'x')
    if x.dim() == 1:
        x = x.unsqueeze(0)
    if x.dim() != 2 or not x.is_contiguous():
        raise ValueError('pcm_encode: a contiguous [channels, n] tensor expected (got shape %s, contiguous=%s)'
                         % (tuple(x.shape), x.is_contiguous()))
    ch, n = x.shape
    if not 1 <= ch <= PCM_MAX_CHANNELS or n < 1:
        raise ValueError('pcm_encode: 1..%d channels and at least one frame expected, got [%d, %d]' % (PCM_MAX_CHANNELS, ch, n))
    n_scale = 0
    if scale is not None:
        if scale.dtype != torch.float64 or not scale.is_contiguous() or scale.numel() not in (1, ch):
            raise ValueError('pcm_encode: scale must be a contiguous float64 tensor of 1 or %d elements' % ch)
        n_scale = scale.numel()
    if out is None:
        out = torch.empty(n * ch * width, dtype=torch.uint8, device=x.device)
    elif out.dtype != torch.uint8 or out.numel() != n * ch * width or not out.is_contiguous():
        raise ValueError('pcm_encode: out must be a contiguous uint8 tensor of %d elements' % (n * ch * width))
    if clip_count is not None and (clip_count.dtype != torch.int64 or clip_count.numel() != ch or not clip_count.is_contiguous()):
        raise ValueError('pcm_encode: clip_count must be a contiguous int64 tensor of %d elements' % ch)
    seed = 0 if dither_seed is None else int(dither_seed) & 0xFFFFFFFFFFFFFFFF
    _lib.check(_lib.lib().dam_pcm_encode(_lib.ptr(x), xk, ch, n, _lib.ptr(scale), n_scale, fmt,
                                         0 if dither_seed is None else 1, seed, _lib.ptr(out), _lib.ptr(clip_count),
                                         _lib.stream()), 'dam_pcm_encode')
    return out


def true_peak_geometry():
    L = _lib.lib()
    return L.dam_true_peak_tile_samples(), L.dam_true_peak_max_blocks()


def true_peak_batch(data, gains=None, out=None, sample_peak_out=None):
    _lib.require_cuda(data, gains, out, sample_peak_out)
    xk = _audio_kind(data, 'data')
    if data.dim() != 3:
        raise ValueError('true_peak_batch: [tracks, samples, channels] expected, got shape %s' % (tuple(data.shape),))
    N, n, ch = data.shape
    if N < 1 or n < 1 or ch < 1 or N * ch > 65535:
        raise ValueError('true_peak_batch: at least one track, sample and channel and at most 65535 rows expected, got %s'
                         % (tuple(data.shape),))
    gains, n_gains = gain_ramp_arg(gains, N, n)
    dev = data.device
    if out is None:
        out = torch.empty((N, ch), dtype=torch.float64, device=dev)
    for o in (out, sample_peak_out):
        if o is not None and (tuple(o.shape) != (N, ch) or o.dtype != torch.float64 or not o.is_contiguous()):
            raise ValueError('true_peak_batch: outputs must be contiguous float64 [%d, %d] tensors' % (N, ch))
    L = _lib.lib()
    ws = torch.empty(L.dam_true_peak_workspace_bytes(N, n, ch) // 8, dtype=torch.float64, device=dev)
    with torch.cuda.device(dev):
        _lib.check(L.dam_true_peak_batch(_lib.ptr(data), xk, N, n, ch, data.stride(0), data.stride(1), data.stride(2),
                                         _lib.ptr(gains), n_gains, _lib.ptr(sample_peak_out), _lib.ptr(out), _lib.ptr(ws),
                                         _lib.stream()), 'dam_true_peak_batch')
    return out


def peak_limit_gains(gains, peaks, ceiling_db):
    _lib.require_cuda(gains, peaks)
    if gains.dtype != torch.float64 or peaks.dtype != torch.float64 or not gains.is_contiguous():
        raise TypeError('peak_limit_gains: a contiguous float64 gains tensor and float64 peaks expected')
    G = gains.numel()
    if G < 1 or peaks.numel() < G or peaks.numel() % G:
        raise ValueError('peak_limit_gains: %d peaks do not divide among %d gains' % (peaks.numel(), G))
    peaks = peaks.contiguous()
    with torch.cuda.device(gains.device):
        _lib.check(_lib.lib().dam_peak_limit_gains(_lib.ptr(gains), _lib.ptr(peaks), G, peaks.numel() // G,
                                                   float(10.0 ** (float(ceiling_db) / 20.0)), _lib.stream()),
                   'dam_peak_limit_gains')
    return gains


def limiter_geometry():
    L = _lib.lib()
    return L.dam_limiter_tile_samples(), L.dam_limiter_max_lookahead(), L.dam_limiter_max_hold()


def limiter_samples(ms, sr):
    return max(1, int(float(ms) * sr / 1000.0 + 0.5))


def limiter_apply(data, ceiling_db, lookahead, hold, pre_gain=None, out=None, out_dtype=None, min_gain_out=None,
                  n_limited_out=None, workspace=None):
    _lib.require_cuda(data, pre_gain, out, min_gain_out, n_limited_out, workspace)
    xk = _audio_kind(data, 'data')
    if data.dim() != 3:
        raise ValueError('limiter_apply: [row sets, samples, channels] expected, got shape %s' % (tuple(data.shape),))
    N, n, ch = data.shape
    if N < 1 or n < 1 or ch < 1 or N > 65535:
        raise ValueError('limiter_apply: 1..65535 row sets and at least one sample and channel expected, got %s'
                         % (tuple(data.shape),))
    L = _lib.lib()
    lookahead, hold = int(lookahead), int(hold)
# ... 273 lines not shown
```

include/dam_hip.h:

```cpp
#ifndef DAM_HIP_H
#define DAM_HIP_H

#include <stdint.h>

#ifdef __cplusplus
extern "C" {
#endif

typedef enum dam_status {
    DAM_OK = 0,
    DAM_ERR_BAD_ARG = -1,
    DAM_ERR_UNSUPPORTED = -2,
    DAM_ERR_LAUNCH = -3,
    DAM_ERR_WORKSPACE = -4
} dam_status;

typedef enum dam_pcm_dtype { DAM_PCM_F32 = 0, DAM_PCM_F64 = 1, DAM_PCM_S16 = 2, DAM_PCM_S32 = 3 } dam_pcm_dtype;
#define DAM_PCM_INDIRECT 0x100
#define DAM_PCM_ROTATE 0x200
struct dam_bn_bwd_sums;

#define DAM_ABI_VERSION 27
const char* dam_arch(void);
int dam_abi_version(void);

int dam_host_dontfork_pinned(int64_t* n_mappings_host, int64_t* n_bytes_host);

int dam_step_mark_create(void** mark_host);
int dam_step_mark_record(void* mark, void* stream);
int dam_step_mark_wait(void* mark, void* stream);
int dam_step_mark_synchronize(void* mark);
int dam_step_mark_destroy(void* mark);


int64_t dam_stft_twiddle_count(int n_fft);
int dam_stft_fill_twiddles_host(int n_fft, float* table_host );

int dam_stft_logmag_f32(const void* pcm, int pcm_dtype, int64_t n_tracks, int64_t n_samples, int channels,
                        int64_t pcm_track_stride, const float* window, const float* twiddles,
                        const float* gain, int n_fft, int hop, float amin, int normalize,
                        float* out, void* stream);

int dam_stft_logmag_strided_f32(const void* pcm, int pcm_dtype, int64_t n_outer, int64_t outer_stride, int64_t n_inner,
                                int64_t inner_stride, int64_t n_samples, int channels, int64_t sample_stride,
                                int64_t channel_stride, const float* window, const float* twiddles, const float* gain,
                                int n_fft, int hop, float amin, int normalize, float* out, float* out_tail, int n_tail,
                                void* stream);

int dam_stft_complex_f32(const void* pcm, int pcm_dtype, int64_t n_tracks, int64_t n_samples, int channels,
                         int64_t pcm_track_stride, int64_t n_sum, int64_t sum_stride, const float* window,
                         const float* twiddles, const float* gain, int n_fft, int hop, float* out, void* stream);
int dam_stft_complex_strided_f32(const void* pcm, int pcm_dtype, int64_t n_outer, int64_t outer_stride, int64_t n_inner,
                                 int64_t inner_stride, int64_t n_sum, int64_t sum_stride, int64_t n_samples, int channels,
                                 int64_t sample_stride, int64_t channel_stride, const float* window, const float* twiddles,
                                 const float* gain, int n_fft, int hop, float* out, void* stream);
int64_t dam_istft_workspace_bytes(int64_t n_tracks, int64_t n_frames, int n_fft, int hop, int64_t length);
int dam_istft_f32(const float* spec, const float* mag_db, int64_t n_tracks, int64_t n_frames, int n_fft, int hop,
                  int64_t length, const float* window, const float* twiddles, float* out, void* workspace,
                  int64_t workspace_bytes, void* stream);

int dam_augment_gains_f32(uint64_t seed, const int64_t* items, int64_t first_item, int n_items, int n_tracks,
                          float lo, float hi, float* gains, void* stream);


int64_t dam_conv_packed_weight_count(int n_out, int k_in, int kh, int kw);

int dam_conv_pack_weights_f32(const float* w_oihw, int O, int I, int KH, int KW, int transpose,
                              float* packed, void* stream);

int dam_conv_pack_weights_multi_f32(const int64_t* desc_dev, int n_tensors, int64_t max_total, void* stream);

int dam_conv2d_tapgrid_f32(const float* x, int B, int H, int W, int C, int in_nchw, const float* w_packed,
                           int k_chunks, int n_out, const float* bias, const float* in_scale,
                           const float* in_shift, int relu_in, int relu_out, float* y, int OHt, int OWt, int Ho, int Wo,
                           int out_stride, int out_off_h, int out_off_w, int in_stride, int nA, int nB,
                           int off_h, int step_h, int off_w, int step_w, int wt_base, int wt_sa, int wt_sb,
                           const float* res, const float* res_mask, float* bn_partial, int* bn_parts_host,
                           const struct dam_bn_bwd_sums* bn_bwd, float* workspace, int64_t workspace_floats,
                           void* batch, void* stream);

int dam_conv1x1_pair_f32(const float* x1, const float* w1_packed, int tap1, const float* x2, const float* w2_packed, int tap2,
                         int B, int H, int W, int C, int n_out, float* y, int OHt, int OWt, int out_stride, int out_off_h,
                         int out_off_w, void* stream);

int dam_dgrad_s2_3x3_f32(const float* dy, const float* w_packed_t, const float* dy_pair, const float* w_pair_packed_t, int B,
                         int Hd, int Wd, int Co, int Ci, float* dx, int H, int W, const struct dam_bn_bwd_sums* bn_bwd,
                         float* bn_partial, int* bn_parts_host, void* stream);

int dam_conv_s2_pair_fwd_f32(const float* x, const float* w_packed, const float* wsc_packed, int B, int H, int W, int Ci, int Co,
                             float* y, float* ysc, float* partial, float* partial_sc, int* parts_host, void* stream);

int64_t dam_conv_batch_bytes(void);
int dam_conv_batch_init(void* batch);
int dam_conv_batch_flush(void* batch, void* stream);

int dam_conv_last_launch(int* out16_host);

int64_t dam_conv2d_wgrad_workspace_floats(int n_out, int c_in, int kh, int kw);
int dam_conv2d_wgrad_f32(const float* x, int B, int H, int W, int C, int in_nchw, const float* in_scale,
                         const float* in_shift, int relu_in, const float* dy, int Ho, int Wo, int n_chan,
                         int n_out, int kh, int kw, int stride, int pad, int dil, float* dw, int c_real,
                         float* workspace, int64_t workspace_floats, void* reduce_queue, void* stream);

int64_t dam_wgrad_queue_bytes(void);
int dam_wgrad_queue_init(void* queue);
int dam_wgrad_queue_pending(const void* queue);
int dam_wgrad_queue_flush(void* queue, void* stream);
int dam_wgrad_queue_set_batching(void* queue, int on);

int dam_wgrad_last_launch(int* out16_host);

int dam_strip_diag_counters(uint32_t* out2_host, int reset);

int64_t dam_bn_workspace_floats(int C);

typedef struct dam_bn_fin {
    const float* gamma; const float* beta;
    float* running_mean; float* running_var; int64_t* num_batches_tracked;
    float momentum, eps;
    float* save_mean; float* save_invstd; float* scale; float* shift;
} dam_bn_fin;

typedef struct dam_bn_bwd_sums {
    const float* x; const float* mean; const float* invstd; const float* mask_scale; const float* mask_shift;
    const uint8_t* res_mask_bits;
    const uint8_t* mask_bits;
} dam_bn_bwd_sums;

int dam_bn_stats_f32(const float* x, int64_t n_pixels, int C, const float* gamma, const float* beta,
                     float* running_mean, float* running_var, int64_t* num_batches_tracked,
                     float momentum, float eps, float* save_mean, float* save_invstd, float* scale,
                     float* shift, float* workspace, void* stream);

int dam_bn_stats_pair_f32(const float* x_a, const float* x_b, int64_t n_pixels, int C, const struct dam_bn_fin* a,
                          const struct dam_bn_fin* b, float* workspace, void* stream);

int dam_bn_finalize_f32(const float* partial, int parts, int C, const float* gamma, const float* beta,
                        float* running_mean, float* running_var, int64_t* num_batches_tracked,
                        float momentum, float eps, float* save_mean, float* save_invstd, float* scale,
                        float* shift, void* stream);

int dam_bn_finalize_pair_f32(const float* partial_a, const float* partial_b, int parts, int C, const struct dam_bn_fin* a,
                             const struct dam_bn_fin* b, void* stream);

int dam_bn_stats_partial_f32(const float* x, int64_t n_pixels, int C, float* workspace, int* parts_host, void* stream);

int dam_bn_finalize_apply_f32(const float* partial, int parts, int C, const struct dam_bn_fin* fin, const float* x,
                              int64_t n_pixels, const float* res, const float* res_scale, const float* res_shift, int relu,
                              float* y, uint8_t* sign_bits, void* stream);

int dam_bn_eval_affine_f32(int C, const float* gamma, const float* beta, const float* running_mean,
                           const float* running_var, float eps, float* save_mean, float* save_invstd,
                           float* scale, float* shift, void* stream);

int dam_bn_apply_f32(const float* x, int64_t n_pixels, int C, const float* scale, const float* shift,
                     const float* res, const float* res_scale, const float* res_shift, int relu, float* y,
                     uint8_t* sign_bits, void* stream);

int dam_bn_backward_f32(const float* dy, const float* y_mask, const float* x, int64_t n_pixels, int C,
                        const float* gamma, const float* save_mean, const float* save_invstd, int training,
                        const float* mask_scale, const float* mask_shift, const uint8_t* mask_bits, float* dx,
                        float* dgamma, float* dbeta, float* workspace, int partials_given, void* stream);

int64_t dam_bn_pair_workspace_floats(int C);
int dam_bn_backward_pair_f32(const float* dy, const float* y_mask, const uint8_t* mask_bits, int64_t n_pixels, int C,
                             int training,
                             const float* x_a, const float* gamma_a, const float* mean_a, const float* invstd_a,
                             float* dx_a, float* dgamma_a, float* dbeta_a,
                             const float* x_b, const float* gamma_b, const float* mean_b, const float* invstd_b,
                             float* dx_b, float* dgamma_b, float* dbeta_b, float* workspace, void* stream);

int dam_channel_sum_f32(const float* x, int64_t n_pixels, int C, int n_real, float* out, float* workspace,
                        void* stream);

int dam_dropout_tick(int64_t* counter, int64_t n, int64_t* snapshot, void* stream);
int dam_dropout_apply_f32(const float* x, int64_t n, float p, uint64_t seed, const int64_t* snapshot, float* y,
                          void* stream);

int dam_heads_fwd_f32(const float* trunk, int B, int P, int C, int S, const float* conv_w, const float* conv_b,
                      const float* fc_w, const float* fc_b, float* h, float* gains, void* stream);
int64_t dam_heads_bwd_workspace_floats(int B, int P, int C, int S);
int dam_heads_bwd_f32(const float* dgains, const float* h, const float* trunk, int B, int P, int C, int S,
                      const float* conv_w, const float* fc_w, float* dtrunk, float* dconv_w, float* dconv_b,
                      float* dfc_w, float* dfc_b, float* workspace, void* stream);
int dam_masksum_fwd_f32(const float* x, const float* gains, int B, int S, int64_t FT, float* masked, void* stream);
int64_t dam_masksum_workspace_floats(int B, int S);
int dam_masksum_bwd_f32(const float* dmasked, const float* x, int B, int S, int64_t FT, float* dgains,
                        float* workspace, void* stream);
int dam_masksum_mse_f32(const float* x, const float* gains, const float* gt, int B, int S, int64_t FT,
                        float* masked, float* loss, float* dgains, float* workspace, void* stream);

int dam_adam_l2_step_f32(float* params, const float* grads, float* exp_avg, float* exp_avg_sq, int64_t n,
                         int64_t* step, float* derived2, float lr, float beta1, float beta2, float eps,
                         float weight_decay, float grad_scale, const float* hyper_dev, void* stream);

int dam_digest64_u32(const uint32_t* x, int64_t n, int64_t index_base, int max_blocks, int accumulate, uint64_t* out,
                     void* stream);


int dam_gains_smooth(const float* raw_db, int n_chunks, int n_stems, int window, int polyorder, double* amp,
                     double* smooth, float* smooth_f32, void* stream);

int dam_gain_ramp_apply(const void* audio, int audio_is_f64, const double* gains, int64_t rows, int64_t rows_per_gain,
                        int64_t n_samples, int n_gains, void* out, int out_is_f64, void* stream);

int64_t dam_mixdown_workspace_elems(int64_t rows);
int dam_mixdown_peak_normalize(const void* audio, int audio_is_f64, const double* gains, int n_stems, int64_t rows,
                               int64_t n_samples, int n_gains, int normalize, void* mix, int mix_is_f64,
                               void* workspace, void* stream);

int dam_loudness_kweight_coeffs(double rate, double* coef12);
int64_t dam_loudness_workspace_bytes(int64_t n_samples, int channels);
int dam_loudness_block_energy(const void* x, int x_is_f64, int64_t n_samples, int channels, int64_t sample_stride,
                              int64_t channel_stride, const double* coef12_host, const int64_t* blk_lo,
                              const int64_t* blk_hi, int n_blocks, double block_len, double* z, void* workspace,
                              void* stream);
int64_t dam_loudness_batch_workspace_bytes(int n_tracks, int64_t n_samples, int channels, int n_blocks);
int dam_loudness_block_energy_batch(const void* x, int x_is_f64, int n_tracks, int64_t n_samples, int channels,
                                    int64_t track_stride, int64_t sample_stride, int64_t channel_stride,
                                    const double* gains, int n_gains, const double* coef12_host, const int64_t* blk_lo,
                                    const int64_t* blk_hi, int n_blocks, double block_len, double* z, void* workspace,
                                    void* stream);
int dam_loudness_gate(const double* z, int n_tracks, int channels, int n_blocks, double* lufs, void* stream);
int dam_loudness_target_gains(const double* lufs, const double* target, int n, double* gains, void* stream);

typedef enum dam_wav_format { DAM_WAV_S16 = 0, DAM_WAV_S24 = 1, DAM_WAV_S32 = 2, DAM_WAV_F32 = 3 } dam_wav_format;
#define DAM_PCM_MAX_CHANNELS 8
#define DAM_PCM_MAX_BLOCKS 2048
int64_t dam_pcm_tile_frames(int x_is_f64);
int dam_pcm_max_blocks(void);
int dam_pcm_encode(const void* x, int x_is_f64, int channels, int64_t n_samples, const double* scale, int n_scale,
                   int format, int dither, uint64_t seed, void* out, int64_t* clip_count, void* stream);

int dam_true_peak_taps_host(double* h49);
int64_t dam_true_peak_tile_samples(void);
int dam_true_peak_max_blocks(void);
int64_t dam_true_peak_workspace_bytes(int n_tracks, int64_t n_samples, int channels);
int dam_true_peak_batch(const void* x, int x_is_f64, int n_tracks, int64_t n_samples, int channels, int64_t track_stride,
                        int64_t sample_stride, int64_t channel_stride, const double* gains, int n_gains,
                        double* sample_peak, double* true_peak, void* workspace, void* stream);
int dam_peak_limit_gains(double* gains, const double* peaks, int n_gains, int peaks_per_gain, double ceiling_lin,
                         void* stream);

int64_t dam_limiter_tile_samples(void);
int dam_limiter_max_lookahead(void);
int dam_limiter_max_hold(void);
int64_t dam_limiter_workspace_bytes(int n_sets, int64_t n_samples);
int dam_limiter_apply(const void* x, int x_is_f64, int n_sets, int64_t n_samples, int channels, int64_t set_stride,
                      int64_t sample_stride, int64_t channel_stride, const double* pre_gain, double ceiling_lin, int lookahead,
                      int hold, void* out, int out_is_f64, double* min_gain, int64_t* n_limited, void* workspace, void* stream);

#define DAM_LOUDNESS_ABS_GATE_POWER 0x1.f791ec6e1d5b7p-24
int dam_loudness_window_power(const double* e, int n_tracks, int channels, int n_hops, int w, double* power, double* lufs,
                              void* stream);
int dam_loudness_curve_stats(const double* power, int n_tracks, int n_windows, double* out, void* stream);
int dam_loudness_profile_error(const double* ref_lufs, const double* cand_lufs, int n_variants, int n_stems,
                               int n_windows, double* err, double* active, void* stream);

#define DAM_SPECTRUM_GATE 0x1.ad7f29abcaf48p-24
int dam_spectrum_frames_per_block(void);
int dam_spectrum_max_bands(void);
int64_t dam_spectrum_workspace_bytes(int n_mixes, int64_t n_samples, int hop, int n_bands);
int dam_spectrum_band_power(const void* x, int x_is_f64, int n_mixes, int n_stems, int channels, int64_t n_samples,
                            int64_t mix_stride, int64_t stem_stride, int64_t sample_stride, int64_t channel_stride,
                            const double* gains, int n_gains, const float* window, const float* twiddles, int n_fft, int hop,
                            const int32_t* edges, int n_bands, double* power, void* workspace, void* stream);
int dam_spectrum_balance_error(const double* ref_power, const double* cand_power, int n_variants, int n_bands, double* err,
                               int32_t* n_kept, void* stream);

#define DAM_GAINFIT_MAX_STEMS 8
#define DAM_GAINFIT_GATE 0x1.5798ee2308c3ap-27
#define DAM_GAINFIT_PIVOT 0x1p-40
int64_t dam_gainfit_tile_samples(void);
int64_t dam_gainfit_workspace_bytes(int n_windows, int64_t n_samples, int n_stems);
int dam_gainfit_moments(const void* x, int x_is_f64, int n_stems, int channels, int64_t n_samples, int64_t stem_stride,
                        int64_t sample_stride, int64_t channel_stride, const void* y, int y_is_f64, int64_t y_sample_stride,
                        int64_t y_channel_stride, int n_windows, double* moments, void* workspace, void* stream);
int dam_gainfit_solve(const double* moments, int n_windows, int n_stems, int pool, double ridge, double* gains,
                      double* residual, int32_t* status, void* stream);
int dam_gainfit_gain_error(const double* fit, const double* cand, int n_variants, int n_stems, int n_windows, int n_cand,
                           double* err, double* err_stem, int32_t* n_kept, void* stream);

int dam_nchw_to_nhwc16_f32(const float* x, int B, int C, int64_t HW, float* y, void* stream);

#ifdef __cplusplus
}
#endif
#endif
```

Measured before the change: 2.038 million stem-spectrogram-frames/s.

## Fuse paired BN backward reductions into downstream block's 3x3 dgrad epilogue

Adds a STATS==3 mode to the pipelined 3x3 conv dgrad kernel. For the shortcut block's two BatchNorms (main and shortcut), it accumulates the per-channel sums of dz, dz*x_a and dz*x_b in the epilogue of the next block's data-gradient conv. The paired BN backward then takes these precomputed partials instead of re-reading dy, the mask and both activations in its own reduction pass. This saves a full read pass over the activations in backward. In exchange the dgrad kernel does more epilogue work and reads more data, and a waves_per_eu attribute is added for that variant to control register pressure.

```diff
diff --git a/deep-audio-mixer_amd/_lib.py b/deep-audio-mixer_amd/_lib.py
--- a/deep-audio-mixer_amd/_lib.py
+++ b/deep-audio-mixer_amd/_lib.py
@@ -7,7 +7,7 @@
 _HERE = os.path.dirname(os.path.abspath(__file__))
 LIB_PATH = os.environ.get('DAM_LIB_PATH') or os.path.join(_HERE, 'libdam_hip.so')
 
-EXPECTED_ABI = 27
+EXPECTED_ABI = 28
 
 _STATUS = {0: 'DAM_OK', -1: 'DAM_ERR_BAD_ARG', -2: 'DAM_ERR_UNSUPPORTED', -3: 'DAM_ERR_LAUNCH',
            -4: 'DAM_ERR_WORKSPACE'}
@@ -67,7 +67,7 @@
     'dam_bn_apply_f32': (c_i, [c_p, c_i64, c_i, c_p, c_p, c_p, c_p, c_p, c_i, c_p, c_p, c_p]),
     'dam_bn_stats_pair_f32': (c_i, [c_p, c_p, c_i64, c_i, c_p, c_p, c_p, c_p]),
     'dam_bn_pair_workspace_floats': (c_i64, [c_i]),
-    'dam_bn_backward_pair_f32': (c_i, [c_p, c_p, c_p, c_i64, c_i, c_i] + [c_p] * 16),
+    'dam_bn_backward_pair_f32': (c_i, [c_p, c_p, c_p, c_i64, c_i, c_i] + [c_p] * 15 + [c_i, c_p]),
     'dam_bn_backward_f32': (c_i, [c_p, c_p, c_p, c_i64, c_i, c_p, c_p, c_p, c_i, c_p, c_p, c_p, c_p, c_p, c_p, c_p, c_i, c_p]),
     'dam_channel_sum_f32': (c_i, [c_p, c_i64, c_i, c_i, c_p, c_p, c_p]),
     'dam_dropout_tick': (c_i, [c_p, c_i64, c_p, c_p]),
@@ -133,7 +133,7 @@
 
 class BnBwdSums(ctypes.Structure):
     _fields_ = [('x', c_p), ('mean', c_p), ('invstd', c_p), ('mask_scale', c_p), ('mask_shift', c_p), ('res_mask_bits', c_p),
-                ('mask_bits', c_p)]
+                ('mask_bits', c_p), ('x2', c_p), ('mean2', c_p), ('invstd2', c_p)]
 
 
 _lib = None
diff --git a/deep-audio-mixer_amd/csrc/dam_bn.hip b/deep-audio-mixer_amd/csrc/dam_bn.hip
--- a/deep-audio-mixer_amd/csrc/dam_bn.hip
+++ b/deep-audio-mixer_amd/csrc/dam_bn.hip
@@ -860,7 +860,8 @@
                                         const float* x_a, const float* gamma_a, const float* mean_a, const float* invstd_a,
                                         float* dx_a, float* dgamma_a, float* dbeta_a,
                                         const float* x_b, const float* gamma_b, const float* mean_b, const float* invstd_b,
-                                        float* dx_b, float* dgamma_b, float* dbeta_b, float* workspace, void* stream) {
+                                        float* dx_b, float* dgamma_b, float* dbeta_b, float* workspace, int partials_given,
+                                        void* stream) {
     if ((y_mask != nullptr) == (mask_bits != nullptr)) return DAM_ERR_BAD_ARG;
     const bool bits = mask_bits != nullptr;
     if (bits) y_mask = reinterpret_cast<const float*>(mask_bits);
@@ -868,12 +869,14 @@
         !mean_b || !invstd_b || !dx_b || !dgamma_b || !dbeta_b || !workspace || n_pixels <= 0)
         return DAM_ERR_BAD_ARG;
     if (C % 16 || C > 1024) return DAM_ERR_UNSUPPORTED;
-    const BnLaunch l = bn_plan(n_pixels, C, fa_max_parts(C, 3));
-    if ((size_t)l.r * C * 3 * sizeof(float) > 64 * 1024) return DAM_ERR_UNSUPPORTED;
+    BnLaunch l = bn_plan(n_pixels, C, fa_max_parts(C, 3));
+    if (partials_given < 0 || partials_given > BN_MAX_PARTS) return DAM_ERR_BAD_ARG;
+    if (partials_given) l.parts = partials_given;
+    else if ((size_t)l.r * C * 3 * sizeof(float) > 64 * 1024) return DAM_ERR_UNSUPPORTED;
     const BnBwdSides<2> sd{{{x_a, gamma_a, mean_a, invstd_a, dx_a, dgamma_a, dbeta_a},
                             {x_b, gamma_b, mean_b, invstd_b, dx_b, dgamma_b, dbeta_b}}};
-    return bn_bwd_launch<2, 1, 3>(l, false, true, bits ? 3 : 1, sd, dy, y_mask, n_pixels, C, training, nullptr, nullptr, workspace,
-                                  (hipStream_t)stream);
+    return bn_bwd_launch<2, 1, 3>(l, partials_given != 0, true, bits ? 3 : 1, sd, dy, y_mask, n_pixels, C, training, nullptr, nullptr,
+                                  workspace, (hipStream_t)stream);
 }
 
 extern "C" int dam_channel_sum_f32(const float* x, int64_t n_pixels, int C, int n_real, float* out, float* workspace,
diff --git a/deep-audio-mixer_amd/csrc/dam_conv.hip b/deep-audio-mixer_amd/csrc/dam_conv.hip
--- a/deep-audio-mixer_amd/csrc/dam_conv.hip
+++ b/deep-audio-mixer_amd/csrc/dam_conv.hip
@@ -575,9 +575,11 @@
         if (bn_bwd->mask_bits ? (bn_bwd->mask_scale || bn_bwd->mask_shift || !res) : (!bn_bwd->mask_scale || !bn_bwd->mask_shift))
             return DAM_ERR_BAD_ARG;
         if (res && (!bn_bwd->res_mask_bits || !res_mask)) return DAM_ERR_BAD_ARG;
+        if (bn_bwd->x2 && (!bn_bwd->mean2 || !bn_bwd->invstd2 || !bn_bwd->mask_bits || !res || relu_out)) return DAM_ERR_BAD_ARG;
         bwd = BnBwdEpi{bn_bwd->x, bn_bwd->mean, bn_bwd->invstd, bn_bwd->mask_scale, bn_bwd->mask_shift, bn_bwd->res_mask_bits,
-                       bn_bwd->mask_bits};
-    }
+                       bn_bwd->mask_bits, bn_bwd->x2, bn_bwd->mean2, bn_bwd->invstd2};
+    }
+    const bool pair = bwd.x2 != nullptr;
     if (!x || !w_packed || !y || B <= 0 || H <= 0 || W <= 0 || C <= 0 || Ho <= 0 || Wo <= 0 || nA <= 0 || nB <= 0)
         return DAM_ERR_BAD_ARG;
     if (n_out % 16 || (in_stride != 1 && in_stride != 2) || out_stride < 1) return DAM_ERR_UNSUPPORTED;
@@ -612,10 +614,10 @@
     }
     if (!in_nchw) {
         int parts = 0;
-        const int rc = conv_strip_try(g, h_lo, h_hi, x, w_packed, bias, y, res, res_mask, bn_partial, &parts,
-                                      in_scale, in_shift, bwd, st);
+        const int rc = conv_strip_try(g, h_lo, h_hi, x, w_packed, bias, y, res, res_mask, pair ? nullptr : bn_partial, &parts,
+                                      in_scale, in_shift, pair ? BnBwdEpi{} : bwd, st);
         if (rc == DAM_OK) {
-            if (bn_partial && bn_parts_host) *bn_parts_host = parts;
+            if (bn_partial && bn_parts_host) *bn_parts_host = pair ? 0 : parts;
             return DAM_OK;
         }
         if (rc != DAM_ERR_UNSUPPORTED) return rc;
@@ -628,8 +630,9 @@
     }
     if (!getenv("DAM_NO_PIPE")) {
         int parts = 0;
+        const bool drop = bwd.x && res && !pair;
         const int rc = conv_pipe_try(g, h_hi - h_lo, x, w_packed, bias, in_scale, in_shift, y, res, res_mask, workspace,
-                                     (bwd.x && res) ? nullptr : bn_partial, &parts, (bwd.x && res) ? BnBwdEpi{} : bwd, st);
+                                     drop ? nullptr : bn_partial, &parts, drop ? BnBwdEpi{} : bwd, st);
         if (rc == DAM_OK && bn_partial && bn_parts_host) *bn_parts_host = parts;
         if (rc != DAM_ERR_UNSUPPORTED) return rc;
         if (nA == 3 && nB == 3 && !in_nchw && !bn_partial) {
diff --git a/deep-audio-mixer_amd/csrc/dam_conv_geo.h b/deep-audio-mixer_amd/csrc/dam_conv_geo.h
--- a/deep-audio-mixer_amd/csrc/dam_conv_geo.h
+++ b/deep-audio-mixer_amd/csrc/dam_conv_geo.h
@@ -31,6 +31,8 @@
     const float* mean; const float* invstd; const float* mscale; const float* mshift;
     const unsigned char* res_bits;
     const unsigned char* mask_bits;
+    const float* x2;
+    const float* mean2; const float* invstd2;
 };
 
 struct StripGeo {
diff --git a/deep-audio-mixer_amd/csrc/dam_conv_pipe.hip b/deep-audio-mixer_amd/csrc/dam_conv_pipe.hip
--- a/deep-audio-mixer_amd/csrc/dam_conv_pipe.hip
+++ b/deep-audio-mixer_amd/csrc/dam_conv_pipe.hip
@@ -43,7 +43,8 @@
 }
 
 template <int MB, int NB, int PIPE_U, int STATS, int KS>
-__global__ __launch_bounds__(PIPE_THREADS) void conv_pipe_kernel(const ConvGeo g, const int nunits, const float* __restrict__ X,
+__global__ __launch_bounds__(PIPE_THREADS) __attribute__((amdgpu_waves_per_eu(STATS == 3 && KS == 2 ? 6 : 1)))
+void conv_pipe_kernel(const ConvGeo g, const int nunits, const float* __restrict__ X,
                                                                  const float4* __restrict__ Wp, const float* __restrict__ bias,
                                                                  const float* __restrict__ in_scale,
                                                                  const float* __restrict__ in_shift, float* __restrict__ Y,
@@ -368,6 +369,11 @@
             bw_k1[nb] = *reinterpret_cast<const v4f*>(bwd.invstd + ch);
             bw_k2[nb] = -(*reinterpret_cast<const v4f*>(bwd.mean + ch)) * bw_k1[nb];
         }
+        float st_s3[STATS == 3 ? NB : 1][4];
+#pragma unroll
+        for (int nb = 0; nb < (STATS == 3 ? NB : 0); ++nb)
+#pragma unroll
+            for (int r = 0; r < 4; ++r) st_s3[nb][r] = 0.f;
 #pragma unroll
         for (int mb = 0; mb < MB; ++mb) {
             const int p = cur.p0 + mt * MW + mb * 16 + j;
@@ -395,6 +401,22 @@
                         st_s1[nb][r] += dz[r];
                         st_s2[nb][r] = fmaf(dz[r], xe[r], st_s2[nb][r]);
                     }
+                } else if (STATS == 3) {
+                    const unsigned ob = (unsigned)o * 4u;
+                    const v4f rv = *reinterpret_cast<const v4f*>(reinterpret_cast<const char*>(res) + ob);
+                    const v4f xa = *reinterpret_cast<const v4f*>(reinterpret_cast<const char*>(bwd.x) + ob);
+                    const v4f xb = *reinterpret_cast<const v4f*>(reinterpret_cast<const char*>(bwd.x2) + ob);
+                    const unsigned rb = bwd.res_bits[ob >> 4], ub = bwd.mask_bits[ob >> 4];
+                    v.x += (rb & 1u) ? rv.x : 0.f; v.y += (rb & 2u) ? rv.y : 0.f;
+                    v.z += (rb & 4u) ? rv.z : 0.f; v.w += (rb & 8u) ? rv.w : 0.f;
+                    const float dz[4] = {(ub & 1u) ? v.x : 0.f, (ub & 2u) ? v.y : 0.f, (ub & 4u) ? v.z : 0.f, (ub & 8u) ? v.w : 0.f};
+                    const float ea[4] = {xa.x, xa.y, xa.z, xa.w}, eb[4] = {xb.x, xb.y, xb.z, xb.w};
+#pragma unroll
+                    for (int r = 0; r < 4; ++r) {
+                        st_s1[nb][r] += dz[r];
+                        st_s2[nb][r] = fmaf(dz[r], ea[r], st_s2[nb][r]);
+                        st_s3[nb][r] = fmaf(dz[r], eb[r], st_s3[nb][r]);
+                    }
                 } else if (res) {
                     const float4 rv = *reinterpret_cast<const float4*>(res + o);
                     if (res_mask) {
@@ -428,6 +450,15 @@
         V_ += __builtin_bit_cast(float, __builtin_amdgcn_update_dpp(0, __builtin_bit_cast(int, V_), 0x121, 0xF, 0xF, false)); \
     } while (0)
             const size_t rec = ((size_t)cur.img * g.tiles_m + (cur.p0 / UPX)) * MT + mt;
+            v4f pc_ia[STATS == 3 ? NB : 1], pc_ma[STATS == 3 ? NB : 1], pc_ib[STATS == 3 ? NB : 1], pc_mb[STATS == 3 ? NB : 1];
+#pragma unroll
+            for (int nb = 0; nb < (STATS == 3 ? NB : 0); ++nb) {
+                const int ch = (cur.nb0 + nb) * 16 + kq * 4;
+                pc_ia[nb] = *reinterpret_cast<const v4f*>(bwd.invstd + ch);
+                pc_ma[nb] = *reinterpret_cast<const v4f*>(bwd.mean + ch);
+                pc_ib[nb] = *reinterpret_cast<const v4f*>(bwd.invstd2 + ch);
+                pc_mb[nb] = *reinterpret_cast<const v4f*>(bwd.mean2 + ch);
+            }
             float n = st_n;
             DAM_ROW_SUM(n);
 #pragma unroll
@@ -438,7 +469,16 @@
                     DAM_ROW_SUM(s1);
                     DAM_ROW_SUM(s2);
                     const int ch = (cur.nb0 + nb) * 16 + kq * 4 + r;
-                    if (STATS == 2) {
+                    if (STATS == 3) {
+                        float s3 = st_s3[nb][r];
+                        DAM_ROW_SUM(s3);
+                        if (j == 0 && ch < g.N) {
+                            float* o = stats + ((unsigned)rec * (unsigned)g.N + (unsigned)ch) * 3u;
+                            o[0] = s1;
+                            o[1] = reinterpret_cast<const float*>(&pc_ia[nb])[r] * fmaf(-reinterpret_cast<const float*>(&pc_ma[nb])[r], s1, s2);
+                            o[2] = reinterpret_cast<const float*>(&pc_ib[nb])[r] * fmaf(-reinterpret_cast<const float*>(&pc_mb[nb])[r], s1, s3);
+                        }
+                    } else if (STATS == 2) {
                         if (j == 0 && ch < g.N) { float* o = stats + (rec * g.N + ch) * 2; o[0] = s1; o[1] = s2; }
                     } else if (j == 0 && ch < g.N) {
                         const float md = n > 0.f ? s1 / n : 0.f;
@@ -484,19 +524,22 @@
     int mode = 0;
     if (stats) {
         const int64_t parts = (int64_t)g.B * g.tiles_m * (4 / KS);
-        mode = bwd.x ? 2 : 1;
+        mode = bwd.x ? (bwd.x2 ? 3 : 2) : 1;
         if (parts > (bwd.x ? BN_BWD_RECORDS_MAX : BN_RECORDS_MAX)) { stats = nullptr; mode = 0; }
+        else if (mode == 3 && (int64_t)g.B * g.OHt * g.OWt * g.N * 4 >= ((int64_t)1 << 32)) { stats = nullptr; mode = 0; }
         else if (stats_parts) *stats_parts = (int)parts;
     }
-    if (bwd.x) res = mode == 2 ? bwd.x : nullptr;
-    int wgs = mode == 2 ? pipe_slots<MB, NB, PU, 2, KS>(lds) : (mode == 1 ? pipe_slots<MB, NB, PU, 1, KS>(lds) : pipe_slots<MB, NB, PU, 0, KS>(lds));
+    if (bwd.x && !bwd.x2) res = mode == 2 ? bwd.x : nullptr;
+    int wgs = mode == 3 ? pipe_slots<MB, NB, PU, 3, KS>(lds)
+                        : (mode == 2 ? pipe_slots<MB, NB, PU, 2, KS>(lds)
+                                     : (mode == 1 ? pipe_slots<MB, NB, PU, 1, KS>(lds) : pipe_slots<MB, NB, PU, 0, KS>(lds)));
     if (const char* e = getenv("DAM_PIPE_WGS")) wgs = atoi(e);
     if (wgs < 1) wgs = 1;
     if (wgs > nunits) wgs = nunits;
 #define DAM_PIPE_LAUNCH(S_)                                                                                                 \
     hipLaunchKernelGGL((conv_pipe_kernel<MB, NB, PU, S_, KS>), dim3((unsigned)wgs), dim3(PIPE_THREADS), lds, st, g, nunits, X,  \
                        reinterpret_cast<const float4*>(Wp), bias, sc, sh, Y, res, res_mask, workspace, stats, bwd)
-    if (mode == 2) DAM_PIPE_LAUNCH(2); else if (mode == 1) DAM_PIPE_LAUNCH(1); else DAM_PIPE_LAUNCH(0);
+    if (mode == 3) DAM_PIPE_LAUNCH(3); else if (mode == 2) DAM_PIPE_LAUNCH(2); else if (mode == 1) DAM_PIPE_LAUNCH(1); else DAM_PIPE_LAUNCH(0);
 #undef DAM_PIPE_LAUNCH
     DAM_CHECK_LAUNCH();
     conv_last_launch = ConvLaunchNote{CONV_FAM_PIPE, MB, NB, 0, 0, 0, 0, 0, PU, mode, KS, 1, 1};
@@ -508,7 +551,9 @@
 int conv_pipe_try(ConvGeo g, int row_span, const float* X, const float* Wp, const float* bias, const float* sc, const float* sh,
                   float* Y, const float* res, const float* res_mask, float* workspace, float* stats, int* stats_parts,
                   const BnBwdEpi& bwd, hipStream_t st) {
-    if (bwd.x && (res || !stats)) return DAM_ERR_BAD_ARG;
+    if (bwd.x && !stats) return DAM_ERR_BAD_ARG;
+    if (bwd.x2 ? (!bwd.x || !res || !bwd.res_bits || !bwd.mask_bits || !bwd.mean2 || !bwd.invstd2 || g.relu_out) : (bwd.x && res))
+        return DAM_ERR_BAD_ARG;
     if (g.nA != 3 || g.nB != 3 || g.in_nchw) return DAM_ERR_UNSUPPORTED;
     if ((size_t)g.H * g.W * g.C * 4 >= ((size_t)1 << 30)) return DAM_ERR_UNSUPPORTED;
     const int64_t npix = (int64_t)g.Ho * g.Wo;
diff --git a/deep-audio-mixer_amd/layers.py b/deep-audio-mixer_amd/layers.py
--- a/deep-audio-mixer_amd/layers.py
+++ b/deep-audio-mixer_amd/layers.py
@@ -194,6 +194,30 @@
         self.partials = None
         if sums is not None:
             _UpstreamBn.hits += 1
+        return sums
+
+    hits = 0
+
+
+class _UpstreamBnPair:
+    __slots__ = ('c2', 'mean2', 'invstd2', 'cs', 'means', 'invstds', 'bits', 'partials', 'dx_ptr', 'dx_version')
+
+    def __init__(self, c2, mean2, invstd2, cs, means, invstds, bits):
+        self.c2, self.mean2, self.invstd2, self.cs, self.means, self.invstds, self.bits = c2, mean2, invstd2, cs, means, invstds, bits
+        self.partials, self.dx_ptr, self.dx_version = None, None, None
+
+    def request(self):
+        return (self.c2, self.mean2, self.invstd2, self.cs, self.means, self.invstds, self.bits)
+
+    def offer(self, sums, dx):
+        self.partials, self.dx_ptr, self.dx_version = sums, dx.data_ptr(), dx._version
+
+    def take(self, grad):
+        ok = self.partials is not None and self.dx_ptr == grad.data_ptr() and self.dx_version == grad._version
+        sums = self.partials if ok else None
+        self.partials = None
+        if sums is not None:
+            _UpstreamBnPair.hits += 1
         return sums
 
     hits = 0
@@ -277,10 +301,14 @@
         ctx.up_self = None
         if wsc is None and ops.DGRAD_BN_SUMS:
             ctx.up_self = out._dam_upstream = _UpstreamBn(c2, m2, i2, None, None, bits)
+        ctx.up_pair = None
+        if wsc is not None and training and ops.DGRAD_BN_SUMS:
+            ctx.up_pair = out._dam_upstream_pair = _UpstreamBnPair(c2, m2, i2, cs, ms, is_, bits)
         ctx.blk, ctx.training, ctx.has_sc = blk, training, wsc is not None
         ctx.upstream = getattr(x, '_dam_upstream', None)
         if wsc is not None and (ctx.upstream is None or ctx.upstream.bits is None or ctx.upstream.scale is not None):
             ctx.upstream = None
+        ctx.upstream_pair = getattr(x, '_dam_upstream_pair', None) if wsc is None and training else None
         ctx.slots = tuple(_slot(p) for p in (w1, g1, b1, w2, g2, b2, wsc, gsc, bsc))
         return out
 
@@ -297,8 +325,10 @@
         keep = lambda grad, slot: None if slot is not None else grad
         wview = lambda slot, w: None if slot is None else slot.view(w.shape)
         if ctx.has_sc:
+            sums_p = ctx.up_pair.take(dout) if ctx.up_pair is not None else None
             (dc2, dg2, db2), (dcs, dgs, dbs) = ops.bn_backward_pair(dout, None, (c2, g2, m2, i2, s_g2, s_b2),
-                                                                    (cs, gsc, ms, is_, s_gs, s_bs), tr, mask_bits=bits)
+                                                                    (cs, gsc, ms, is_, s_gs, s_bs), tr, mask_bits=bits,
+                                                                    partials=sums_p)
         else:
             sums2 = ctx.up_self.take(dout) if ctx.up_self is not None else None
             dc2, dg2, db2 = ops.bn_backward(dout, None, c2, g2, m2, i2, tr, dgamma=s_g2, dbeta=s_b2, mask_bits=bits, partials=sums2)
@@ -332,6 +362,10 @@
         if up is not None and ops.DGRAD_BN_SUMS and up.c.shape == x.shape:
             dx, sums = blk.spec1.dgrad(dc1, w1, hw, res=dout, res_mask=out, res_mask_bits=bits, bn_bwd=up.request())
             up.offer(sums, dx)
+        elif ctx.upstream_pair is not None and ops.DGRAD_BN_SUMS and ctx.upstream_pair.c2.shape == x.shape:
+            upp = ctx.upstream_pair
+            dx, sums = blk.spec1.dgrad(dc1, w1, hw, res=dout, res_mask=out, res_mask_bits=bits, bn_bwd_pair=upp.request())
+            upp.offer(sums, dx)
         else:
             dx = blk.spec1.dgrad(dc1, w1, hw, res=dout, res_mask=out)
         return (dx,) + first + (None, None, None, None, None)
diff --git a/deep-audio-mixer_amd/ops.py b/deep-audio-mixer_amd/ops.py
--- a/deep-audio-mixer_amd/ops.py
+++ b/deep-audio-mixer_amd/ops.py
@@ -118,8 +118,28 @@
 
 
 def conv2d_dgrad(dy, wpt, n_in, H, W, kh, kw, stride=1, pad=0, dil=1, res=None, res_mask=None, accumulate_into=None,
-                 bn_bwd=None, res_mask_bits=None, pair_1x1=None, _s2_sums=None):
+                 bn_bwd=None, res_mask_bits=None, pair_1x1=None, _s2_sums=None, bn_bwd_pair=None):
     _lib.require_cuda(dy, wpt)
+    if bn_bwd_pair is not None:
+        if bn_bwd is not None or stride != 1 or accumulate_into is not None:
+            raise ValueError('bn_bwd_pair: stride-1 data gradients only, not together with bn_bwd')
+        if res is None or res_mask is None or res_mask_bits is None:
+            raise ValueError('bn_bwd_pair: with res, res_mask and res_mask_bits')
+        _f32c(dy, 'dy'), _f32c(res, 'res'), _f32c(res_mask, 'res_mask')
+        xa, mean_a, invstd_a, xb, mean_b, invstd_b, up_bits = bn_bwd_pair
+        _lib.require_cuda(xa, xb, up_bits)
+        _f32c(xa, 'c2'), _f32c(xb, 'cs')
+        B, Ho, Wo, Co = dy.shape
+        n16 = (n_in + 15) // 16 * 16
+        if tuple(xa.shape) != (B, H, W, n16) or xb.shape != xa.shape or tuple(res.shape) != (B, H, W, n16):
+            raise ValueError('bn_bwd_pair: c2, cs and res have the shape of the data gradient')
+        dx = torch.empty((B, H, W, n16), dtype=torch.float32, device=dy.device)
+        rec = torch.empty(_lib.lib().dam_bn_pair_workspace_floats(n16), dtype=torch.float32, device=dy.device)
+        epi = _lib.BnBwdSums(_lib.ptr(xa), _lib.ptr(mean_a), _lib.ptr(invstd_a), None, None, _lib.ptr(res_mask_bits),
+                             _lib.ptr(up_bits), _lib.ptr(xb), _lib.ptr(mean_b), _lib.ptr(invstd_b))
+        parts = _tapgrid(dy, B, Ho, Wo, Co, False, wpt, Co // 16, n16, None, None, None, False, dx, H, W, H, W, 1, 0, 0, 1,
+                         kh, kw, pad, -dil, pad, -dil, 0, kw, 1, res, res_mask, bn_partial=rec, bn_bwd=epi)
+        return dx, ((rec, parts) if parts > 0 else None)
     if bn_bwd is not None and stride == 2:
         if accumulate_into is not None or res is not None or len(bn_bwd) < 6 or bn_bwd[5] is None or bn_bwd[3] is not None:
             raise ValueError('bn_bwd at stride 2: mask as sign bytes, no residual / accumulation')
@@ -469,7 +489,7 @@
     return (y, bits) if sign_bits else y
 
 
-def bn_backward_pair(dy, y_mask, a, b, training=True, mask_bits=None):
+def bn_backward_pair(dy, y_mask, a, b, training=True, mask_bits=None, partials=None):
     _lib.require_cuda(dy, a[0], b[0])
     if (y_mask is None) == (mask_bits is None):
         raise ValueError('exactly one of y_mask / mask_bits')
@@ -483,13 +503,13 @@
         dbeta = torch.empty(C, dtype=torch.float32, device=x.device) if dbeta is None else dbeta
         outs.append((dx, dgamma, dbeta))
     L = _lib.lib()
-    ws = _workspace(dy.device, L.dam_bn_pair_workspace_floats(C))
+    ws, given = (_workspace(dy.device, L.dam_bn_pair_workspace_floats(C)), 0) if partials is None else partials
     args = []
     for (x, gamma, mean, invstd, _, _), (dx, dgamma, dbeta) in zip((a, b), outs):
         args += [_lib.ptr(x), _lib.ptr(gamma), _lib.ptr(mean), _lib.ptr(invstd), _lib.ptr(dx), _lib.ptr(dgamma), _lib.ptr(dbeta)]
     _lib.check(L.dam_bn_backward_pair_f32(_lib.ptr(dy), _lib.ptr(y_mask), _lib.ptr(mask_bits), dy.numel() // C, C,
                                           1 if training else 0, *args,
-                                          _lib.ptr(ws), _lib.stream()), 'dam_bn_backward_pair_f32')
+                                          _lib.ptr(ws), given, _lib.stream()), 'dam_bn_backward_pair_f32')
     return outs[0], outs[1]
 
 
diff --git a/include/dam_hip.h b/include/dam_hip.h
--- a/include/dam_hip.h
+++ b/include/dam_hip.h
@@ -20,7 +20,7 @@
 #define DAM_PCM_ROTATE 0x200
 struct dam_bn_bwd_sums;
 
-#define DAM_ABI_VERSION 27
+#define DAM_ABI_VERSION 28
 const char* dam_arch(void);
 int dam_abi_version(void);
 
@@ -125,6 +125,7 @@
     const float* x; const float* mean; const float* invstd; const float* mask_scale; const float* mask_shift;
     const uint8_t* res_mask_bits;
     const uint8_t* mask_bits;
+    const float* x2; const float* mean2; const float* invstd2;
 } dam_bn_bwd_sums;
 
 int dam_bn_stats_f32(const float* x, int64_t n_pixels, int C, const float* gamma, const float* beta,
@@ -168,7 +169,7 @@
                              const float* x_a, const float* gamma_a, const float* mean_a, const float* invstd_a,
                              float* dx_a, float* dgamma_a, float* dbeta_a,
                              const float* x_b, const float* gamma_b, const float* mean_b, const float* invstd_b,
-                             float* dx_b, float* dgamma_b, float* dbeta_b, float* workspace, void* stream);
+                             float* dx_b, float* dgamma_b, float* dbeta_b, float* workspace, int partials_given, void* stream);
 
 int dam_channel_sum_f32(const float* x, int64_t n_pixels, int C, int n_real, float* out, float* workspace,
                         void* stream);
```

Result: no change. 2.046 million stem-spectrogram-frames/s, median of 6 (+0.4%).
